# nyu-systems/CLM-GS

Measured on AMD Instinct MI355X. Metric: training images/s (Rubble-4K 28M Gaussians clm_offload), higher is better.
Workload: dtype f32

## Files before the change

clm_gs_amd/_lib.py:

```python
import ctypes
import os
import time

import torch

_HERE = os.path.dirname(os.path.abspath(__file__))
LIB_PATH = os.environ.get("CLMGS_LIB_PATH") or os.path.join(_HERE, "libclmgs_hip.so")

_vp, _i, _i64, _f, _sz = ctypes.c_void_p, ctypes.c_int, ctypes.c_int64, ctypes.c_float, ctypes.c_size_t
_d = ctypes.c_double

SIGNATURES = {
    "clmgs_version": (_i, []),
    "clmgs_last_error": (ctypes.c_char_p, []),
    "clmgs_projection_fwd": (_i, [_vp, _i, _i, _vp, _vp, _vp, _vp, _vp, _i, _i, _f, _f, _f, _f, _vp, _vp, _vp, _vp]),
    "clmgs_visibility_select_temp_bytes": (_sz, [_i, _i]),
    "clmgs_visibility_select_count": (_i, [_vp, _i, _i, _vp, _vp, _vp, _vp, _vp, _i, _i, _f, _f, _f, _f, _vp, _sz, _vp]),
    "clmgs_visibility_select_count_blocks": (_i, [_vp, _i, _i, _vp, _vp, _vp, _vp, _vp, _i, _i, _f, _f, _f, _f, _vp, _sz, _vp, _vp]),
    "clmgs_visibility_select_count_blocks_sel": (_i, [_vp, _i, _i, _vp, _vp, _vp, _vp, _vp, _i, _i, _f, _f, _f, _f, _vp, _sz, _vp, _vp,
                                                      _vp, ctypes.c_uint64, _i, _i]),
    "clmgs_visibility_select_emit": (_i, [_vp, _i, _i, _vp, _vp]),
    "clmgs_visibility_raw": (_i, [_vp, _i, _i, _vp, _vp, _vp, _vp, _vp, _i, _i, _f, _f, _f, _f, _vp]),
    "clmgs_projection_bwd": (_i, [_vp, _i, _i, _vp, _vp, _vp, _vp, _vp, _i, _i, _f, _vp, _vp, _vp, _vp, _vp, _vp, _vp]),
    "clmgs_sh_fwd": (_i, [_vp, _i, _i, _vp, _vp, _vp, _vp]),
    "clmgs_sh_bwd": (_i, [_vp, _i, _i, _vp, _vp, _vp, _vp, _vp, _i, _vp]),
    "clmgs_isect_count_temp_bytes": (_sz, [_i]),
    "clmgs_isect_count": (_i, [_vp, _i, _i, _vp, _vp, _i, _i, _i, _vp, _vp, _vp, _sz]),
    "clmgs_isect_sort_temp_bytes": (_sz, [_i64]),
    "clmgs_isect_emit_sort": (_i, [_vp, _i, _i, _i64, _vp, _vp, _vp, _vp, _i, _i, _i, _vp, _vp, _vp, _sz]),
    "clmgs_isect_offsets": (_i, [_vp, _i64, _vp, _i, _i, _i, _vp]),
    "clmgs_isect2_order_temp_bytes": (_sz, [_i]),
    "clmgs_isect2_order_count": (_i, [_vp, _i, _vp, _vp, _vp, _i, _i, _i, _vp, _vp, _vp, _vp, _vp, _vp, _sz, _vp]),
    "clmgs_isect2_sort_temp_bytes": (_sz, [_i64]),
    "clmgs_isect2_emit_sort": (_i, [_vp, _i, _i64, _vp, _vp, _vp, _vp, _i, _i, _vp, _vp, _vp, _vp, _vp, _sz, _vp]),
    "clmgs_isect2_emit_sort_dev": (_i, [_vp, _i, _i64, _vp, _vp, _vp, _vp, _vp, _i, _i, _vp, _vp, _vp, _vp, _vp, _sz, _vp]),
    "clmgs_isect3_front_temp_bytes": (_sz, [_i, _i]),
    "clmgs_isect3_front": (_i, [_vp, _i, _vp, _vp, _i, _i, _i, _vp, _vp, _vp, _vp, _sz]),
    "clmgs_isect3_bin_temp_bytes": (_sz, [_i64, _i]),
    "clmgs_isect3_bin": (_i, [_vp, _i, _i64, _vp, _i, _i, _vp, _vp, _vp, _vp, _vp, _vp, _vp, _sz]),
    "clmgs_isect3_bin_dev": (_i, [_vp, _i, _i64, _vp, _vp, _i, _i, _vp, _vp, _vp, _vp, _vp, _vp, _vp, _sz]),
    "clmgs_rasterize_fwd_dev": (_i, [_vp, _i, _i, _i64, _vp, _vp, _i, _i, _i, _i, _i, _vp, _vp, _vp, _vp, _vp, _vp]),
    "clmgs_rasterize_bwd_dev": (_i, [_vp, _i, _i, _i64, _vp, _vp, _vp, _i, _i, _i, _i, _i, _vp, _vp, _vp, _vp, _vp, _vp, _vp, _vp, _vp]),
    "clmgs_rasterize_pack_bytes": (_sz, [_i, _i]),
    "clmgs_rasterize_fwd": (_i, [_vp, _i, _i, _i64, _vp, _vp, _vp, _vp, _vp, _i, _i, _i, _i, _i, _vp, _vp, _vp, _vp, _vp, _vp]),
    "clmgs_rasterize_partials_bytes": (_sz, [_i64]),
    "clmgs_rasterize_bwd": (_i, [_vp, _i, _i, _i64, _vp, _vp, _i, _i, _i, _i, _i, _vp, _vp, _vp, _vp, _vp, _vp, _vp, _vp, _vp, _vp, _vp, _vp, _vp, _vp]),
    "clmgs_rasterize_contrib_pack_bytes": (_sz, [_i, _i]),
    "clmgs_rasterize_contrib": (_i, [_vp, _i, _i, _i64, _vp, _vp, _vp, _i, _i, _i, _i, _i, _vp, _vp, _vp, _i64, _vp, _vp, _vp, _vp]),
    "clmgs_rasterize_median_pack_bytes": (_sz, [_i, _i]),
    "clmgs_rasterize_median": (_i, [_vp, _i, _i, _i64, _vp, _vp, _vp, _vp, _i, _i, _i, _i, _i, _vp, _vp, _vp, _vp, _vp]),
    "clmgs_ray_depth": (_i, [_vp, _i, _i, _i, _i, _vp, _vp, _vp, _vp, _vp, _vp, _d, _i, _vp]),
    "clmgs_rasterize4_fwd": (_i, [_vp, _i, _i, _i64, _vp, _vp, _vp, _vp, _vp, _i, _i, _i, _i, _i, _vp, _vp, _vp, _vp, _vp, _vp]),
    "clmgs_rasterize4_bwd": (_i, [_vp, _i, _i, _i64, _vp, _vp, _i, _i, _i, _i, _i, _vp, _vp, _vp, _vp, _vp, _vp, _vp, _vp, _vp, _vp, _vp, _vp, _vp, _vp]),
    "clmgs_rasterize4_slot_bwd": (_i, [_vp, _i, _i, _i64, _vp, _vp, _i, _i, _i, _i, _i, _vp, _vp, _vp, _vp, _vp, _vp, _vp, _vp, _vp, _vp, _vp, _vp, _vp, _vp]),
    "clmgs_rasterize4_fwd_dev": (_i, [_vp, _i, _i, _i64, _vp, _vp, _i, _i, _i, _i, _i, _vp, _vp, _vp, _vp, _vp, _vp]),
    "clmgs_rasterize4_bwd_dev": (_i, [_vp, _i, _i, _i64, _vp, _vp, _vp, _i, _i, _i, _i, _i, _vp, _vp, _vp, _vp, _vp, _vp, _vp, _vp, _vp]),
    "clmgs_preprocess_grid_cap": (_i, []),
    "clmgs_preprocess_fwd": (_i, [_vp, _i, _vp, _vp, _vp, _vp, _vp, _vp, _i, _vp, _vp, _vp, _i, _i, _i, _f, _f, _f, _f, _vp, _vp, _vp, _vp, _vp, _vp, _vp, _vp]),
    "clmgs_preprocess_bwd": (_i, [_vp, _i, _vp, _vp, _vp, _vp, _vp, _vp, _i, _vp, _vp, _vp, _i, _i, _i, _f, _vp, _vp, _vp, _vp, _vp, _vp, _vp, _vp, _vp, _vp, _vp, _i, _vp, _vp, _vp, _vp, _i]),
    "clmgs_rasterize_abs_bwd": (_i, [_vp, _i, _i, _i64, _vp, _vp, _i, _i, _i, _i, _i, _vp, _vp, _vp, _vp, _vp, _vp, _vp, _vp, _vp, _vp, _vp, _vp, _vp, _vp, _vp]),
    "clmgs_rasterize_abs_bwd_dev": (_i, [_vp, _i, _i, _i64, _vp, _vp, _vp, _i, _i, _i, _i, _i, _vp, _vp, _vp, _vp, _vp, _vp, _vp, _vp, _vp]),
    "clmgs_preprocess_abs_bwd": (_i, [_vp, _i, _vp, _vp, _vp, _vp, _vp, _vp, _i, _vp, _vp, _vp, _i, _i, _i, _f, _vp, _vp, _vp, _vp, _vp, _vp, _vp, _vp, _vp, _vp, _vp, _i, _vp, _vp, _vp, _vp, _i, _vp]),
    "clmgs_projection_aa_fwd": (_i, [_vp, _i, _i, _vp, _vp, _vp, _vp, _vp, _i, _i, _f, _f, _f, _f, _vp, _vp, _vp, _vp, _vp]),
    "clmgs_projection_aa_bwd": (_i, [_vp, _i, _i, _vp, _vp, _vp, _vp, _vp, _i, _i, _f, _vp, _vp, _vp, _vp, _vp, _vp, _vp, _vp]),
    "clmgs_projection_ortho_fwd": (_i, [_vp, _i, _i, _vp, _vp, _vp, _vp, _vp, _i, _i, _f, _f, _f, _f, _vp, _vp, _vp, _vp, _vp]),
    "clmgs_projection_ortho_bwd": (_i, [_vp, _i, _i, _vp, _vp, _vp, _vp, _vp, _i, _i, _f, _vp, _vp, _vp, _vp, _vp, _vp, _vp, _vp]),
    "clmgs_preprocess_aa_fwd": (_i, [_vp, _i, _vp, _vp, _vp, _vp, _vp, _vp, _i, _vp, _vp, _vp, _i, _i, _i, _f, _f, _f, _f, _vp, _vp, _vp, _vp, _vp, _vp, _vp, _vp]),
    "clmgs_preprocess_aa_bwd": (_i, [_vp, _i, _vp, _vp, _vp, _vp, _vp, _vp, _i, _vp, _vp, _vp, _i, _i, _i, _f, _vp, _vp, _vp, _vp, _vp, _vp, _vp, _vp, _vp, _vp, _vp, _i, _vp, _vp, _vp, _vp, _i]),
    "clmgs_preprocess_aa_abs_bwd": (_i, [_vp, _i, _vp, _vp, _vp, _vp, _vp, _vp, _i, _vp, _vp, _vp, _i, _i, _i, _f, _vp, _vp, _vp, _vp, _vp, _vp, _vp, _vp, _vp, _vp, _vp, _i, _vp, _vp, _vp, _vp, _i, _vp]),
    "clmgs_ssim_fwd": (_i, [_vp, _i, _i, _i, _i, _vp, _vp, _vp, _vp, _vp, _vp]),
    "clmgs_ssim_bwd": (_i, [_vp, _i, _i, _i, _i, _vp, _vp, _vp, _f, _vp, _vp, _vp, _vp]),
    "clmgs_loss_slots": (_i, []),
    "clmgs_l1_ssim_loss_fwd": (_i, [_vp, _i, _i, _vp, _i64, _i64, _i64, _vp, _vp, _vp, _vp, _vp]),
    "clmgs_l1_ssim_loss_bwd": (_i, [_vp, _i, _i, _vp, _i64, _i64, _i64, _vp, _vp, _f, _vp, _vp, _vp, _vp]),
    "clmgs_l1_ssim_loss_masked_fwd": (_i, [_vp, _i, _i, _vp, _i64, _i64, _i64, _vp, _vp, _vp, _vp, _vp, _vp]),
    "clmgs_l1_ssim_loss_masked_bwd": (_i, [_vp, _i, _i, _vp, _i64, _i64, _i64, _vp, _vp, _f, _vp, _vp, _vp, _vp, _vp]),
    "clmgs_exposure_partials_rows": (_i, [_i, _i]),
    "clmgs_exposure_fwd": (_i, [_vp, _i, _i, _vp, _i64, _i64, _i64, _vp, _vp, _i64, _i64, _i64]),
    "clmgs_exposure_bwd": (_i, [_vp, _i, _i, _vp, _i64, _i64, _i64, _vp, _vp, _i64, _i64, _i64, _vp, _i64, _i64, _i64, _vp]),
    "clmgs_exposure_grad_finish": (_i, [_vp, _i, _vp, _vp]),
    "clmgs_bilagrid_partials_rows": (_i, [_i, _i, _i, _i]),
    "clmgs_bilagrid_fwd": (_i, [_vp, _i, _i, _vp, _i64, _i64, _i64, _vp, _i, _i, _i, _vp, _i64, _i64, _i64]),
    "clmgs_bilagrid_bwd": (_i, [_vp, _i, _i, _vp, _i64, _i64, _i64, _vp, _i, _i, _i, _vp, _i64, _i64, _i64, _vp, _i64, _i64, _i64, _vp]),
    "clmgs_bilagrid_grad_finish": (_i, [_vp, _i, _i, _i, _i, _i, _vp, _vp]),
    "clmgs_bilagrid_tv_grad": (_i, [_vp, _vp, _i64, _i, _i, _i, _f, _vp]),
    "clmgs_sky_fwd": (_i, [_vp, _i, _i, _vp, _i64, _i64, _i64, _vp, _vp, _vp, _vp, _i, _i, _vp, _i64, _i64, _i64]),
    "clmgs_sky_bwd": (_i, [_vp, _i, _i, _vp, _i64, _i64, _i64, _vp, _vp, _vp, _vp, _i, _i, _vp, _vp]),
    "clmgs_sky_acc_add": (_i, [_vp, _i64, _vp, _vp]),
    "clmgs_sky_grad_convert": (_i, [_vp, _i64, _vp, _vp]),
    "clmgs_pose_grad_partials_rows": (_i, [_i]),
    "clmgs_pose_grad": (_i, [_vp, _i, _vp, _vp, _vp, _vp, _vp, _vp, _i, _vp, _vp, _vp, _i, _i, _i, _f, _vp, _vp, _vp, _vp, _vp, _i, _vp]),
    "clmgs_pose_grad_finish": (_i, [_vp, _i, _vp, _vp]),
    "clmgs_projection_viewmat_partials_rows": (_i, [_i]),
    "clmgs_projection_viewmat_bwd": (_i, [_vp, _i, _i, _vp, _vp, _vp, _vp, _vp, _i, _i, _f, _vp, _vp, _vp, _vp, _vp, _vp, _vp]),
    "clmgs_invdepth_partials_rows": (_i, [_i, _i]),
    "clmgs_invdepth_pack": (_i, [_vp, _i, _vp, _vp, _vp]),
    "clmgs_invdepth_l1_fwd_bwd": (_i, [_vp, _i, _i, _vp, _i64, _i64, _vp, _f, _f, _vp, _f, _vp, _i64, _i64, _vp]),
    "clmgs_invdepth_finish": (_i, [_vp, _i, _vp, _vp]),
    "clmgs_invdepth_rows_bwd": (_i, [_vp, _i, _vp, _vp, _vp, _vp, _vp, _vp, _vp, _vp, _i]),
    "clmgs_area_resample_u8": (_i, [_vp, _i, _i, _i, _i, _vp, _vp]),
    "clmgs_area_resample_u16": (_i, [_vp, _i, _i, _i, _vp, _vp]),
    "clmgs_area_resample_mask": (_i, [_vp, _i, _i, _i, _vp, _vp, _vp]),
    "clmgs_undistort_u8": (_i, [_vp, _i, _i, _i, _i, _i, _vp, _i, _d, _d, _vp, _vp, _vp, _vp, _vp]),
    "clmgs_undistort_u16": (_i, [_vp, _i, _i, _i, _i, _vp, _i, _d, _d, _vp, _vp]),
    "clmgs_vq_assign_temp_bytes": (_sz, [_i]),
    "clmgs_vq_assign": (_i, [_vp, _i64, _i, _vp, _vp, _vp, _vp, _vp, _sz]),
    "clmgs_vq_accumulate": (_i, [_vp, _i64, _i, _vp, _vp, _d, _vp, _vp]),
    "clmgs_vq_finish": (_i, [_vp, _i, _vp, _vp, _d, _vp]),
    "clmgs_tsdf_integrate": (_i, [_vp, _i, _i, _i, _vp, _i, _i, _i, _vp, _vp, _vp, _vp, _f, _f, _f, _f, _f, _i]),
    "clmgs_tsdf_cells": (_i, [_vp, _i, _i, _i, _vp, _f, _vp]),
    "clmgs_tsdf_vertices": (_i, [_vp, _i, _i, _i, _vp, _vp, _i, _vp, _vp, _vp]),
    "clmgs_tsdf_quad_count": (_i, [_vp, _i, _i, _i, _vp, _f, _vp, _vp]),
    "clmgs_tsdf_quads": (_i, [_vp, _i, _i, _i, _vp, _f, _vp, _vp, _i, _i, _vp]),
    "clmgs_tsdf_mark": (_i, [_vp, _i, _i, _i, _vp, _i, _i, _i, _vp, _vp, _vp, _f, _f, _f, _f, _d]),
    "clmgs_tsdf_sparse_integrate": (_i, [_vp, _i, _i, _i, _i, _vp, _vp, _i, _i, _i, _vp, _vp, _vp, _vp, _f, _f, _f, _f, _f, _i]),
    "clmgs_tsdf_sparse_extract": (_i, [_vp, _i, _i, _i, _i, _i, _vp, _vp, _vp, _f, _vp, _vp, _vp, _i, _i, _vp, _vp, _vp, _vp,
                                       _vp, _vp]),
    "clmgs_mesh_hook": (_i, [_vp, _i, _i, _vp, _vp, _vp]),
    "clmgs_mesh_shortcut": (_i, [_vp, _i, _vp, _vp]),
    "clmgs_mesh_component_faces": (_i, [_vp, _i, _i, _vp, _vp, _vp]),
    "clmgs_mesh_decimate_mark": (_i, [_vp, _i, _i, _vp, _vp]),
    "clmgs_mesh_decimate_keys": (_i, [_vp, _i, _vp, _vp, _d, _vp, _vp]),
    "clmgs_mesh_decimate_faces": (_i, [_vp, _i, _i, _i, _vp, _vp, _vp, _vp, _vp]),
    "clmgs_mesh_decimate_place": (_i, [_vp, _i, _i, _i, _vp, _vp, _vp, _vp, _vp, _vp, _i64, _vp, _vp, _i64, _vp, _d, _vp, _vp,
                                       _vp]),
    "clmgs_mcmc_relocation": (_i, [_vp, _i64, _vp, _vp, _vp, _vp, _vp]),
    "clmgs_mcmc_reg_grad": (_i, [_vp, _i64, _vp, _i64, _vp, _i64, _vp, _i64, _vp, _i64, _f, _f]),
    "clmgs_mcmc_noise": (_i, [_vp, _i64, _vp, _vp, _vp, _vp, _vp, _f, _vp]),
    "clmgs_rows_gather": (_i, [_vp, _vp, _vp, _vp, _vp, _i, _i64, _i, _i]),
    "clmgs_rows_scatter_add": (_i, [_vp, _vp, _vp, _vp, _vp, _i, _i64, _i, _i]),
    "clmgs_scatter_to_bit": (_i, [_vp, _vp, _i, _vp, _i64, _i]),
    "clmgs_extract_ffs": (_i, [_vp, _vp, _i, _i64, _vp]),
    "clmgs_pair_overlap_count": (_i, [_vp, _vp, _i, _i64, _i, _vp]),
    "clmgs_set_signal": (_i, [_vp, _vp, _i, ctypes.c_int32]),
    "clmgs_adam_rows": (_i, [_vp, _vp, _vp, _vp, _vp, _vp, _i, _vp, _i64, _i, _vp, _d, _d, _d, _i, _i, _f, _i]),
    "clmgs_pack_small": (_i, [_vp, _i64, _vp, _vp, _vp, _vp, _vp]),
    "clmgs_adam_small_packed": (_i, [_vp, _i64, _vp, _vp, _vp, _vp, _vp, _vp, _d, _d, _d, _i, _i, _f, _vp, _i]),
    "clmgs_adam_catch_up": (_i, [_vp, _vp, _vp, _vp, _vp, _vp, _i, _i64, _i, _vp, _d, _d, _d, _i, _i, _i, _vp, _vp, _f, _i]),
    "clmgs_host_adam_rows": (_i, [_vp, _vp, _vp, _vp, _vp, _i64, _i, _vp, _d, _d, _d, _i, _i, _f, _i, _vp, _i]),
    "clmgs_host_pool_start": (_i, [_i]),
    "clmgs_host_usable_cpus": (_i, []),
    "clmgs_memcpy_async": (_i, [_vp, _vp, _vp, _sz, _i]),
    "clmgs_host_rows_prepare": (_i, [_vp, _vp, _vp, _vp, _vp, _vp, _vp, _i64, _i, _vp, _d, _d, _d, _i, _i, _i, _f, _i, _vp, _i]),
    "clmgs_densify_stats": (_i, [_vp, _i64, _vp, _vp, _vp, _i, _f, _f, _vp, _vp, _vp]),
    "clmgs_morton_order_temp_bytes": (_sz, [_i64]),
    "clmgs_morton_order": (_i, [_vp, _i64, _vp, _vp, _vp, _vp, _sz]),
    "clmgs_tsp_tour": (_i, [_i, _vp, _vp]),
    "clmgs_knn3_mean_dist2": (_i, [_vp, _i, _vp, _vp, _f, _f, _f, _f, _i, _i, _i, _i, _vp]),
    "clmgs_host_groups_temp_bytes": (_sz, [_i64]),
    "clmgs_host_groups": (_i, [_vp, _i64, _vp, _vp, _i, _i, _vp, _i, _vp, _vp, _vp, _vp, _vp, _sz]),
    "clmgs_publish_pack": (_i, [_vp, _vp, _vp, _vp, _vp, _i, _i64, _i64, _i64, _i]),
    "clmgs_visibility_candidates": (_i, [_vp, _i, _i, _i, _i, _vp, _vp, _vp, _vp, _i, _i, _f, _f, _f, _f, _f, _vp]),
    "clmgs_small_rows_scatter": (_i, [_vp, _i64, _vp, _vp, _vp, _vp, _vp, _vp, _vp]),
    "clmgs_adam_small_packed_range": (_i, [_vp, _i64, _i64, _i64, _vp, _vp, _vp, _vp, _vp, _vp, _d, _d, _d, _i, _i, _f, _vp, _i]),
    "clmgs_small_deferred_kmax": (_i, []),
    "clmgs_adam_small_deferred": (_i, [_vp, _i64, _vp, _vp, _vp, _vp, _vp, _vp, _vp, _i, _i, _vp, _vp, _vp, _vp, _d, _d, _d,
                                       _f, _i, _vp, _vp, _i, _i, _f, _f, _f, _i, _vp]),
    "clmgs_adam_small_deferred_sel": (_i, [_vp, _i64, _vp, _vp, _vp, _vp, _vp, _vp, _vp, _i, _i, _vp, _vp, _vp, _vp, _d, _d, _d,
                                           _f, _i, _vp, _vp, _i, _i, _f, _f, _f, _i, _vp, _vp, _vp, ctypes.c_uint64, _i]),
    "clmgs_device_errors": (_i, [_vp, _i]),
    "clmgs_pinned_alloc": (_vp, [_sz]),
    "clmgs_pinned_free": (_i, [_vp]),
}

_lib = None

TIMING = None
STATS = {"n_isects": [], "n_emitted": [], "host_wait_s": 0.0}


class ClmgsError(RuntimeError):
    pass


class _Entry:

    def __init__(self, name, fn, takes_stream):
        self.name, self.fn, self.takes_stream = name, fn, takes_stream

    def __call__(self, *args):
        if TIMING is None or not self.takes_stream:
            return self.fn(*args)
        s, e = torch.cuda.Event(enable_timing=True), torch.cuda.Event(enable_timing=True)
        h = getattr(args[0], "value", args[0])
        st = torch.cuda.ExternalStream(h) if h else torch.cuda.current_stream()
        s.record(st)
        rc = self.fn(*args)
        e.record(st)
        TIMING.setdefault(self.name, []).append((s, e))
        return rc


class _Namespace:
    pass


_NO_STREAM = {"clmgs_version", "clmgs_loss_slots", "clmgs_preprocess_grid_cap","clmgs_exposure_partials_rows", "clmgs_bilagrid_partials_rows", "clmgs_invdepth_partials_rows", "clmgs_pose_grad_partials_rows", "clmgs_projection_viewmat_partials_rows", "clmgs_small_deferred_kmax", "clmgs_isect3_front_temp_bytes",
              "clmgs_isect3_bin_temp_bytes", "clmgs_last_error", "clmgs_isect_count_temp_bytes",
              "clmgs_isect_sort_temp_bytes", "clmgs_host_groups_temp_bytes", "clmgs_isect2_order_temp_bytes", "clmgs_isect2_sort_temp_bytes", "clmgs_visibility_select_temp_bytes", "clmgs_rasterize_pack_bytes", "clmgs_rasterize_contrib_pack_bytes", "clmgs_rasterize_median_pack_bytes", "clmgs_rasterize_partials_bytes", "clmgs_host_adam_rows", "clmgs_host_pool_start", "clmgs_host_usable_cpus", "clmgs_host_rows_prepare", "clmgs_tsp_tour",
              "clmgs_pinned_alloc", "clmgs_pinned_free", "clmgs_device_errors", "clmgs_vq_assign_temp_bytes"}


def timing_summary():
    out = {}
    for name, evs in (TIMING or {}).items():
        out[name] = (len(evs), sum(s.elapsed_time(e) for s, e in evs))
    return out


def lib():
    global _lib
    if _lib is None:
        if not os.path.exists(LIB_PATH):
            raise ClmgsError(
                f"{LIB_PATH} not found: build it with `python -c 'import __graft_entry__ as g; g.build()'` "
                "(make -C clm_gs_amd/csrc).  clm_gs_amd has no CPU/eager fallback."
            )
        l = ctypes.CDLL(LIB_PATH)
        ns = _Namespace()
        for name, (res, args) in SIGNATURES.items():
            fn = getattr(l, name)
            fn.restype = res
# ... 88 lines not shown
```

clm_gs_amd/csrc/clm_ops.hip:

```cpp
#include <stdlib.h>

#include "common.h"
#include "vis_math.h"
#include "radix.h"

namespace clmgs {
__device__ uint32_t g_dev_err;
static uint32_t* device_error_word() {
  static thread_local uint32_t* p[16] = {nullptr};
  int dev = 0;
  if (hipGetDevice(&dev) != hipSuccess || dev < 0 || dev >= 16) dev = 0;
  if (!p[dev]) {
    void* a = nullptr;
    if (hipGetSymbolAddress(&a, HIP_SYMBOL(g_dev_err)) == hipSuccess) p[dev] = (uint32_t*)a;
  }
  return p[dev];
}


template <typename IdxT>
__device__ __forceinline__ int64_t row_of(const void* idx, int64_t i) {
  return idx ? (int64_t)reinterpret_cast<const IdxT*>(idx)[i] : i;
}

template <typename IdxT, bool ADD>
__global__ void __launch_bounds__(256)
rows_move_f4_kernel(float* __restrict__ dst, const float* __restrict__ src,
                    const void* __restrict__ dst_idx, const void* __restrict__ src_idx,
                    int64_t n_rows, int f4_per_row) {
  const int64_t total = n_rows * f4_per_row;
  for (int64_t i = blockIdx.x * (int64_t)blockDim.x + threadIdx.x; i < total;
       i += (int64_t)gridDim.x * blockDim.x) {
    const int64_t r = i / f4_per_row;
    const int k = (int)(i - r * f4_per_row);
    const int64_t sr = row_of<IdxT>(src_idx, r), dr = row_of<IdxT>(dst_idx, r);
    const float4 v = reinterpret_cast<const float4*>(src)[sr * f4_per_row + k];
    float4* d = reinterpret_cast<float4*>(dst) + dr * f4_per_row + k;
    if (ADD) {
      float4 o = *d;
      o.x += v.x; o.y += v.y; o.z += v.z; o.w += v.w;
      *d = o;
    } else {
      *d = v;
    }
  }
}

template <typename IdxT, bool ADD>
__global__ void __launch_bounds__(256)
rows_move_f1_kernel(float* __restrict__ dst, const float* __restrict__ src,
                    const void* __restrict__ dst_idx, const void* __restrict__ src_idx,
                    int64_t n_rows, int cols) {
  const int64_t total = n_rows * cols;
  for (int64_t i = blockIdx.x * (int64_t)blockDim.x + threadIdx.x; i < total;
       i += (int64_t)gridDim.x * blockDim.x) {
    const int64_t r = i / cols;
    const int k = (int)(i - r * cols);
    const int64_t sr = row_of<IdxT>(src_idx, r), dr = row_of<IdxT>(dst_idx, r);
    const float v = src[sr * cols + k];
    if (ADD) dst[dr * cols + k] += v; else dst[dr * cols + k] = v;
  }
}

template <bool ADD>
static int rows_move(void* stream, float* dst, const float* src, const void* dst_idx,
                     const void* src_idx, int idx_is_64, int64_t n_rows, int cols,
                     int grid_blocks) {
  CLMGS_CHECK_ARG(n_rows >= 0 && cols > 0);
  if (n_rows == 0) return 0;
  CLMGS_CHECK_ARG(dst && src);
  hipStream_t s = (hipStream_t)stream;
  const bool f4 = (cols % 4 == 0) && (((uintptr_t)dst | (uintptr_t)src) % 16 == 0);
  const int64_t total = f4 ? n_rows * (cols / 4) : n_rows * cols;
  int grid = grid_blocks > 0 ? grid_blocks : min(ceil_div(total, 256), 256 * 8);
  if (f4) {
    if (idx_is_64)
      hipLaunchKernelGGL((rows_move_f4_kernel<int64_t, ADD>), dim3(grid), dim3(256), 0, s, dst, src,
                         dst_idx, src_idx, n_rows, cols / 4);
    else
      hipLaunchKernelGGL((rows_move_f4_kernel<int32_t, ADD>), dim3(grid), dim3(256), 0, s, dst, src,
                         dst_idx, src_idx, n_rows, cols / 4);
  } else {
    if (idx_is_64)
      hipLaunchKernelGGL((rows_move_f1_kernel<int64_t, ADD>), dim3(grid), dim3(256), 0, s, dst, src,
                         dst_idx, src_idx, n_rows, cols);
    else
      hipLaunchKernelGGL((rows_move_f1_kernel<int32_t, ADD>), dim3(grid), dim3(256), 0, s, dst, src,
                         dst_idx, src_idx, n_rows, cols);
  }
  CLMGS_LAUNCH_CHECK();
  return 0;
}

__global__ void __launch_bounds__(256)
publish_pack_kernel(float* __restrict__ msg, const float* __restrict__ table, const int64_t* __restrict__ own,
                    const int32_t* __restrict__ stamp, int step, int64_t lo, int64_t n, int64_t chunk, int f4_per_row) {
  const int64_t total = n * f4_per_row;
  for (int64_t i = blockIdx.x * (int64_t)blockDim.x + threadIdx.x; i < total;
       i += (int64_t)gridDim.x * blockDim.x) {
    const int64_t r = i / f4_per_row;
    const int k = (int)(i - r * f4_per_row);
    const int64_t row = own[r];
    const bool live = !stamp || stamp[row] == step;
    float4 v = make_float4(0.f, 0.f, 0.f, 0.f);
    if (live) v = reinterpret_cast<const float4*>(table)[row * f4_per_row + k];
    reinterpret_cast<float4*>(msg)[i] = v;
    if (k == 0) reinterpret_cast<int32_t*>(msg)[chunk * f4_per_row * 4 + r] = (int32_t)(row - lo);
  }
}

template <typename T>
__global__ void __launch_bounds__(256)
host_group_keys_kernel(int64_t n, const int64_t* __restrict__ touched, const T* __restrict__ bitmap, int bsz,
                       const uint8_t* __restrict__ staged, uint32_t* __restrict__ kf, uint32_t* __restrict__ kl,
                       int32_t* __restrict__ rows32) {
  for (int64_t j = blockIdx.x * (int64_t)blockDim.x + threadIdx.x; j < n; j += (int64_t)gridDim.x * blockDim.x) {
    const int64_t row = touched[j];
    unsigned long long bm = (unsigned long long)(typename std::make_unsigned<T>::type)bitmap[row];
    if (bsz < 64) bm &= (1ull << bsz) - 1ull;
    int first = 254, last = 254;
    if (bm) {
      first = (bsz - 1) - (63 - __clzll((long long)bm));
      last = (bsz - 1) - (__ffsll((long long)bm) - 1);
    }
    kf[j] = (staged && staged[row]) ? 255u : (uint32_t)first;
    kl[j] = (uint32_t)last;
    rows32[j] = (int32_t)row;
  }
}

__global__ void __launch_bounds__(256)
host_group_finish_kernel(int64_t n, int bsz, const uint32_t* __restrict__ tot_first, const uint32_t* __restrict__ tot_last,
                         const int32_t* __restrict__ late_sorted, int slot0, int32_t* __restrict__ slot_of,
                         int64_t* __restrict__ counts) {
  const int64_t n_late = n - (int64_t)tot_first[255];
  if (blockIdx.x == 0 && threadIdx.x <= 2 * bsz) {
    const int t = threadIdx.x;
    counts[t] = t < bsz ? (int64_t)tot_first[t] : (t < 2 * bsz ? (int64_t)tot_last[t - bsz] : n_late);
  }
  for (int64_t k = blockIdx.x * (int64_t)blockDim.x + threadIdx.x; k < n_late; k += (int64_t)gridDim.x * blockDim.x)
    slot_of[late_sorted[k]] = slot0 + (int32_t)k;
}

template <typename T>
__global__ void scatter_to_bit_kernel(T* __restrict__ bitmap, const int64_t* __restrict__ filter,
                                      int64_t n, int bit) {
  using U = typename std::make_unsigned<T>::type;
  const U m = (U)((U)1 << bit);
  for (int64_t i = blockIdx.x * (int64_t)blockDim.x + threadIdx.x; i < n;
       i += (int64_t)gridDim.x * blockDim.x) {
    U* p = reinterpret_cast<U*>(bitmap) + filter[i];
    *p = (U)(*p | m);
  }
}

template <typename T>
__global__ void extract_ffs_kernel(const T* __restrict__ bitmap, int64_t N, uint8_t* __restrict__ ffs) {
  using U = typename std::make_unsigned<T>::type;
  for (int64_t i = blockIdx.x * (int64_t)blockDim.x + threadIdx.x; i < N;
       i += (int64_t)gridDim.x * blockDim.x) {
    const unsigned long long v = (unsigned long long)(U)bitmap[i];
    ffs[i] = (uint8_t)(v ? (__ffsll((long long)v)) : 0);
  }
}

template <typename T>
__global__ void __launch_bounds__(256)
pair_overlap_kernel(const T* __restrict__ bitmap, int64_t N, int bsz, int32_t* __restrict__ cnt) {
  using U = typename std::make_unsigned<T>::type;
  __shared__ int sh[64];
  for (int i = threadIdx.x; i < 64; i += blockDim.x) sh[i] = 0;
  __syncthreads();
  for (int64_t i = blockIdx.x * (int64_t)blockDim.x + threadIdx.x; i < N;
       i += (int64_t)gridDim.x * blockDim.x) {
    const unsigned long long v = (unsigned long long)(U)bitmap[i];
    unsigned long long both = v & (v << 1);
    while (both) {
      const int b = __ffsll((long long)both) - 1;
      both &= both - 1;
      atomicAdd(&sh[bsz - 1 - b], 1);
    }
  }
  __syncthreads();
  for (int i = threadIdx.x; i < bsz - 1; i += blockDim.x)
    if (sh[i]) atomicAdd(&cnt[i], sh[i]);
}

__global__ void set_signal_kernel(int32_t* signal, int idx, int32_t value) {
  __threadfence_system();
  __hip_atomic_store(signal + idx, value, __ATOMIC_RELEASE, __HIP_MEMORY_SCOPE_SYSTEM);
}

__device__ __forceinline__ float adam_update(float p, float m, float v, float lr_bc, float inv_sqrt_bc2, float eps) {
#pragma clang fp contract(off)
  const float ratio = m * __builtin_amdgcn_rcpf(__builtin_fmaf(__builtin_amdgcn_sqrtf(v), inv_sqrt_bc2, eps));
  return __builtin_fmaf(-lr_bc, ratio, p);
}

template <bool GRAD_FUSED = false>
__device__ __forceinline__ float adam_elem(float& m, float& v, float p, float g, float lr_bc, float beta1,
                                           float beta2, float ob1, float ob2, float eps,
                                           float inv_sqrt_bc2) {
#pragma clang fp contract(off)
  if constexpr (GRAD_FUSED) {
    m = __builtin_fmaf(ob1, g, beta1 * m);
    v = __builtin_fmaf(ob2 * g, g, beta2 * v);
  } else {
    m = __builtin_fmaf(beta1, m, ob1 * g);
    v = __builtin_fmaf(beta2, v, (ob2 * g) * g);
  }
  return adam_update(p, m, v, lr_bc, inv_sqrt_bc2, eps);
}

__device__ __forceinline__ float adam_elem_nograd(float& m, float& v, float p, float lr_bc, float beta1, float beta2,
                                                  float eps, float inv_sqrt_bc2) {
#pragma clang fp contract(off)
  m = beta1 * m;
  v = beta2 * v;
  return adam_update(p, m, v, lr_bc, inv_sqrt_bc2, eps);
}

template <int VEC> struct VecT;
template <> struct VecT<1> { using type = float; };
template <> struct VecT<4> { using type = float4; };
template <int VEC> __device__ __forceinline__ void vload(const float* a, float (&x)[VEC]) {
  if constexpr (VEC == 4) { const float4 t = *reinterpret_cast<const float4*>(a); x[0] = t.x; x[1] = t.y; x[2] = t.z; x[3] = t.w; }
  else x[0] = *a;
}
template <int VEC> __device__ __forceinline__ void vstore(float* a, const float (&x)[VEC]) {
  if constexpr (VEC == 4) *reinterpret_cast<float4*>(a) = make_float4(x[0], x[1], x[2], x[3]);
  else *a = x[0];
}

template <typename IdxT, int VEC>
__global__ void __launch_bounds__(256)
adam_rows_kernel(float* __restrict__ p, float* __restrict__ g, float* __restrict__ m,
                 float* __restrict__ v, const void* __restrict__ rows,
                 const uint8_t* __restrict__ mask, int64_t n_rows, int cols,
                 const float* __restrict__ col_lr, float beta1, float beta2, float ob1, float ob2,
                 float eps, float inv_bc1, float inv_sqrt_bc2, float grad_scale, int zero_grad) {
  const int cv = cols / VEC;
  const int64_t total = n_rows * cv;
  for (int64_t i = blockIdx.x * (int64_t)blockDim.x + threadIdx.x; i < total;
       i += (int64_t)gridDim.x * blockDim.x) {
    const int64_t r = i / cv;
    const int k = (int)(i - r * cv) * VEC;
    const int64_t row = row_of<IdxT>(rows, r);
    if (mask && !mask[row]) continue;
    const int64_t o = row * cols + k;
    float gg[VEC], mm[VEC], vv[VEC], pp[VEC], lr[VEC];
    vload<VEC>(m + o, mm); vload<VEC>(v + o, vv); vload<VEC>(p + o, pp); vload<VEC>(col_lr + k, lr);
    if (g) vload<VEC>(g + o, gg);
#pragma unroll
    for (int c = 0; c < VEC; ++c) {
      pp[c] = adam_elem(mm[c], vv[c], pp[c], g ? gg[c] * grad_scale : 0.f, lr[c] * inv_bc1, beta1, beta2, ob1, ob2,
                        eps, inv_sqrt_bc2);
      gg[c] = 0.f;
    }
    vstore<VEC>(m + o, mm); vstore<VEC>(v + o, vv); vstore<VEC>(p + o, pp);
    if (zero_grad && g) vstore<VEC>(g + o, gg);
  }
}

__device__ __forceinline__ float pow_beta(float beta, float x) {
  return __builtin_amdgcn_exp2f(x * __builtin_amdgcn_logf(beta));
}

struct CatchUpK {
  float beta1, beta2, ob1, ob2, eps, grad_scale;
  int bias_correction, max_replay;
};

__device__ __forceinline__ void adam_bias(const CatchUpK& K, float pw1, float pw2, float& inv_bc1, float& inv_sqrt_bc2) {
#pragma clang fp contract(off)
  inv_bc1 = inv_sqrt_bc2 = 1.f;
  if (K.bias_correction) {
    inv_bc1 = 1.f / (1.f - pw1);
    inv_sqrt_bc2 = 1.f / sqrtf(1.f - pw2);
  }
}

template <int VEC>
__device__ __forceinline__ void adam_replay(const CatchUpK& K, int from, int to, float (&pp)[VEC], float (&mm)[VEC],
                                            float (&vv)[VEC], const float (&lr)[VEC]) {
#pragma clang fp contract(off)
  const int missed = to - from;
  if (missed <= 0) return;
  const int n = min(missed, K.max_replay);
  float pw1 = pow_beta(K.beta1, (float)(from + 1)), pw2 = pow_beta(K.beta2, (float)(from + 1));
  for (int j = 0; j < n; ++j) {
    float inv_bc1, inv_sqrt_bc2;
    adam_bias(K, pw1, pw2, inv_bc1, inv_sqrt_bc2);
#pragma unroll
    for (int c = 0; c < VEC; ++c)
      pp[c] = adam_elem_nograd(mm[c], vv[c], pp[c], lr[c] * inv_bc1, K.beta1, K.beta2, K.eps, inv_sqrt_bc2);
    pw1 = pw1 * K.beta1; pw2 = pw2 * K.beta2;
  }
  if (missed > n) {
    const int d = missed - n;
    const float f1 = pow_beta(K.beta1, (float)d), f2 = pow_beta(K.beta2, (float)d);
#pragma unroll
    for (int c = 0; c < VEC; ++c) { mm[c] = mm[c] * f1; vv[c] = vv[c] * f2; }
  }
}

template <int VEC>
__device__ __forceinline__ void adam_waiting_step(const CatchUpK& K, int gs, float (&pp)[VEC], float (&mm)[VEC],
                                                  float (&vv)[VEC], float (&gg)[VEC], const float (&lr)[VEC]) {
#pragma clang fp contract(off)
  float inv_bc1, inv_sqrt_bc2;
  adam_bias(K, pow_beta(K.beta1, (float)gs), pow_beta(K.beta2, (float)gs), inv_bc1, inv_sqrt_bc2);
#pragma unroll
  for (int c = 0; c < VEC; ++c) {
    pp[c] = adam_elem<true>(mm[c], vv[c], pp[c], gg[c] * K.grad_scale, lr[c] * inv_bc1, K.beta1, K.beta2, K.ob1, K.ob2,
                            K.eps, inv_sqrt_bc2);
    gg[c] = 0.f;
  }
}

template <int VEC> __device__ __forceinline__ bool adam_any_state(const float (&mm)[VEC], const float (&vv)[VEC]) {
  bool any_state = false;
#pragma unroll
  for (int c = 0; c < VEC; ++c) any_state |= (mm[c] != 0.f) | (vv[c] != 0.f);
  return any_state;
}

template <typename IdxT, int VEC>
__global__ void __launch_bounds__(256)
adam_catch_up_kernel(float* __restrict__ p, float* __restrict__ m, float* __restrict__ v,
                     const int32_t* __restrict__ last_step, const void* __restrict__ rows,
                     int64_t n_rows, int cols, const float* __restrict__ col_lr, float beta1,
                     float beta2, float eps, int to_step, int bias_correction, int max_replay,
                     float* __restrict__ g, const int32_t* __restrict__ g_step, float grad_scale,
                     float ob1, float ob2,
                     int keep_grad) {
  const CatchUpK K = {beta1, beta2, ob1, ob2, eps, grad_scale, bias_correction, max_replay};
  const int cv = cols / VEC;
  const int64_t total = n_rows * cv;
  for (int64_t i = blockIdx.x * (int64_t)blockDim.x + threadIdx.x; i < total;
       i += (int64_t)gridDim.x * blockDim.x) {
    const int64_t r = i / cv;
    const int k = (int)(i - r * cv) * VEC;
    const int64_t row = row_of<IdxT>(rows, r);
    int a = last_step[row];
    const int gs = g_step ? g_step[row] : 0;
    const bool pending = gs > a && gs <= to_step;
    if (to_step - a <= 0) continue;
    const int64_t o = row * cols + k;
    float mm[VEC], vv[VEC], pp[VEC], lr[VEC], gg[VEC];
    vload<VEC>(m + o, mm); vload<VEC>(v + o, vv); vload<VEC>(p + o, pp); vload<VEC>(col_lr + k, lr);
    if (pending) vload<VEC>(g + o, gg);
    if (!pending && !adam_any_state<VEC>(mm, vv)) continue;
    if (pending) {
      adam_replay<VEC>(K, a, gs - 1, pp, mm, vv, lr);
      adam_waiting_step<VEC>(K, gs, pp, mm, vv, gg, lr);
      if (!keep_grad) vstore<VEC>(g + o, gg);
      a = gs;
    }
    adam_replay<VEC>(K, a, to_step, pp, mm, vv, lr);
    vstore<VEC>(m + o, mm); vstore<VEC>(v + o, vv); vstore<VEC>(p + o, pp);
  }
}

template <typename IdxT>
__global__ void __launch_bounds__(256)
adam_catch_up48_kernel(float* __restrict__ p, float* __restrict__ m, float* __restrict__ v,
                       const int32_t* __restrict__ last_step, const void* __restrict__ rows,
                       unsigned n_rows, const float* __restrict__ col_lr, float beta1,
                       float beta2, float eps, int to_step, int bias_correction, int max_replay,
                       float* __restrict__ g, const int32_t* __restrict__ g_step, float grad_scale,
                       float ob1, float ob2, int keep_grad) {
  constexpr int VEC = 4;
  const CatchUpK K = {beta1, beta2, ob1, ob2, eps, grad_scale, bias_correction, max_replay};
  const unsigned t0 = blockIdx.x * 256u + threadIdx.x;
  const unsigned r_stride = gridDim.x * 256u / 12u;
  unsigned r = t0 / 12u;
  const int k = (int)(t0 - r * 12u) * VEC;
  if (r >= n_rows) return;
  float lr[VEC];
  vload<VEC>(col_lr + k, lr);
  int64_t row_next = row_of<IdxT>(rows, (int64_t)r);
  int a_next = last_step[row_next];
  int gs_next = g_step ? g_step[row_next] : 0;
  int64_t row_next2 = (r + r_stride < n_rows) ? row_of<IdxT>(rows, (int64_t)(r + r_stride)) : row_next;
  for (; r < n_rows; r += r_stride) {
    const int64_t row = row_next;
    int a = a_next;
    const int gs = gs_next;
    row_next = row_next2;
    if (r + r_stride < n_rows) {
      a_next = last_step[row_next];
      gs_next = g_step ? g_step[row_next] : 0;
      if (r + 2 * r_stride < n_rows) row_next2 = row_of<IdxT>(rows, (int64_t)(r + 2 * r_stride));
    }
    const int64_t o = row * 48 + k;
    float mm[VEC], vv[VEC], pp[VEC], gg[VEC];
    const bool pending = gs > a && gs <= to_step;
    if (to_step - a <= 0) continue;
    vload<VEC>(m + o, mm); vload<VEC>(v + o, vv); vload<VEC>(p + o, pp);
    if (pending) vload<VEC>(g + o, gg);
    if (!pending && !adam_any_state<VEC>(mm, vv)) continue;
    if (pending) {
      adam_replay<VEC>(K, a, gs - 1, pp, mm, vv, lr);
      adam_waiting_step<VEC>(K, gs, pp, mm, vv, gg, lr);
      if (!keep_grad) vstore<VEC>(g + o, gg);
      a = gs;
    }
    adam_replay<VEC>(K, a, to_step, pp, mm, vv, lr);
    vstore<VEC>(m + o, mm); vstore<VEC>(v + o, vv); vstore<VEC>(p + o, pp);
  }
}

struct SmallAdam {
  float* p[4]; float* m[4]; float* v[4];
  float lr[4];
};

constexpr int SA_ROWS = 256;

__device__ __forceinline__ constexpr int small_w(int ti) { return ti == 0 ? 3 : (ti == 1 ? 1 : (ti == 2 ? 3 : 4)); }
__device__ __forceinline__ constexpr int small_co(int ti) { return ti == 0 ? 0 : (ti == 1 ? 3 : (ti == 2 ? 4 : 7)); }

template <typename Admit>
__device__ __forceinline__ void small_stage(float (&sg)[SA_ROWS * 12], const float4* __restrict__ packed_g,
                                            int64_t row0, int rows, Admit admit) {
#pragma clang loop unroll(disable) vectorize(disable) interleave(disable)
  for (int i = threadIdx.x; i < rows * 3; i += SA_ROWS)
    reinterpret_cast<float4*>(sg)[i] = admit(i / 3) ? packed_g[row0 * 3 + i] : make_float4(0.f, 0.f, 0.f, 0.f);
}

template <typename Step>
__device__ __forceinline__ void small_walk(const SmallAdam& t, int64_t row0, int rows, const float* sg, float* sp,
                                           float grad_scale, Step step) {
  const int tid = threadIdx.x;
  if (tid < rows) sp[tid * 12 + 11] = 0.f;
  __syncthreads();
#pragma unroll
  for (int ti = 0; ti < 4; ++ti) {
    const int w = small_w(ti), co = small_co(ti);
    const int n_el = rows * w;
    float* P = t.p[ti] + row0 * w;
    float* M = t.m[ti] + row0 * w;
    float* V = t.v[ti] + row0 * w;
    for (int i = tid * 4; i < n_el; i += SA_ROWS * 4) {
      if (i + 3 < n_el) {
        float4 p4 = *reinterpret_cast<float4*>(P + i), m4 = *reinterpret_cast<float4*>(M + i),
               v4 = *reinterpret_cast<float4*>(V + i);
        float pp[4] = {p4.x, p4.y, p4.z, p4.w}, mm[4] = {m4.x, m4.y, m4.z, m4.w},
              vv[4] = {v4.x, v4.y, v4.z, v4.w};
        float gg[4];
        int row[4];
#pragma unroll
        for (int k = 0; k < 4; ++k) {
          row[k] = (i + k) / w;
          gg[k] = sg[row[k] * 12 + co + (i + k - row[k] * w)] * grad_scale;
        }
        step(ti, row, pp, mm, vv, gg);
#pragma unroll
        for (int k = 0; k < 4; ++k) sp[row[k] * 12 + co + (i + k - row[k] * w)] = pp[k];
        *reinterpret_cast<float4*>(P + i) = make_float4(pp[0], pp[1], pp[2], pp[3]);
        *reinterpret_cast<float4*>(M + i) = make_float4(mm[0], mm[1], mm[2], mm[3]);
        *reinterpret_cast<float4*>(V + i) = make_float4(vv[0], vv[1], vv[2], vv[3]);
      } else {
        for (int idx = i; idx < n_el; ++idx) {
          const int row[1] = {idx / w};
          float pp[1] = {P[idx]}, mm[1] = {M[idx]}, vv[1] = {V[idx]};
          const float gg[1] = {sg[row[0] * 12 + co + (idx - row[0] * w)] * grad_scale};
          step(ti, row, pp, mm, vv, gg);
          P[idx] = pp[0]; M[idx] = mm[0]; V[idx] = vv[0];
          sp[row[0] * 12 + co + (idx - row[0] * w)] = pp[0];
        }
      }
    }
  }
  __syncthreads();
}

// ... 642 lines not shown
```

clm_gs_amd/csrc/preprocess.hip:

```cpp
#include <stdlib.h>

#include "common.h"
#include "gs_math.h"

namespace clmgs {

constexpr int PP_ROWS = 64;
constexpr int PP_PITCH = 52;
constexpr int PP_GRID_CAP = 256 * 12;

struct PreArgs {
  const int64_t* filter;
  const float* xyz;
  const float* opacity_raw;
  const float* scaling_raw;
  const float* rotation_raw;
  const float* sh_rows;
  int sh_by_filter;
  const int32_t* sh_index;
  int packed_small;
  float viewmat[16];
  float K[9];
  float campos[3];
  int width, height, degree;
  float eps2d, near_plane, far_plane, radius_clip;
};

#define CLMGS_FOR12(X) X(0) X(1) X(2) X(3) X(4) X(5) X(6) X(7) X(8) X(9) X(10) X(11)
#define CLMGS_DECL_ST(j) float4 st##j = make_float4(0.f, 0.f, 0.f, 0.f);
#define CLMGS_ELEM(j) const int e = tl + PP_ROWS * j, r = e / NF4, k = e - r * NF4;
#define CLMGS_LAUNDER_LANE int tl = t; asm volatile("" : "+v"(tl));

__device__ __forceinline__ float sigmoidf(float x) { return 1.f / (1.f + __expf(-x)); }

struct SmallRow { float m[3]; float4 q4; float s[3]; float oraw; };
template <bool PK>
__device__ __forceinline__ SmallRow load_small(const PreArgs& a, int64_t g) {
  SmallRow r;
  if (PK) {
    const float4* row = reinterpret_cast<const float4*>(a.xyz) + 3 * g;
    const float4 r0 = row[0], r1 = row[1], r2 = row[2];
    r.m[0] = r0.x; r.m[1] = r0.y; r.m[2] = r0.z; r.oraw = r0.w;
    r.s[0] = r1.x; r.s[1] = r1.y; r.s[2] = r1.z;
    r.q4 = make_float4(r1.w, r2.x, r2.y, r2.z);
  } else {
    r.m[0] = a.xyz[3 * g]; r.m[1] = a.xyz[3 * g + 1]; r.m[2] = a.xyz[3 * g + 2];
    r.q4 = *reinterpret_cast<const float4*>(a.rotation_raw + 4 * g);
    r.s[0] = a.scaling_raw[3 * g]; r.s[1] = a.scaling_raw[3 * g + 1]; r.s[2] = a.scaling_raw[3 * g + 2];
    r.oraw = a.opacity_raw[g];
  }
  return r;
}

__device__ __forceinline__ Cam launder_cam(const Cam& c) {
  Cam r = c;
#pragma unroll
  for (int i = 0; i < 9; ++i) asm volatile("" : "+s"(r.R[i]));
#pragma unroll
  for (int i = 0; i < 3; ++i) asm volatile("" : "+s"(r.t[i]));
  asm volatile("" : "+s"(r.fx)); asm volatile("" : "+s"(r.fy));
  asm volatile("" : "+s"(r.cx)); asm volatile("" : "+s"(r.cy));
  return r;
}

__device__ __forceinline__ void wave_lds_sync() {
  __builtin_amdgcn_fence(__ATOMIC_RELEASE, "wavefront");
  __builtin_amdgcn_wave_barrier();
  __builtin_amdgcn_fence(__ATOMIC_ACQUIRE, "wavefront");
}

template <int DEG, bool OVERLAP, bool PK, bool AA = false>
__global__ void __launch_bounds__(PP_ROWS, 3)
preprocess_fwd_kernel(int V, PreArgs a, int32_t* __restrict__ radii, float* __restrict__ means2d,
                      float* __restrict__ depths, float* __restrict__ conics,
                      float* __restrict__ colors, float* __restrict__ opacities,
                      float4* __restrict__ packed) {
  constexpr int NB = (DEG + 1) * (DEG + 1);
  constexpr int NF4 = (NB * 3 + 3) / 4;
  __shared__ __attribute__((aligned(16))) float lds[PP_ROWS * PP_PITCH];
  const Cam cam = load_cam(a.viewmat, a.K);
  const int n_chunks = (V + PP_ROWS - 1) / PP_ROWS;
  const int t = threadIdx.x;
  int chunk = blockIdx.x;
  int my_row = -1, my_sh = 0;
  if (chunk < n_chunks && chunk * PP_ROWS + t < V) {
    my_row = a.filter ? (int)a.filter[chunk * PP_ROWS + t] : chunk * PP_ROWS + t;
    my_sh = a.sh_index ? a.sh_index[chunk * PP_ROWS + t] : my_row;
  }
  for (; chunk < n_chunks; chunk += gridDim.x) {
    const int base = chunk * PP_ROWS;
    const bool mine = my_row >= 0;
    const int64_t g = mine ? my_row : 0;
    const int sh_id = mine ? my_sh : 0;
    const SmallRow sr = load_small<PK>(a, g);
    const float m[3] = {sr.m[0], sr.m[1], sr.m[2]};
    const float4 q4 = sr.q4;
    const float s[3] = {sr.s[0], sr.s[1], sr.s[2]};
    const float oraw = sr.oraw;
    CLMGS_FOR12(CLMGS_DECL_ST)
    if (OVERLAP) {
#define CLMGS_X(j)                                                                                  \
  if constexpr (j < NF4) {                                                                          \
    CLMGS_ELEM(j)                                                                                   \
    const int64_t src = a.sh_by_filter ? (int64_t)__shfl(sh_id, r) : (int64_t)min(base + r, V - 1); \
    st##j = *reinterpret_cast<const float4*>(a.sh_rows + src * 48 + 4 * k);                         \
  }
      { CLMGS_LAUNDER_LANE
      CLMGS_FOR12(CLMGS_X)
      }
#undef CLMGS_X
    }
    {
      const int ni = (chunk + (int)gridDim.x) * PP_ROWS + t;
      my_row = -1;
      if (ni < V) { my_row = a.filter ? (int)a.filter[ni] : ni; my_sh = a.sh_index ? a.sh_index[ni] : my_row; }
    }
    Proj p;
    p.radius = 0; p.mx = p.my = p.depth = p.ca = p.cb = p.cc = 0.f;
    float o = 0.f;
    if (mine) {
      const float q[4] = {q4.x, q4.y, q4.z, q4.w};
      const float se[3] = {__expf(s[0]), __expf(s[1]), __expf(s[2])};
      o = sigmoidf(oraw);
      if constexpr (AA) {
        float comp;
        p = project_fwd_aa(cam, m, q, se, (float)a.width, (float)a.height, a.eps2d, a.near_plane,
                           a.far_plane, a.radius_clip, comp);
        o *= comp;
      } else {
        p = project_fwd(cam, m, q, se, (float)a.width, (float)a.height, a.eps2d, a.near_plane,
                        a.far_plane, a.radius_clip);
      }
    }
    wave_lds_sync();
    if (OVERLAP) {
#define CLMGS_X(j)                                                                                  \
  if constexpr (j < NF4) {                                                                          \
    CLMGS_ELEM(j)                                                                                   \
    *reinterpret_cast<float4*>(lds + r * PP_PITCH + 4 * k) = st##j;                                 \
  }
      { CLMGS_LAUNDER_LANE
      CLMGS_FOR12(CLMGS_X)
      }
#undef CLMGS_X
    } else {
      const unsigned long long live = __ballot(p.radius > 0);
      const int first = live ? (int)__builtin_ctzll(live) : 0;
      if (live) {
#pragma unroll
        for (int j = 0; j < NF4; ++j) {
          const int e = t + PP_ROWS * j, r = e / NF4, k = e - r * NF4;
          const int rr = ((live >> r) & 1ull) ? r : first;
          const int64_t src = a.sh_by_filter ? (int64_t)__shfl(sh_id, rr) : (int64_t)(base + rr);
          *reinterpret_cast<float4*>(lds + r * PP_PITCH + 4 * k) =
              *reinterpret_cast<const float4*>(a.sh_rows + src * 48 + 4 * k);
        }
      }
    }
    wave_lds_sync();
    if (mine) {
      const int i = base + t;
      float cr = 0.f, cg = 0.f, cb = 0.f;
      if (p.radius > 0) {
        float x = m[0] - a.campos[0], y = m[1] - a.campos[1], z = m[2] - a.campos[2];
        const float inv = 1.0f / sqrtf(x * x + y * y + z * z);
        x *= inv; y *= inv; z *= inv;
        float B[16];
        sh_basis(DEG, x, y, z, B);
        const float* row = lds + t * PP_PITCH;
#pragma unroll
        for (int k = 0; k < NB; ++k) { cr += B[k] * row[3 * k]; cg += B[k] * row[3 * k + 1]; cb += B[k] * row[3 * k + 2]; }
        cr = fmaxf(cr + 0.5f, 0.f); cg = fmaxf(cg + 0.5f, 0.f); cb = fmaxf(cb + 0.5f, 0.f);
      }
      radii[i] = p.radius;
      *reinterpret_cast<float2*>(means2d + 2 * (size_t)i) = make_float2(p.mx, p.my);
      depths[i] = p.depth;
      if (conics) {
        conics[3 * (size_t)i] = p.ca; conics[3 * (size_t)i + 1] = p.cb; conics[3 * (size_t)i + 2] = p.cc;
        colors[3 * (size_t)i] = cr; colors[3 * (size_t)i + 1] = cg; colors[3 * (size_t)i + 2] = cb;
        opacities[i] = o;
      }
      float4* rec = packed + 4 * (size_t)i;
      rec[0] = make_float4(p.mx, p.my, o, p.ca);
      rec[1] = make_float4(p.cb, p.cc, cr, cg);
      rec[2] = make_float4(cb, 0.f, 0.f, 0.f);
    }
  }
}

struct PreGrads {
  float* g_xyz;
  float* g_opacity;
  float* g_scaling;
  float* g_rotation;
  float* g_sh_rows;
  float* max_radii2D;
  float* grad_accum;
  float* denom;
  int packed_grads;
  int packed_stats;
  float* v_means2d_out;
  int stats_only_visible;
  const float4* partials;
  const int64_t* row_cum;
  int32_t* sh_stamp;
  int cur_step;
};

template <bool ABS> struct PreGradsOf : PreGrads {};
template <> struct PreGradsOf<true> : PreGrads { float* v_means2d_abs_out; };

template <int DEG, bool PK, bool ABS = false, bool AA = false>
__global__ void __launch_bounds__(PP_ROWS, 2)
preprocess_bwd_kernel(int V, PreArgs a, const int32_t* __restrict__ radii,
                      const float4* __restrict__ packed_grad, PreGradsOf<ABS> o) {
  constexpr int NB = (DEG + 1) * (DEG + 1);
  constexpr int NF4 = (NB * 3 + 3) / 4;
  __shared__ __attribute__((aligned(16))) float lds[PP_ROWS * PP_PITCH];
  const Cam cam = load_cam(a.viewmat, a.K);
  const int n_chunks = (V + PP_ROWS - 1) / PP_ROWS;
  const int t = threadIdx.x;
  int chunk = blockIdx.x;
  int my_row = -1, my_radius = 0, my_sh = 0, my_stamp = 0;
  int64_t my_s0 = 0;
  int my_cnt = 0;
  if (chunk < n_chunks && chunk * PP_ROWS + t < V) {
    const int i = chunk * PP_ROWS + t;
    my_row = a.filter ? (int)a.filter[i] : i;
    my_sh = a.sh_index ? a.sh_index[i] : my_row;
    my_radius = radii[i];
    if (o.sh_stamp) my_stamp = o.sh_stamp[my_sh];
    if (o.partials) { my_s0 = i ? o.row_cum[i - 1] : 0; my_cnt = (int)(o.row_cum[i] - my_s0); }
  }
  for (; chunk < n_chunks; chunk += gridDim.x) {
    const int base = chunk * PP_ROWS;
    const int radius = my_radius;
    const int64_t s0 = my_s0;
    const int cnt = my_cnt;
    const bool mine = my_row >= 0;
    const bool vis = mine && radius > 0;
    const bool stat = mine && o.max_radii2D && (radius > 0 || !o.stats_only_visible);
    const unsigned long long live = __ballot(vis);
    const int first = live ? (int)__builtin_ctzll(live) : 0;
    const int64_t g = mine ? my_row : 0;
    const int sh_id = mine ? my_sh : 0;
    const bool fresh = o.sh_stamp && vis && (my_stamp != o.cur_step);
    const unsigned long long fresh_rows = __ballot(fresh);
    const int64_t gl = vis ? g : (int64_t)__shfl((int)g, first);
    const int i = mine ? base + t : base;
    float4 ga, gb;
    float go;
    float4 pa[4], pb[4];
    float po[4];
    float2 gq = make_float2(0.f, 0.f), pq[4];
    if (o.partials) {
      ga = make_float4(0.f, 0.f, 0.f, 0.f); gb = ga; go = 0.f;
      const float4* src = o.partials + PART_F4 * (size_t)s0;
#pragma unroll
      for (int u = 0; u < 4; ++u) {
        pa[u] = ga; pb[u] = ga; po[u] = 0.f;
        if constexpr (ABS) pq[u] = gq;
        if (mine && u < cnt) {
          pa[u] = src[PART_F4 * u]; pb[u] = src[PART_F4 * u + 1];
          if constexpr (ABS) { const float4 c = src[PART_F4 * u + 2]; po[u] = c.x; pq[u] = make_float2(c.z, c.w); }
          else po[u] = src[PART_F4 * u + 2].x;
        }
      }
    } else {
      ga = packed_grad[4 * (size_t)i];
      gb = packed_grad[4 * (size_t)i + 1];
      if constexpr (ABS) { const float4 c = packed_grad[4 * (size_t)i + 2]; go = c.x; gq = make_float2(c.z, c.w); }
      else go = packed_grad[4 * (size_t)i + 2].x;
    }
    const SmallRow sr = load_small<PK>(a, gl);
    const float m[3] = {sr.m[0], sr.m[1], sr.m[2]};
    const float4 q4 = sr.q4;
    const float s[3] = {sr.s[0], sr.s[1], sr.s[2]};
    const float oraw = sr.oraw;
    float c_xyz[3], c_sc[3], c_op;
    float4 c_rot;
    if (PK) {
      const float4* grow = reinterpret_cast<const float4*>(o.g_xyz) + 3 * gl;
      float4 g0 = make_float4(0.f, 0.f, 0.f, 0.f), g1 = g0, g2 = g0;
      if (!fresh) { g0 = grow[0]; g1 = grow[1]; g2 = grow[2]; }
// ... 70 lines not shown
    }
    if (stat) {
      const float gx = (ABS ? gq.x : v_m2[0]) * (0.5f * a.width), gy = (ABS ? gq.y : v_m2[1]) * (0.5f * a.height);
      if (o.packed_stats) {
        reinterpret_cast<float4*>(o.max_radii2D)[g] =
            make_float4(fmaxf(c_mr, (float)radius), c_ga + sqrtf(gx * gx + gy * gy), c_dn + 1.f, 0.f);
      } else {
        o.max_radii2D[g] = fmaxf(c_mr, (float)radius);
        o.grad_accum[g] = c_ga + sqrtf(gx * gx + gy * gy);
        o.denom[g] = c_dn + 1.f;
      }
    }
    float vm[3] = {0.f, 0.f, 0.f};
    float n_sc[3] = {0.f, 0.f, 0.f}, n_op = 0.f;
    float4 n_rot = make_float4(0.f, 0.f, 0.f, 0.f);
    if (vis) {
      const float q[4] = {q4.x, q4.y, q4.z, q4.w};
      const float se[3] = {__expf(s[0]), __expf(s[1]), __expf(s[2])};
      const float op = sigmoidf(oraw);
      const float v_con[3] = {ga.z, ga.w, gb.x};
      float vq[4], vs[3];
      const Cam camL = launder_cam(cam);
      float gk = go;
      if constexpr (AA)
        gk *= project_bwd_aa(camL, m, q, se, (float)a.width, (float)a.height, a.eps2d, v_m2, 0.f, v_con, go * op, vm, vq, vs);
      else
        project_bwd(camL, m, q, se, (float)a.width, (float)a.height, a.eps2d, v_m2, 0.f, v_con, vm, vq, vs);
      n_sc[0] = c_sc[0] + vs[0] * se[0]; n_sc[1] = c_sc[1] + vs[1] * se[1]; n_sc[2] = c_sc[2] + vs[2] * se[2];
      n_rot = make_float4(c_rot.x + vq[0], c_rot.y + vq[1], c_rot.z + vq[2], c_rot.w + vq[3]);
      n_op = c_op + gk * op * (1.f - op);
      if (!PK) {
        o.g_scaling[3 * g] = n_sc[0]; o.g_scaling[3 * g + 1] = n_sc[1]; o.g_scaling[3 * g + 2] = n_sc[2];
        *reinterpret_cast<float4*>(o.g_rotation + 4 * g) = n_rot;
        o.g_opacity[g] = n_op;
      }
    }
    if (!live) continue;
    { CLMGS_LAUNDER_LANE CLMGS_FOR12(CLMGS_LOAD_SH) }
#undef CLMGS_LOAD_SH
    wave_lds_sync();
#define CLMGS_X(j)                                                                                  \
  if constexpr (j < NF4) {                                                                          \
    CLMGS_ELEM(j)                                                                                   \
    *reinterpret_cast<float4*>(lds + r * PP_PITCH + 4 * k) = st##j;                                 \
  }
    { CLMGS_LAUNDER_LANE
    CLMGS_FOR12(CLMGS_X)
    }
#undef CLMGS_X
    wave_lds_sync();
    if (vis) {
      float* row = lds + t * PP_PITCH;
      float dx = m[0] - a.campos[0], dy = m[1] - a.campos[1], dz = m[2] - a.campos[2];
      const float inv = 1.0f / sqrtf(dx * dx + dy * dy + dz * dz);
      const float x = dx * inv, y = dy * inv, z = dz * inv;
      float B[16];
      sh_basis(DEG, x, y, z, B);
      float P[3] = {0.f, 0.f, 0.f};
      float U[3][3] = {{0.f, 0.f, 0.f}, {0.f, 0.f, 0.f}, {0.f, 0.f, 0.f}};
      {
        float Bx[16], By[16], Bz[16];
        if (DEG > 0) sh_basis_grad(DEG, x, y, z, Bx, By, Bz);
#pragma unroll
        for (int k = 0; k < NB; ++k) {
          if (k == 1 || k == 4 || k == 9) __builtin_amdgcn_sched_barrier(0);
          const float rk[3] = {row[3 * k], row[3 * k + 1], row[3 * k + 2]};
#pragma unroll
          for (int c = 0; c < 3; ++c) {
            P[c] += B[k] * rk[c];
            if (DEG > 0 && k > 0) { U[c][0] += rk[c] * Bx[k]; U[c][1] += rk[c] * By[k]; U[c][2] += rk[c] * Bz[k]; }
          }
        }
      }
      const float vc[3] = {(P[0] + 0.5f > 0.f) ? gb.y : 0.f, (P[1] + 0.5f > 0.f) ? gb.z : 0.f,
                           (P[2] + 0.5f > 0.f) ? gb.w : 0.f};
      float vdx = 0.f, vdy = 0.f, vdz = 0.f;
      if (DEG > 0) {
        const float ux = vc[0] * U[0][0] + vc[1] * U[1][0] + vc[2] * U[2][0];
        const float uy = vc[0] * U[0][1] + vc[1] * U[1][1] + vc[2] * U[2][1];
        const float uz = vc[0] * U[0][2] + vc[1] * U[1][2] + vc[2] * U[2][2];
        const float dot = ux * x + uy * y + uz * z;
        vdx = (ux - dot * x) * inv; vdy = (uy - dot * y) * inv; vdz = (uz - dot * z) * inv;
      }
#pragma unroll
      for (int k = 0; k < 4 * NF4 / 3 + 1 && k < 16; ++k) {
        const float bk = (k < NB) ? B[k] : 0.f;
        row[3 * k] = bk * vc[0]; row[3 * k + 1] = bk * vc[1]; row[3 * k + 2] = bk * vc[2];
      }
      if (PK) {
        float4* grow = reinterpret_cast<float4*>(o.g_xyz) + 3 * g;
        grow[0] = make_float4(c_xyz[0] + vm[0] + vdx, c_xyz[1] + vm[1] + vdy, c_xyz[2] + vm[2] + vdz, n_op);
        grow[1] = make_float4(n_sc[0], n_sc[1], n_sc[2], n_rot.x);
        grow[2] = make_float4(n_rot.y, n_rot.z, n_rot.w, 0.f);
      } else {
        o.g_xyz[3 * g] = c_xyz[0] + vm[0] + vdx;
        o.g_xyz[3 * g + 1] = c_xyz[1] + vm[1] + vdy;
        o.g_xyz[3 * g + 2] = c_xyz[2] + vm[2] + vdz;
      }
    }
    wave_lds_sync();
    int g_l = sh_id;
    asm volatile("" : "+v"(g_l));
#define CLMGS_X(j)                                                                                  \
  if constexpr (j < NF4) {                                                                          \
    CLMGS_ELEM(j)                                                                                   \
    const int64_t dst_row = a.sh_by_filter ? (int64_t)__shfl(g_l, r) : (int64_t)(base + r);         \
    if ((live >> r) & 1ull) {                                                                       \
      const float4 v = *reinterpret_cast<const float4*>(lds + r * PP_PITCH + 4 * k);                \
      float4 c = make_float4(0.f, 0.f, 0.f, 0.f);                                                   \
      if (!((fresh_rows >> r) & 1ull))                                                              \
        c = *reinterpret_cast<const float4*>(o.g_sh_rows + dst_row * 48 + 4 * k);                   \
      c.x += v.x; c.y += v.y; c.z += v.z; c.w += v.w;                                               \
      *reinterpret_cast<float4*>(o.g_sh_rows + dst_row * 48 + 4 * k) = c;                           \
    }                                                                                               \
  }
    { CLMGS_LAUNDER_LANE
    CLMGS_FOR12(CLMGS_X)
    }
#undef CLMGS_X
    if (fresh) o.sh_stamp[sh_id] = o.cur_step;
  }
}

}

using namespace clmgs;

static void fill_args(PreArgs& a, const int64_t* filter, const float* xyz, const float* opacity_raw,
                      const float* scaling_raw, const float* rotation_raw, const float* sh_rows,
                      int sh_by_filter, const float* viewmat, const float* K, const float* campos,
                      int width, int height, int degree, float eps2d, float near_plane,
                      float far_plane, float radius_clip) {
  a.filter = filter; a.xyz = xyz; a.opacity_raw = opacity_raw; a.scaling_raw = scaling_raw;
  a.rotation_raw = rotation_raw; a.sh_rows = sh_rows; a.sh_by_filter = sh_by_filter; a.sh_index = nullptr;
  a.packed_small = (!opacity_raw && !scaling_raw && !rotation_raw) ? 1 : 0;
  for (int i = 0; i < 16; ++i) a.viewmat[i] = viewmat[i];
  for (int i = 0; i < 9; ++i) a.K[i] = K[i];
  for (int i = 0; i < 3; ++i) a.campos[i] = campos[i];
  a.width = width; a.height = height; a.degree = degree;
  a.eps2d = eps2d; a.near_plane = near_plane; a.far_plane = far_plane; a.radius_clip = radius_clip;
}

extern "C" int clmgs_preprocess_grid_cap(void) { return PP_GRID_CAP; }

template <bool AA>
static int preprocess_fwd_impl(void* stream, int V, const int64_t* filter, const float* xyz,
                                    const float* opacity_raw, const float* scaling_raw,
                                    const float* rotation_raw, const float* sh_rows,
                                    int sh_by_filter, const float* viewmat_host,
                                    const float* K_host, const float* campos_host, int width,
                                    int height, int degree, float eps2d, float near_plane,
                                    float far_plane, float radius_clip, int32_t* radii,
                                    float* means2d, float* depths, float* conics, float* colors,
                                    float* opacities, void* packed, const int32_t* sh_index) {
  CLMGS_CHECK_ARG(V >= 0 && degree >= 0 && degree <= 3 && width > 0 && height > 0);
  if (V == 0) return 0;
  CLMGS_CHECK_ARG(xyz && sh_rows && viewmat_host && K_host && campos_host && radii && means2d &&
                  depths && packed);
  CLMGS_CHECK_ARG((opacity_raw && scaling_raw && rotation_raw) ||
                  (!opacity_raw && !scaling_raw && !rotation_raw && (((uintptr_t)xyz & 15) == 0)));
  CLMGS_CHECK_ARG(!conics || (colors && opacities));
  PreArgs a;
  fill_args(a, filter, xyz, opacity_raw, scaling_raw, rotation_raw, sh_rows, sh_by_filter,
            viewmat_host, K_host, campos_host, width, height, degree, eps2d, near_plane, far_plane,
            radius_clip);
  CLMGS_CHECK_ARG(!sh_index || sh_by_filter);
  a.sh_index = sh_index;
  const size_t lds = 0;
  const int grid = min(ceil_div(V, PP_ROWS), PP_GRID_CAP);
#define CLMGS_PRE_FWD(D, O)                                                                        \
  do {                                                                                             \
    if (a.packed_small)                                                                            \
      hipLaunchKernelGGL((preprocess_fwd_kernel<D, O, true, AA>), dim3(grid), dim3(PP_ROWS), lds,      \
                         (hipStream_t)stream, V, a, radii, means2d, depths, conics, colors,        \
                         opacities, (float4*)packed);                                              \
    else                                                                                           \
      hipLaunchKernelGGL((preprocess_fwd_kernel<D, O, false, AA>), dim3(grid), dim3(PP_ROWS), lds,     \
                         (hipStream_t)stream, V, a, radii, means2d, depths, conics, colors,        \
                         opacities, (float4*)packed);                                              \
  } while (0)
  const bool ov = filter != nullptr;
  switch (degree) {
    case 0: if (ov) CLMGS_PRE_FWD(0, true); else CLMGS_PRE_FWD(0, false); break;
    case 1: if (ov) CLMGS_PRE_FWD(1, true); else CLMGS_PRE_FWD(1, false); break;
    case 2: if (ov) CLMGS_PRE_FWD(2, true); else CLMGS_PRE_FWD(2, false); break;
    default: if (ov) CLMGS_PRE_FWD(3, true); else CLMGS_PRE_FWD(3, false); break;
  }
#undef CLMGS_PRE_FWD
  CLMGS_LAUNCH_CHECK();
  return 0;
}

#define CLMGS_PRE_FWD_PARAMS                                                                       \
  void* stream, int V, const int64_t* filter, const float* xyz, const float* opacity_raw,          \
  const float* scaling_raw, const float* rotation_raw, const float* sh_rows, int sh_by_filter,     \
  const float* viewmat_host, const float* K_host, const float* campos_host, int width, int height, \
  int degree, float eps2d, float near_plane, float far_plane, float radius_clip, int32_t* radii,   \
  float* means2d, float* depths, float* conics, float* colors, float* opacities, void* packed,     \
  const int32_t* sh_index
#define CLMGS_PRE_FWD_ARGS                                                                         \
  stream, V, filter, xyz, opacity_raw, scaling_raw, rotation_raw, sh_rows, sh_by_filter,           \
  viewmat_host, K_host, campos_host, width, height, degree, eps2d, near_plane, far_plane,          \
  radius_clip, radii, means2d, depths, conics, colors, opacities, packed, sh_index

extern "C" int clmgs_preprocess_fwd(CLMGS_PRE_FWD_PARAMS) { return preprocess_fwd_impl<false>(CLMGS_PRE_FWD_ARGS); }

extern "C" int clmgs_preprocess_aa_fwd(CLMGS_PRE_FWD_PARAMS) { return preprocess_fwd_impl<true>(CLMGS_PRE_FWD_ARGS); }

template <bool ABS>
static const PreGradsOf<ABS>& pre_grads_of(const PreGradsOf<false>& plain, const PreGradsOf<true>& abs) {
  if constexpr (ABS) return abs; else return plain;
}

template <bool AA>
static int preprocess_bwd_impl(bool abs, float* v_means2d_abs_out, void* stream, int V, const int64_t* filter, const float* xyz,
                                    const float* opacity_raw, const float* scaling_raw,
                                    const float* rotation_raw, const float* sh_rows,
                                    int sh_by_filter, const float* viewmat_host,
                                    const float* K_host, const float* campos_host, int width,
                                    int height, int degree, float eps2d, const int32_t* radii,
                                    const void* packed_grad, float* g_xyz, float* g_opacity,
                                    float* g_scaling, float* g_rotation, float* g_sh_rows,
                                    float* max_radii2D, float* grad_accum, float* denom,
                                    float* v_means2d_out, int stats_only_visible,
                                    const void* partials, const int64_t* row_cum,
                                    const int32_t* sh_index, int32_t* sh_stamp, int cur_step) {
  CLMGS_CHECK_ARG(V >= 0 && degree >= 0 && degree <= 3 && width > 0 && height > 0);
  CLMGS_CHECK_ARG(!sh_stamp || (sh_by_filter && cur_step >= 1));
  if (V == 0) return 0;
  CLMGS_CHECK_ARG(xyz && sh_rows && viewmat_host && K_host && campos_host && radii && g_xyz && g_sh_rows);
  CLMGS_CHECK_ARG((packed_grad != nullptr) != (partials != nullptr));
  CLMGS_CHECK_ARG(!partials || (row_cum && (((uintptr_t)partials & 15) == 0)));
  CLMGS_CHECK_ARG((opacity_raw && scaling_raw && rotation_raw) ||
                  (!opacity_raw && !scaling_raw && !rotation_raw && (((uintptr_t)xyz & 15) == 0)));
  const bool pg = !g_opacity && !g_scaling && !g_rotation;
  CLMGS_CHECK_ARG(pg || (g_opacity && g_scaling && g_rotation));
  CLMGS_CHECK_ARG(pg == (!opacity_raw && !scaling_raw && !rotation_raw) && (!pg || (((uintptr_t)g_xyz & 15) == 0)));
  const bool ps = max_radii2D && !grad_accum && !denom;
  CLMGS_CHECK_ARG(!max_radii2D || ps || (grad_accum && denom));
  CLMGS_CHECK_ARG(!ps || (((uintptr_t)max_radii2D & 15) == 0));
  PreArgs a;
  fill_args(a, filter, xyz, opacity_raw, scaling_raw, rotation_raw, sh_rows, sh_by_filter,
            viewmat_host, K_host, campos_host, width, height, degree, eps2d, 0.f, 0.f, 0.f);
  CLMGS_CHECK_ARG(!sh_index || sh_by_filter);
  a.sh_index = sh_index;
  PreGrads o{g_xyz, g_opacity, g_scaling, g_rotation, g_sh_rows, max_radii2D, grad_accum, denom,
             pg ? 1 : 0, ps ? 1 : 0, v_means2d_out, stats_only_visible, (const float4*)partials, row_cum,
             sh_stamp, cur_step};
  const size_t lds = 0;
  const int grid = min(ceil_div(V, PP_ROWS), PP_GRID_CAP);
  PreGradsOf<false> o0;
  PreGradsOf<true> o1;
  static_cast<PreGrads&>(o0) = o; static_cast<PreGrads&>(o1) = o; o1.v_means2d_abs_out = v_means2d_abs_out;
#define CLMGS_PRE_BWD_K(D, PKD, A)                                                                \
  hipLaunchKernelGGL((preprocess_bwd_kernel<D, PKD, A, AA>), dim3(grid), dim3(PP_ROWS), lds,           \
                     (hipStream_t)stream, V, a, radii, (const float4*)packed_grad, pre_grads_of<A>(o0, o1))
#define CLMGS_PRE_BWD(D)                                                                          \
  do {                                                                                             \
    if (abs) { if (pg) CLMGS_PRE_BWD_K(D, true, true); else CLMGS_PRE_BWD_K(D, false, true); }     \
    else if (pg) CLMGS_PRE_BWD_K(D, true, false);                                                  \
    else CLMGS_PRE_BWD_K(D, false, false);                                                         \
  } while (0)
  switch (degree) {
    case 0: CLMGS_PRE_BWD(0); break;
    case 1: CLMGS_PRE_BWD(1); break;
    case 2: CLMGS_PRE_BWD(2); break;
    default: CLMGS_PRE_BWD(3); break;
  }
#undef CLMGS_PRE_BWD
#undef CLMGS_PRE_BWD_K
  CLMGS_LAUNCH_CHECK();
  return 0;
}

extern "C" int clmgs_preprocess_bwd(void* stream, int V, const int64_t* filter, const float* xyz,
                                    const float* opacity_raw, const float* scaling_raw,
                                    const float* rotation_raw, const float* sh_rows,
                                    int sh_by_filter, const float* viewmat_host,
                                    const float* K_host, const float* campos_host, int width,
                                    int height, int degree, float eps2d, const int32_t* radii,
                                    const void* packed_grad, float* g_xyz, float* g_opacity,
                                    float* g_scaling, float* g_rotation, float* g_sh_rows,
                                    float* max_radii2D, float* grad_accum, float* denom,
                                    float* v_means2d_out, int stats_only_visible,
                                    const void* partials, const int64_t* row_cum,
                                    const int32_t* sh_index, int32_t* sh_stamp, int cur_step) {
  return preprocess_bwd_impl<false>(false, nullptr, stream, V, filter, xyz, opacity_raw, scaling_raw, rotation_raw, sh_rows,
                             sh_by_filter, viewmat_host, K_host, campos_host, width, height, degree, eps2d, radii,
                             packed_grad, g_xyz, g_opacity, g_scaling, g_rotation, g_sh_rows, max_radii2D, grad_accum,
                             denom, v_means2d_out, stats_only_visible, partials, row_cum, sh_index, sh_stamp, cur_step);
}

extern "C" int clmgs_preprocess_abs_bwd(void* stream, int V, const int64_t* filter, const float* xyz,
                                        const float* opacity_raw, const float* scaling_raw,
                                        const float* rotation_raw, const float* sh_rows,
                                        int sh_by_filter, const float* viewmat_host,
                                        const float* K_host, const float* campos_host, int width,
                                        int height, int degree, float eps2d, const int32_t* radii,
                                        const void* packed_grad, float* g_xyz, float* g_opacity,
                                        float* g_scaling, float* g_rotation, float* g_sh_rows,
                                        float* max_radii2D, float* grad_accum, float* denom,
                                        float* v_means2d_out, int stats_only_visible,
                                        const void* partials, const int64_t* row_cum,
                                        const int32_t* sh_index, int32_t* sh_stamp, int cur_step,
                                        float* v_means2d_abs_out) {
  return preprocess_bwd_impl<false>(true, v_means2d_abs_out, stream, V, filter, xyz, opacity_raw, scaling_raw, rotation_raw,
                             sh_rows, sh_by_filter, viewmat_host, K_host, campos_host, width, height, degree, eps2d, radii,
                             packed_grad, g_xyz, g_opacity, g_scaling, g_rotation, g_sh_rows, max_radii2D, grad_accum,
                             denom, v_means2d_out, stats_only_visible, partials, row_cum, sh_index, sh_stamp, cur_step);
}

extern "C" int clmgs_preprocess_aa_bwd(void* stream, int V, const int64_t* filter, const float* xyz,
                                       const float* opacity_raw, const float* scaling_raw,
                                       const float* rotation_raw, const float* sh_rows,
                                       int sh_by_filter, const float* viewmat_host,
                                       const float* K_host, const float* campos_host, int width,
                                       int height, int degree, float eps2d, const int32_t* radii,
                                       const void* packed_grad, float* g_xyz, float* g_opacity,
                                       float* g_scaling, float* g_rotation, float* g_sh_rows,
                                       float* max_radii2D, float* grad_accum, float* denom,
                                       float* v_means2d_out, int stats_only_visible,
                                       const void* partials, const int64_t* row_cum,
                                       const int32_t* sh_index, int32_t* sh_stamp, int cur_step) {
  return preprocess_bwd_impl<true>(false, nullptr, stream, V, filter, xyz, opacity_raw, scaling_raw, rotation_raw, sh_rows,
                                   sh_by_filter, viewmat_host, K_host, campos_host, width, height, degree, eps2d, radii,
                                   packed_grad, g_xyz, g_opacity, g_scaling, g_rotation, g_sh_rows, max_radii2D, grad_accum,
                                   denom, v_means2d_out, stats_only_visible, partials, row_cum, sh_index, sh_stamp, cur_step);
}

extern "C" int clmgs_preprocess_aa_abs_bwd(void* stream, int V, const int64_t* filter, const float* xyz,
                                           const float* opacity_raw, const float* scaling_raw,
                                           const float* rotation_raw, const float* sh_rows,
                                           int sh_by_filter, const float* viewmat_host,
                                           const float* K_host, const float* campos_host, int width,
                                           int height, int degree, float eps2d, const int32_t* radii,
                                           const void* packed_grad, float* g_xyz, float* g_opacity,
                                           float* g_scaling, float* g_rotation, float* g_sh_rows,
                                           float* max_radii2D, float* grad_accum, float* denom,
                                           float* v_means2d_out, int stats_only_visible,
                                           const void* partials, const int64_t* row_cum,
                                           const int32_t* sh_index, int32_t* sh_stamp, int cur_step,
                                           float* v_means2d_abs_out) {
  return preprocess_bwd_impl<true>(true, v_means2d_abs_out, stream, V, filter, xyz, opacity_raw, scaling_raw, rotation_raw,
                                   sh_rows, sh_by_filter, viewmat_host, K_host, campos_host, width, height, degree, eps2d,
                                   radii, packed_grad, g_xyz, g_opacity, g_scaling, g_rotation, g_sh_rows, max_radii2D,
                                   grad_accum, denom, v_means2d_out, stats_only_visible, partials, row_cum, sh_index,
                                   sh_stamp, cur_step);
}
```

clm_gs_amd/fused.py:

```python
import ctypes
import math

import numpy as np
import torch

from . import _lib, utils
from ._lib import check, dptr
from .cameras import (camera_colour, camera_invdepth, camera_loss_mask, camera_pose_grad, camera_sky, check_sky_background,
                      refuse_ortho)
from .clm_kernels import COLOUR, check_depth_prior_args, check_sky, masked_loss_value, sky_acc_add, sky_backward, sky_forward
from .gsplat import _record_counts, bucket_size, empty_bucketed, isect_begin, isect_counts, isect_finish

F32, I32, U8, U16 = torch.float32, torch.int32, torch.uint8, torch.uint16
TILE = 16


def _partial_line_floats():
    global _PART_FLOATS
    if _PART_FLOATS is None:
        _PART_FLOATS = int(_lib.lib().clmgs_rasterize_partials_bytes(1)) // 4
    return _PART_FLOATS


_PART_FLOATS = None


def _cam_host(camera):
    refuse_ortho(camera, "the fused front end (fused.camera_front)")
    h = getattr(camera, "_clmgs_host", None)
    if h is None:
        vm = camera.world_view_transform.detach().t().contiguous().cpu().numpy().astype(np.float32)
        K = camera.K.detach().cpu().numpy().astype(np.float32) if getattr(camera, "K", None) is not None \
            else camera.create_k_on_gpu().cpu().numpy().astype(np.float32)
        c2w = getattr(camera, "camtoworlds", None)
        if c2w is not None:
            campos = c2w.detach().reshape(-1, 4, 4)[0, :3, 3].cpu().numpy().astype(np.float32)
        else:
            campos = np.linalg.inv(vm.astype(np.float64))[:3, 3].astype(np.float32)
        h = (np.ascontiguousarray(vm.reshape(16)), np.ascontiguousarray(K.reshape(9)),
             np.ascontiguousarray(campos.reshape(3)))
        camera._clmgs_host = h
    return h


def _np(a):
    return a.ctypes.data_as(ctypes.c_void_p)


class _CameraPass:
    __slots__ = ("V", "cam", "filt", "sh_rows", "sh_by_filter", "small_in", "small_packed", "radii",
                 "packed", "fids", "offsets", "emit_slot", "row_cum", "out", "alphas", "last_ids",
                 "bg", "v_out", "maps", "loss", "ev_loss", "streams", "deg", "aux", "loss_partials",
                 "lambda_dssim", "gt_u8", "background", "isect", "sh_index", "means2d", "n_dev", "antialiased",
                 "loss_mask", "mask_count", "colour", "colour_partials",
                 "invdepth", "depth_weight", "depths", "id_partials", "id_term", "pose_grad",
                 "sky", "v_alphas", "sky_scratch")


def _sptr(torch_stream):
    return ctypes.c_void_p(torch_stream.cuda_stream)


_CAPACITY = {}
_CAP_HELD = {}
_CAP_IDS = __import__("itertools").count(1)


def _cap_key(gaussians, W, H):
    k = getattr(gaussians, "_clmgs_cap_id", None)
    if k is None:
        k = gaussians._clmgs_cap_id = next(_CAP_IDS)
    return (int(W), int(H), k)


def _observe_count(key, n):
    _CAPACITY[key] = max(int(n), int(0.98 * _CAPACITY.get(key, 0)))


def _capacity_for(key, args):
    seen = _CAPACITY.get(key)
    if not seen or not getattr(args, "device_side_counts", True):
        return None
    margin = float(getattr(args, "isect_capacity_margin", 1.25))
    floor = int(getattr(args, "isect_capacity_floor", 4096))
    held = _CAP_HELD.get(key)
    if held is not None and margin > 1.0 and int(seen * 1.10) + floor <= held <= int(seen * margin * 1.5) + floor:
        return held
    cap = int(seen * margin) + floor
    cap = bucket_size(cap) if cap > 4096 else max(cap, 1)
    _CAP_HELD[key] = cap
    return cap


def camera_forward(gaussians, camera, this_filter, sh_rows, sh_by_filter, background, gt_u8,
                   lambda_dssim=0.2, small_packed=None, streams=None, sh_index=None, exact=True):
    return camera_forward_finish(gaussians, camera_front(
        gaussians, camera, this_filter, sh_rows, sh_by_filter, background, gt_u8, lambda_dssim,
        small_packed, streams, sh_index), exact=exact)


def camera_front(gaussians, camera, this_filter, sh_rows, sh_by_filter, background, gt_u8,
                 lambda_dssim=0.2, small_packed=None, streams=None, sh_index=None):
    L = _lib.lib()
    args = utils.get_args()
    W, H = int(utils.get_img_width()), int(utils.get_img_height())
    dev = gaussians._xyz.device
    cur = torch.cuda.current_stream()
    s_front, s_mem, s_raster = streams if streams is not None else (cur, cur, cur)
    p = _CameraPass()
    p.streams = (s_front, s_mem, s_raster)
    V = p.V = int(this_filter.shape[0]) if this_filter is not None else int(gaussians._xyz.shape[0])
    p.cam = _cam_host(camera)
    vm, K, campos = p.cam
    deg = p.deg = int(gaussians.active_sh_degree)
    p.sh_rows, p.sh_by_filter, p.small_packed = sh_rows, sh_by_filter, small_packed
    p.sh_index = sh_index
    p.gt_u8, p.lambda_dssim, p.background = gt_u8, float(lambda_dssim), background
    p.loss_mask, p.mask_count = camera_loss_mask(camera)
    p.colour, p.colour_partials = camera_colour(camera), None
    p.invdepth = camera_invdepth(camera) if check_depth_prior_args(camera) else None
    p.depth_weight, p.id_partials, p.id_term, p.depths = 0.0, None, None, None
    if p.invdepth is not None:
        raw = p.invdepth[0]
        if tuple(raw.shape) != (H, W) or raw.dtype != U16:
            raise _lib.ClmgsError(f"camera.invdepth must be uint16 [{H}, {W}], got {raw.dtype} {tuple(raw.shape)}")
        p.depth_weight = utils.depth_l1_weight()
    p.pose_grad = camera_pose_grad(camera)
    if p.pose_grad is not None:
        if p.invdepth is not None:
            raise ValueError("a camera carries both a pose-gradient buffer and an inverse-depth prior: pose refinement is not "
                             "supported with the depth regularisation")
        if tuple(p.pose_grad.shape) != (15,) or p.pose_grad.dtype != F32 or not p.pose_grad.is_contiguous():
            raise _lib.ClmgsError(f"camera.pose_grad must be contiguous float32 [15], got {p.pose_grad.dtype} "
                                  f"{tuple(p.pose_grad.shape)}")
        if sh_index is not None or not sh_rows.is_cuda:
            raise ValueError("pose refinement needs the SH rows in HBM (sh_residency=\"hbm\")")
    p.sky, p.v_alphas, p.sky_scratch = camera_sky(camera), None, None
    if p.sky is not None:
        check_sky(p.sky[0], "camera.sky")
        check_sky_background(background)
    p.antialiased = utils.antialiased()
    filt = p.filt = this_filter.contiguous() if this_filter is not None else None
    if small_packed is not None:
        small_in = (dptr(small_packed, F32), None, None, None)
        p.aux = (small_packed,)
    else:
        xyz, opa = gaussians._xyz.detach(), gaussians._opacity.detach()
        sca, rot = gaussians._scaling.detach(), gaussians._rotation.detach()
        small_in = (dptr(xyz, F32), dptr(opa, F32), dptr(sca, F32), dptr(rot, F32))
        p.aux = (xyz, opa, sca, rot)
    p.small_in = small_in
    tw, th = math.ceil(W / float(TILE)), math.ceil(H / float(TILE))
    with torch.cuda.stream(s_front):
        radii = p.radii = empty_bucketed(V, (), I32, dev).reshape(1, V)
        means2d = empty_bucketed(V, (2,), F32, dev).reshape(1, V, 2)
        depths = empty_bucketed(V, (), F32, dev).reshape(1, V)
        packed = p.packed = empty_bucketed(V, (16,), F32, dev)
        check((L.clmgs_preprocess_aa_fwd if p.antialiased else L.clmgs_preprocess_fwd)(
            _sptr(s_front), V, dptr(filt, torch.int64, True), *small_in,
            dptr(sh_rows, F32, allow_host=True), int(sh_by_filter), _np(vm), _np(K), _np(campos), W, H, deg,
            0.3, 0.01, 1e10, float(getattr(args, "radius_clip", 0.0)), dptr(radii), dptr(means2d),
            dptr(depths), None, None, None, dptr(packed),
            dptr(sh_index, I32, True)))
        if p.invdepth is not None:
            check(L.clmgs_invdepth_pack(_sptr(s_front), V, dptr(radii), dptr(depths), dptr(packed)))
            p.depths = depths
        p.isect = isect_begin("tile" if getattr(args, "binning", "tile") == "tile" else "sort", means2d, radii, depths, TILE,
                              tw, th, want_slots=True, packed=packed if getattr(args, "exact_tile_cull", True) else None)
        p.aux = p.aux + (means2d, depths)
        p.means2d = means2d
    return p


def camera_forward_finish(gaussians, p, exact=False):
    L = _lib.lib()
    args = utils.get_args()
    W, H = int(utils.get_img_width()), int(utils.get_img_height())
    dev = gaussians._xyz.device
    s_front, s_mem, s_raster = p.streams
    V, packed, background, gt_u8, lambda_dssim = p.V, p.packed, p.background, p.gt_u8, p.lambda_dssim
    tw, th = math.ceil(W / float(TILE)), math.ceil(H / float(TILE))
    cap = None if (exact or V == 0) else _capacity_for(_cap_key(gaussians, W, H), args)
    with torch.cuda.stream(s_front):
        with _lib.host_region("fwd_isect"):
            p.fids, p.offsets, _, (p.emit_slot, p.row_cum) = isect_finish(p.isect, capacity=cap)
        if cap is None:
            p.isect, p.n_dev = None, None
            if V:
                _observe_count(_cap_key(gaussians, W, H), p.fids.numel())
        else:
            p.n_dev = p.isect.totals
        nch = 4 if p.invdepth is not None else 3
        p.out = torch.empty((H, W, nch), dtype=F32, device=dev)
        p.alphas = torch.empty((H, W), dtype=F32, device=dev)
        p.last_ids = torch.empty((H, W), dtype=I32, device=dev)
        p.bg = background.reshape(1, 3).to(F32).contiguous() if background is not None and p.sky is None else None
        if nch == 4 and p.bg is not None:
            p.bg = torch.cat([p.bg, p.bg.new_zeros((1, 1))], dim=1).contiguous()
    if s_raster is not s_front:
        s_raster.wait_stream(s_front)
    n_isects = p.fids.numel()
    raster_fwd, raster_fwd_dev = (L.clmgs_rasterize4_fwd, L.clmgs_rasterize4_fwd_dev) if nch == 4 else \
        (L.clmgs_rasterize_fwd, L.clmgs_rasterize_fwd_dev)
    if p.n_dev is None:
        check(raster_fwd(_sptr(s_raster), 1, V, n_isects, None, None, None, None, dptr(p.bg, F32, True),
                         W, H, TILE, tw, th, dptr(p.offsets), dptr(p.fids), dptr(packed), dptr(p.out),
                         dptr(p.alphas), dptr(p.last_ids)))
    else:
        check(raster_fwd_dev(_sptr(s_raster), 1, V, n_isects, dptr(p.n_dev), dptr(p.bg, F32, True),
                             W, H, TILE, tw, th, dptr(p.offsets), dptr(p.fids), dptr(packed), dptr(p.out),
                             dptr(p.alphas), dptr(p.last_ids)))
    if s_mem is not s_raster:
        ev = torch.cuda.Event()
        ev.record(s_raster)
        s_mem.wait_event(ev)
    with torch.cuda.stream(s_mem):
        slots = L.clmgs_loss_slots()
        partials = torch.zeros((slots, 2), dtype=F32, device=dev)
        maps = p.maps = torch.empty((3, 3, H, W), dtype=F32, device=dev)
        sc, sy, sx = 1, nch * W, nch
        gt = gt_u8.contiguous()
        sm = _sptr(s_mem)
        mask = p.loss_mask
        if p.sky is not None:
            sky_forward(sm, H, W, dptr(p.out), (sc, sy, sx), p.alphas, p.cam[0], p.cam[1], p.sky[0],
                        dptr(p.out), (sc, sy, sx))
        img = p.out
        if p.colour is not None:
            kind, param, _ = p.colour
            COLOUR[kind].check(param, f"camera.{kind}")
            img = torch.empty_like(p.out)
            COLOUR[kind].forward(sm, H, W, dptr(p.out), (sc, sy, sx), param, dptr(img), (sc, sy, sx))
        if mask is None:
            check(L.clmgs_l1_ssim_loss_fwd(sm, H, W, dptr(img), sc, sy, sx, dptr(gt, U8), dptr(partials),
                                           dptr(maps[0]), dptr(maps[1]), dptr(maps[2])))
        else:
            if tuple(mask.shape) != (H, W):
                raise _lib.ClmgsError(f"loss_mask is {tuple(mask.shape)}, the image is {(H, W)}")
            check(L.clmgs_l1_ssim_loss_masked_fwd(sm, H, W, dptr(img), sc, sy, sx, dptr(gt, U8), dptr(partials),
                                                  dptr(maps[0]), dptr(maps[1]), dptr(maps[2]), dptr(mask, U8)))
        p.loss_partials, p.loss = partials, None
        one = getattr(gaussians, "_clmgs_one", None)
        if one is None or one.device != dev:
            one = gaussians._clmgs_one = torch.ones((1,), dtype=F32, device=dev)
        p.v_out = torch.empty_like(p.out)
        if mask is None:
            check(L.clmgs_l1_ssim_loss_bwd(sm, H, W, dptr(img), sc, sy, sx, dptr(gt, U8), dptr(one),
                                           float(lambda_dssim), dptr(maps[0]), dptr(maps[1]), dptr(maps[2]),
                                           dptr(p.v_out)))
        else:
            check(L.clmgs_l1_ssim_loss_masked_bwd(sm, H, W, dptr(img), sc, sy, sx, dptr(gt, U8), dptr(one),
                                                  float(lambda_dssim), dptr(maps[0]), dptr(maps[1]), dptr(maps[2]),
                                                  dptr(p.v_out), dptr(mask, U8)))
        if p.colour is not None:
            kind, param, _ = p.colour
            p.colour_partials = COLOUR[kind].backward(sm, H, W, dptr(p.out), (sc, sy, sx), param, dptr(p.v_out), (sc, sy, sx),
                                                      dptr(p.v_out), (sc, sy, sx), dev)
        p.v_alphas, p.sky_scratch = None, None
        if p.sky is not None and p.sky[1] is not None:
            p.v_alphas = torch.empty((H, W), dtype=F32, device=dev)
            p.sky_scratch = torch.zeros(p.sky[0].shape, dtype=torch.int64, device=dev)
            sky_backward(sm, H, W, dptr(p.v_out), (sc, sy, sx), p.alphas, p.cam[0], p.cam[1], p.sky[0], p.v_alphas,
                         p.sky_scratch)
        if p.invdepth is not None:
            raw, scale, offset = p.invdepth
            p.id_partials = torch.empty((int(L.clmgs_invdepth_partials_rows(H, W)),), dtype=F32, device=dev)
            p.id_term = None
            ch3 = 3 * p.out.element_size()
            check(L.clmgs_invdepth_l1_fwd_bwd(sm, H, W, ctypes.c_void_p(p.out.data_ptr() + ch3), 4 * W, 4, dptr(raw, U16),
                                              scale, offset, dptr(mask, U8, True), p.depth_weight,
                                              ctypes.c_void_p(p.v_out.data_ptr() + ch3), 4 * W, 4, dptr(p.id_partials)))
        p.ev_loss = None
        if s_raster is not s_mem:
            p.ev_loss = torch.cuda.Event()
            p.ev_loss.record(s_mem)
        p.aux = p.aux + (gt, one, partials) + ((mask,) if mask is not None else ())
        p.maps = None
        del maps, img
    return p


def camera_loss(p):
    if p.loss is None:
        W, H = int(utils.get_img_width()), int(utils.get_img_height())
        if p.loss_mask is None:
            tot = p.loss_partials.sum(dim=0) / float(3 * H * W)
            p.loss = ((1.0 - p.lambda_dssim) * tot[0] + p.lambda_dssim * (1.0 - tot[1])).detach()
        else:
            tot = p.loss_partials.sum(dim=0)
            p.loss = masked_loss_value(tot[0], tot[1], p.lambda_dssim, p.mask_count, H, W).detach()
        if p.id_partials is not None:
            L = _lib.lib()
            total = torch.empty((1,), dtype=F32, device=p.id_partials.device)
            check(L.clmgs_invdepth_finish(_lib.stream(), int(p.id_partials.numel()), dptr(p.id_partials), dptr(total)))
            p.id_term = (total[0] * (p.depth_weight / float(H * W))).detach()
            p.loss = p.loss + p.id_term
    return p.loss


def camera_verify(gaussians, p):
    c = p.isect
    if c is None or p.n_dev is None:
        return
    W, H = int(utils.get_img_width()), int(utils.get_img_height())
    n, n_ref = isect_counts(c)
    _observe_count(_cap_key(gaussians, W, H), n)
    if n <= p.fids.numel():
        _record_counts(n, n_ref)
        p.isect = None
        return
    _lib.STATS["isect_capacity_redo"] = _lib.STATS.get("isect_capacity_redo", 0) + 1
    for st in set(p.streams):
        st.synchronize()
    p.n_dev = None
    camera_forward_finish(gaussians, p, exact=True)


def camera_backward(gaussians, p, g_sh_rows, small_grad=None, update_stats=True, stats_delta=None,
                    stats_only_visible=False, visibility_out=None, accumulate_after=None, sh_stamp=None,
                    cur_step=0, release=False):
    L = _lib.lib()
    args = utils.get_args()
    W, H = int(utils.get_img_width()), int(utils.get_img_height())
    dev = gaussians._xyz.device
    camera_verify(gaussians, p)
    s_front, s_mem, s_raster = p.streams
    if p.colour_partials is not None:
        kind, param, grad = p.colour
        if grad is not None:
            COLOUR[kind].finish(_sptr(s_mem), H, W, param, p.colour_partials, grad)
        p.colour_partials = None
    if p.sky_scratch is not None:
        with torch.cuda.stream(s_mem):
            sky_acc_add(_sptr(s_mem), p.sky_scratch, p.sky[1])
        p.sky_scratch = None
    V = p.V
    vm, K, campos = p.cam
    tw, th = math.ceil(W / float(TILE)), math.ceil(H / float(TILE))
    n_isects = p.fids.numel()
    if p.small_packed is not None:
        assert small_grad is not None
        small_out = (dptr(small_grad, F32), None, None, None)
    else:
        small_out = (dptr(gaussians._xyz.grad, F32), dptr(gaussians._opacity.grad, F32),
                     dptr(gaussians._scaling.grad, F32), dptr(gaussians._rotation.grad, F32))
    with torch.cuda.stream(s_raster):
        partials = empty_bucketed(max(n_isects, 1), (_partial_line_floats(),), F32, dev)
    if p.ev_loss is not None:
        s_raster.wait_event(p.ev_loss)
    absgrad = bool(getattr(args, "absgrad", False))
    raster_bwd, raster_bwd_dev = (L.clmgs_rasterize_abs_bwd, L.clmgs_rasterize_abs_bwd_dev) if absgrad else \
        (L.clmgs_rasterize_bwd, L.clmgs_rasterize_bwd_dev)
    if p.invdepth is not None:
        assert not absgrad
        raster_bwd, raster_bwd_dev = L.clmgs_rasterize4_slot_bwd, L.clmgs_rasterize4_bwd_dev
    if p.n_dev is None:
        check(raster_bwd(_sptr(s_raster), 1, V, n_isects, dptr(p.packed), dptr(p.bg, F32, True), W, H,
                         TILE, tw, th, dptr(p.offsets), dptr(p.fids), dptr(p.alphas), dptr(p.last_ids),
                         dptr(p.v_out), dptr(p.v_alphas, F32, True), None, None, None, None, None,
                         dptr(p.emit_slot), dptr(p.row_cum), dptr(partials), *((None,) if absgrad else ())))
    else:
        check(raster_bwd_dev(_sptr(s_raster), 1, V, n_isects, dptr(p.n_dev), dptr(p.packed),
                             dptr(p.bg, F32, True), W, H, TILE, tw, th, dptr(p.offsets), dptr(p.fids),
                             dptr(p.alphas), dptr(p.last_ids), dptr(p.v_out), dptr(p.v_alphas, F32, True),
                             dptr(p.emit_slot), dptr(p.row_cum), dptr(partials)))
    if s_mem is not s_raster:
        ev = torch.cuda.Event()
        ev.record(s_raster)
        s_mem.wait_event(ev)
    stats = update_stats and (not args.disable_auto_densification) and \
        utils.get_cur_iter() <= args.densify_until_iter
    if stats and stats_delta is not None:
        stat_ptrs = (dptr(stats_delta, F32), None, None)
    else:
        stat_ptrs = (dptr(gaussians.max_radii2D if stats else None, F32, True),
                     dptr(gaussians.xyz_gradient_accum if stats else None, F32, True),
                     dptr(gaussians.denom if stats else None, F32, True))
    with torch.cuda.stream(s_mem):
        if accumulate_after is not None:
            s_mem.wait_event(accumulate_after)
        if visibility_out is not None:
            visibility_out |= (p.radii.reshape(-1) > 0)
        if p.antialiased:
            pre_bwd = L.clmgs_preprocess_aa_abs_bwd if absgrad else L.clmgs_preprocess_aa_bwd
        else:
            pre_bwd = L.clmgs_preprocess_abs_bwd if absgrad else L.clmgs_preprocess_bwd
        check(pre_bwd(
            _sptr(s_mem), V, dptr(p.filt, torch.int64, True), *p.small_in, dptr(p.sh_rows, F32, allow_host=True),
            int(p.sh_by_filter), _np(vm), _np(K), _np(campos), W, H, p.deg, 0.3, dptr(p.radii),
            None, *small_out, dptr(g_sh_rows, F32, allow_host=True),
            *stat_ptrs, None, int(bool(stats_only_visible)), dptr(partials), dptr(p.row_cum),
            dptr(p.sh_index, I32, True), dptr(sh_stamp, I32, True), int(cur_step), *((None,) if absgrad else ())))
        if p.pose_grad is not None:
            pose_rows = torch.empty((int(L.clmgs_pose_grad_partials_rows(V)), 16), dtype=F32, device=dev)
            check(L.clmgs_pose_grad(
                _sptr(s_mem), V, dptr(p.filt, torch.int64, True), *p.small_in, dptr(p.sh_rows, F32),
                int(p.sh_by_filter), _np(vm), _np(K), _np(campos), W, H, p.deg, 0.3, dptr(p.radii), None,
                dptr(partials), dptr(p.row_cum), None, int(bool(p.antialiased)), dptr(pose_rows)))
            check(L.clmgs_pose_grad_finish(_sptr(s_mem), int(pose_rows.shape[0]), dptr(pose_rows), dptr(p.pose_grad, F32)))
            del pose_rows
        if p.invdepth is not None:
            check(L.clmgs_invdepth_rows_bwd(_sptr(s_mem), V, dptr(p.filt, torch.int64, True), dptr(p.radii),
                                            dptr(p.depths), _np(vm), dptr(partials), dptr(p.row_cum), None,
                                            small_out[0], 1 if p.small_packed is not None else 0))
    if s_mem is not s_raster:
        partials.record_stream(s_mem)
        p.v_out.record_stream(s_raster)
        if p.v_alphas is not None:
            p.v_alphas.record_stream(s_raster)
    del partials
    p.v_out, p.v_alphas = None, None
    if release:
        for name in ("radii", "packed", "fids", "offsets", "emit_slot", "row_cum", "out", "alphas", "last_ids", "n_dev",
                     "depths"):
            t = getattr(p, name)
            if t is not None:
                for st in {s_mem, s_raster} - {s_front}:
                    t.record_stream(st)
                setattr(p, name, None)
        for t in p.aux:
            if isinstance(t, torch.Tensor) and t.is_cuda and t is not p.loss_partials:
                for st in {s_mem, s_raster} - {s_front}:
                    t.record_stream(st)
        p.aux = (p.loss_partials,)
        p.means2d = None
    return p


def train_one_camera(gaussians, camera, this_filter, sh_rows, sh_by_filter, g_sh_rows, background,
                     gt_u8, lambda_dssim=0.2, update_stats=True, keep=None, accumulate_after=None,
                     return_event=False, stats_only_visible=False, visibility_out=None,
                     raster_stream=None, small_packed=None, small_grad=None, stats_delta=None, sh_index=None,
                     sh_stamp=None, cur_step=0):
    cur = torch.cuda.current_stream()
    p = camera_forward(gaussians, camera, this_filter, sh_rows, sh_by_filter, background, gt_u8,
                       lambda_dssim, small_packed, (cur, cur, raster_stream if raster_stream is not None else cur),
                       sh_index, exact=False)
    camera_backward(gaussians, p, g_sh_rows, small_grad, update_stats, stats_delta,
                    stats_only_visible, visibility_out, accumulate_after, sh_stamp, cur_step)
    loss = camera_loss(p)
    if keep is not None:
        keep.append(p)
    if return_event:
        ev = torch.cuda.Event()
        ev.record(cur)
        return loss, ev
    return loss
```

clm_gs_amd/strategies/clm_offload/engine.py:

```python
import os

import torch

from ... import _lib, clm_kernels, dp, fast_tsp, mcmc, utils
from ...clm_kernels import (apply_camera_colour, check_depth_prior_args,
                            send_shs2cpu_grad_buffer_stream, send_shs2gpu_stream, spherical_harmonics_bwd_inplace)
from ...densification import check_mcmc_args, update_densification_stats_offload_accum_grads
from ...host import pinned_empty
from ..base_engine import (select_filters, select_filter_words, calculate_filters, camera_forward_ops,
                           camera_loss_backward, pipeline_forward_one_step)

_BITMAP_DTYPE = {4: torch.int8, 8: torch.int8, 16: torch.int16, 32: torch.int32, 64: torch.int64}


def pipeline_forward_one_step_shs_inplace(filtered_opacity_gpu, filtered_scaling_gpu,
                                          filtered_rotation_gpu, filtered_xyz_gpu, filtered_shs,
                                          camera, scene, gaussians, background, pipe_args, render_mode="RGB"):
    image, means2D, radiis, depth_alpha, sh_leaf = camera_forward_ops(
        filtered_xyz_gpu, filtered_rotation_gpu, filtered_scaling_gpu, filtered_opacity_gpu,
        filtered_shs.reshape(1, filtered_xyz_gpu.shape[0], 16, 3), gaussians.active_sh_degree,
        camera.world_view_transform.transpose(0, 1), camera.K, camera.camtoworlds[:, None, :3, 3],
        background.reshape(1, 3) if background is not None else None, render_mode, train=True, sh_autograd=False,
        sky_camera=camera)
    return (image, means2D, radiis) + sh_leaf + depth_alpha[:1]
# ... 164 lines not shown
    total = sum(int(nb) for _, nb in plan.values())
    shrink = 1.0 if not free_now or total <= free_now / 3 else (free_now / 3) / total
    for name, (st, nbytes) in plan.items():
        nbytes = int(nbytes * shrink)
        if nbytes < (1 << 20):
            out[name] = 0
            continue
        try:
            with torch.cuda.stream(st):
                blk = torch.empty((nbytes,), dtype=torch.uint8, device=gaussians._xyz.device)
                small = [torch.empty((1 << 19,), dtype=torch.uint8, device=gaussians._xyz.device) for _ in range(16)]
                del blk, small
            out[name] = nbytes
        except torch.cuda.OutOfMemoryError:
            torch.cuda.empty_cache()
            out[name] = 0
    return out


class _Batch:
    """State of one HBM-resident batch, handed from stage to stage (see _train_one_batch_hbm)."""


def _host_camera_mats(cams, device):
    import numpy as np
    C = len(cams)
    h = torch.from_numpy(np.concatenate([c._clmgs_host[0] for c in cams] + [c._clmgs_host[1] for c in cams])
                         .astype(np.float32, copy=False)).pin_memory()
    d = h.to(device, non_blocking=True)
    return d[:16 * C].view(C, 4, 4), d[16 * C:].view(C, 3, 3)


def _head_record(b):
    sd = b.gaussians._small_def
    if b.head_overlap and b.head_words is not None and b.head_event is not None and sd["hist"] \
            and sd["hist"][-1][0] == b.step and sd["blk_last"] is b.head_blk_last:
        mask = 0
        for c in b.ordered_cams[-b.head_depth:]:
            mask |= 1 << int(c)
        sd["head"] = {"event": b.head_event, "words": b.head_words, "last": int(b.ordered_cams[-1]), "mask": mask,
                      "mutations": b.gaussians._mutations, "step": b.step, "n": b.N}


def _stage_visibility(b):
    gaussians, args, cams = b.gaussians, b.args, b.cameras
    N = b.N
    b.touched = b.touched_rows = None
    b.small_owner = bool(getattr(gaussians, "small_owner", False) and gaussians.lazy_rows and dp.active()
                         and not args.stop_update_param)
    if b.small_owner:
        with torch.no_grad(), _lib.host_region("dp_small_fetch"), dp.phase("S"):
            gaussians.small_prepare(cams)
    b.small_deferred = bool(getattr(gaussians, "small_deferred", False) and b.fused and gaussians.lazy_rows
                            and not args.stop_update_param and getattr(args, "packed_small", True))
    blk_flags = None
    sd = getattr(gaussians, "_small_def", None)
    rec = sd.pop("head", None) if sd else None
    b.head_words = b.head_event = None
    b.head_overlap = bool(b.small_deferred and getattr(args, "head_overlap", True) and b.bsz >= 2 and not dp.active()
                          and getattr(args, "overlap_cameras", True) in (True, "pipeline")
                          and not getattr(args, "pose_opt", False) and sd["hist"]
                          and all(getattr(c, "_clmgs_host", None) is not None for c in cams))
    b.head_depth = max(1, min(int(getattr(args, "head_overlap_cameras", 2)), b.bsz - 1))
    sel = temp = None
    if b.small_deferred:
        with torch.no_grad():
            if b.head_overlap:
                b.head_words = gaussians.small_head_words()
                if (rec is not None and rec["mutations"] == getattr(gaussians, "_mutations", 0)
                        and rec["step"] == sd["hist"][-1][0] and rec["n"] == N and rec["words"].shape == b.head_words.shape):
                    sel = (rec["words"], rec["mask"])
                    s_front = _pipeline_streams(gaussians)["mem"][0]
                    s_front.wait_event(rec["event"])
                    with torch.cuda.stream(s_front):
                        mats = _host_camera_mats(cams, gaussians._xyz.device)
                        flags0 = gaussians.small_catch_up(cams, cam_words=b.head_words, sel=sel + (0,), cam_mats=mats)
                        temp = select_filter_words(cams, gaussians._xyz.detach(), gaussians._scaling.detach(),
                                                   gaussians._rotation.detach(), mats, flags0, sel + (0,))
                    torch.cuda.current_stream().wait_stream(s_front)
                    _lib.STATS["head_overlap_split"] = _lib.STATS.get("head_overlap_split", 0) + 1
            blk_flags = gaussians.small_catch_up(cams, cam_words=b.head_words, sel=sel + (1,) if sel else None)
            b.head_blk_last = sd["blk_last"]
    with torch.no_grad():
        if b.fused:
            with _lib.host_region("select_filters"):
                b.filters, b.touched_rows = select_filters(cams, gaussians._xyz.detach(), gaussians._scaling.detach(),
                                                           gaussians._rotation.detach(), block_flags=blk_flags,
                                                           block_sel=sel + (1,) if sel else None, temp=temp)
        else:
            b.filters, _, _ = calculate_filters(cams, gaussians.get_xyz, gaussians.get_opacity,
                                                gaussians.get_scaling, gaussians.get_rotation)
    if b.small_owner and os.environ.get("CLMGS_DP_DEBUG") and b.touched_rows is not None:
        lo_, hi_ = dp.owner_range(N)
        foreign = b.touched_rows[(b.touched_rows < lo_) | (b.touched_rows >= hi_)]
        cand_ = getattr(gaussians, "_dbg_cand", None)
        miss = -1
        if cand_ is not None and gaussians._small_since > 0:
            isc = torch.zeros((N,), dtype=torch.bool, device=foreign.device)
            isc[cand_] = True
            miss = int((~isc[foreign]).sum())
        print("DPDEBUG batch rank %d since %d foreign touched rows %d not candidates %d" % (
            dp.rank(), gaussians._small_since, foreign.numel(), miss), flush=True)
        assert miss <= 0
    b.sparsity = [len(f) / float(N) for f in b.filters]
    b.ordered_cams = list(range(b.bsz))
    if getattr(args, "reference_camera_order", False):
        _, b.cameras, b.filters, b.sparsity, b.ordered_cams = order_calculation(
            list(b.filters), list(cams), N, b.bsz, None, args)[:5]


def _stage_plan(b):
    gaussians, args, N, bsz = b.gaussians, b.args, b.N, b.bsz
    b.lazy = gaussians.lazy_rows and not args.stop_update_param
    mode = getattr(args, "overlap_cameras", True)
    b.pipelined = b.fused and mode in (True, "pipeline")
    b.use_packed = (b.fused and getattr(args, "packed_small", True) and not args.sparse_adam
                    and not args.stop_update_param)
    b.locality = bool(b.lazy and dp.active() and getattr(args, "dp_locality", False))
    b.locality_sparse = bool(dp.active() and getattr(args, "dp_locality", False) and args.sparse_adam and b.fused
                             and not args.stop_update_param and not b.lazy)
    if getattr(args, "dp_locality", False) and dp.active():
        assert b.touched_rows is not None and (b.locality_sparse or (b.locality and b.use_packed and gaussians.first_touch_grads)), (
            "dp_locality needs the fused front end and either the dense deferred row optimizer with the packed "
            "small-attribute tables and first-touch gradient stores (defaults) or sparse_adam")
    need_mask = b.touched_rows is None or args.sparse_adam or (dp.active() and not b.locality) or not b.lazy
    if need_mask:
        b.touched = torch.zeros((N,), dtype=torch.bool, device=gaussians._xyz.device)
        if b.touched_rows is not None:
            utils.fill_rows(b.touched, b.touched_rows, True)
        else:
            for f in b.filters:
                utils.fill_rows(b.touched, f, True)
        if dp.active() and not b.locality_sparse:
            b.local_touched = b.touched
            b.touched = dp.allreduce_touched(b.touched)
            b.touched_rows = None
    b.row_adam = gaussians.optimizer.cpu_adam
    b.params = gaussians._parameters
    b.grad_buf = b.parameters_grad_buffer[:N]
    b.params.grad = b.grad_buf
    b.row_adam.global_step += 1
    b.step = b.row_adam.global_step
    _mark_batch(gaussians)
    b.group = b.row_adam.param_groups[0]
    b.st = b.row_adam.state[b.params]
    b.default_stream = torch.cuda.current_stream()
    b.side_event = None
    b.col_lr = b.row_adam._col_lr(b.params.device)
    if b.touched_rows is None:
        b.touched_rows = torch.nonzero(b.touched).flatten()
    b.touched_rows = b.touched_rows.to(torch.int32)
    _lib.STATS.setdefault("touched_rows", []).append(int(b.touched_rows.shape[0]))
    b.ft_stamp = gaussians._row_g_step if (b.lazy and b.fused and gaussians.first_touch_grads) else None


def _mark_batch(gaussians):
    gaussians._lazy_dirty = True
    gaussians._mutations = getattr(gaussians, "_mutations", 0) + 1
    gaussians._sorted_tag = None


def _row_update(b, rows, zero_grad_rows=False):
    clm_kernels.adam_rows(b.params.data, None if zero_grad_rows else b.grad_buf, b.st["exp_avg"],
                          b.st["exp_avg_sq"], rows, b.col_lr,
                          b.group["betas"][0], b.group["betas"][1], b.group["eps"], b.step,
                          b.group["bias_correction"], 1.0 / (b.bsz * dp.world_size()), True)


def _stage_exchange_head(b):
    gaussians, args, N, bsz, step = b.gaussians, b.args, b.N, b.bsz, b.step
    params, touched_rows = b.params, b.touched_rows
    b.owner = b.border = None
    b.split_catch = False
    b.dp_ev_b0 = b.dp_ev_b1 = b.dp_comm = None
    b.dp_split = False
    if b.locality:
        b.dp_split = bool(b.pipelined and bsz >= 2 and getattr(args, "dp_overlap", True))
        with _lib.host_region("dp_border_plan"), dp.phase("plan"):
            b.border = dp.border_plan(touched_rows.long(), N, first_rows=b.filters[0] if b.dp_split else None,
                                      last_rows=b.filters[bsz - 1] if b.dp_split else None,
                                      publish_counts=not b.small_owner)
        gaussians._owner_dirty = True
        own_rows = b.border.own_rows
        if own_rows.numel():
            with dp.phase("catch_up_own"):
                gaussians.catch_up_rows(own_rows.to(torch.int32), to_step=step - 1)
        if b.dp_split:
            b.dp_comm = getattr(gaussians, "_dp_comm_stream", None)
            if b.dp_comm is None:
                b.dp_comm = gaussians._dp_comm_stream = torch.cuda.Stream()
            b.dp_comm.wait_stream(b.default_stream)
            with torch.cuda.stream(b.dp_comm):
                with dp.phase("B0"):
                    dp.border_params_out(params.data, b.border, "params0")
                b.dp_ev_b0 = torch.cuda.Event()
                b.dp_ev_b0.record(b.dp_comm)
                with dp.phase("B1"):
                    dp.border_params_out(params.data, b.border, "params1")
                b.dp_ev_b1 = torch.cuda.Event()
                b.dp_ev_b1.record(b.dp_comm)
        else:
            with dp.phase("B"):
                dp.border_params_out(params.data, b.border)
    elif b.locality_sparse:
        with _lib.host_region("dp_border_plan"), dp.phase("plan"):
            b.border = dp.border_plan(touched_rows.long(), N)
        gaussians._owner_dirty = True
        with dp.phase("B"):
            dp.border_params_out(params.data, b.border)
    elif b.lazy and dp.active() and getattr(args, "dp_owner_computes", False):
        b.owner = dp.owner_plan(touched_rows.long(), N)
        gaussians._owner_dirty = True
        own_rows = touched_rows[b.owner.lo:b.owner.hi]
        if b.owner.hi > b.owner.lo:
            gaussians.catch_up_rows(own_rows, to_step=step - 1)
        dp.owner_gather_rows(params.data, b.owner)
    elif b.lazy:
        if (b.pipelined and bsz >= 2 and getattr(args, "split_catch_up", True) and b.filters is not None):
            b.foreign_rows = None
            if dp.active():
                lt = getattr(b, "local_touched", None)
                assert lt is not None
                b.foreign_rows = touched_rows[~lt[touched_rows.long()]]
            b.split_catch = True
            s_front = _pipeline_streams(gaussians)["mem"][0]
            s_front.wait_stream(b.default_stream)
            b.first_catch_done = bool(getattr(args, "early_first_catch_up", True))
            if b.first_catch_done and b.filters[0].numel():
                with torch.cuda.stream(s_front):
                    gaussians.catch_up_rows(b.filters[0], to_step=step - 1)
        else:
            gaussians.catch_up_rows(touched_rows, to_step=step - 1)
    elif not args.stop_update_param and not args.sparse_adam:
        untouched_rows = torch.nonzero(~b.touched).flatten().to(torch.int32)
        b.comm_stream.wait_stream(b.default_stream)
        with torch.cuda.stream(b.comm_stream):
            _row_update(b, untouched_rows, zero_grad_rows=True)
            b.side_event = torch.cuda.Event()
            b.side_event.record(b.comm_stream)
        untouched_rows.record_stream(b.comm_stream)


def _cameras_pipelined(b):
    from ...fused import camera_backward, camera_forward_finish, camera_front, camera_loss
    gaussians, bsz, step = b.gaussians, b.bsz, b.step
    sts = _pipeline_streams(gaussians)
    s_front, s_mem, s_raster = sts["mem"][0], sts["mem"][1], sts["raster"][0]
    if getattr(gaussians, "_clmgs_one", None) is None:
        gaussians._clmgs_one = torch.ones((1,), dtype=torch.float32, device=b.params.device)
    for st_ in (s_front, s_mem, s_raster):
        st_.wait_stream(b.default_stream)
    gaussians._clmgs_passes = None
    passes = []
    dp_recv0 = [None]

    def backward(k):
        with _lib.host_region("camera_backward"):
            camera_backward(gaussians, passes[k], b.grad_buf, b.small_gk, stats_delta=b.stats_d,
                            sh_stamp=b.ft_stamp, cur_step=step, release=True)
        if b.head_overlap and k == bsz - 1 - b.head_depth:
            b.head_event = torch.cuda.Event()
            b.head_event.record(s_mem)
        if b.dp_split and k == bsz - 2:
            ev = torch.cuda.Event()
            ev.record(s_mem)
            b.dp_comm.wait_event(ev)
            with torch.cuda.stream(b.dp_comm), dp.phase("D0"):
                dp_recv0[0] = dp.border_grads_send([b.grad_buf, b.small_gk], b.ft_stamp, step, b.border, "grads0")

    def catch(k):
        if b.filters[k].numel():
            with torch.cuda.stream(s_front):
                gaussians.catch_up_rows(b.filters[k], to_step=step - 1)
    for k in range(bsz):
        if b.dp_split:
            s_front.wait_event(b.dp_ev_b0 if k == 0 else b.dp_ev_b1)
        if b.split_catch and (k or not b.first_catch_done):
            catch(k)
        if b.split_catch and k == bsz - 1 and getattr(b, "foreign_rows", None) is not None and b.foreign_rows.numel():
            with torch.cuda.stream(s_front):
                gaussians.catch_up_rows(b.foreign_rows, to_step=step - 1)
        with _lib.host_region("camera_front"):
            cur_pass = camera_front(gaussians, b.cameras[k], b.filters[k], b.params.data, 1, b.background,
                                    b.cameras[k].original_image, small_packed=b.small_pk,
                                    streams=(s_front, s_mem, s_raster))
        with _lib.host_region("camera_forward"):
            passes.append(camera_forward_finish(gaussians, cur_pass))
        if k >= 1:
            backward(k - 1)
    backward(bsz - 1)
    if b.dp_split:
        b.default_stream.wait_stream(b.dp_comm)
        gaussians._dp_recv0 = dp_recv0[0]
    for st_ in (s_front, s_mem, s_raster):
        b.default_stream.wait_stream(st_)
    losses = [camera_loss(p_) for p_ in passes]
    gaussians._clmgs_passes = passes
    return losses


def _stage_cameras(b):
    gaussians, args, bsz = b.gaussians, b.args, b.bsz
    b.small_pk = b.small_gk = b.stats_d = None
    if b.use_packed:
        b.small_pk, b.small_gk = gaussians.small_packed(), gaussians.small_grad()
        if (getattr(args, "packed_stats", True) and (not args.disable_auto_densification)
                and utils.get_cur_iter() <= args.densify_until_iter):
            b.stats_d = gaussians.stats_delta()
    else:
        _zero_small_grads(gaussians)
    if b.pipelined:
        return _cameras_pipelined(b)
    losses = []
    if b.fused:
        from ...fused import train_one_camera
        for k in range(bsz):
            losses.append(train_one_camera(
                gaussians, b.cameras[k], b.filters[k], b.params.data, 1, b.grad_buf, b.background,
                b.cameras[k].original_image, small_packed=b.small_pk, small_grad=b.small_gk,
                stats_delta=b.stats_d, sh_stamp=b.ft_stamp, cur_step=b.step))
        return losses
    for k in range(bsz):
        this_filter = b.filters[k]
        with torch.no_grad():
            shs = torch.empty((this_filter.shape[0], 48), device=b.params.device)
            send_shs2gpu_stream(shs, b.params.data, this_filter)
            shs_grad = torch.zeros_like(shs)
        loss = _render_and_backward(gaussians, b.scene, b.cameras[k], b.background, b.pipe_args, this_filter, shs,
                                    shs_grad)
        with torch.no_grad():
            send_shs2cpu_grad_buffer_stream(shs_grad, b.grad_buf, this_filter, True)
        losses.append(loss)
    return losses


def _stage_exchange_tail(b):
    if not dp.active():
        return
    gaussians, N, step = b.gaussians, b.N, b.step
    grad_buf, small_gk, ft_stamp, border = b.grad_buf, b.small_gk, b.ft_stamp, b.border
    if border is not None and b.locality_sparse:
        small_grads = [gaussians._xyz.grad, gaussians._opacity.grad, gaussians._scaling.grad, gaussians._rotation.grad]
        dp.border_grads_home([grad_buf] + small_grads, None, 0, border)
        own_rows = border.own_rows
        _, got = dp.publish_rows(small_grads, own_rows, N, counts=border.own_counts)
        b.touched = torch.zeros((N,), dtype=torch.bool, device=b.params.device)
        for ids in [own_rows] + got:
            if ids.numel():
                utils.fill_rows(b.touched, ids, True)
        b.touched_rows = own_rows.to(torch.int32)
    elif border is not None:
        if b.dp_split:
            r0 = gaussians._dp_recv0
            gaussians._dp_recv0 = None
            for t_ in (r0[0], r0[1], r0[3]):
                if isinstance(t_, torch.Tensor) and t_.is_cuda:
                    t_.record_stream(b.default_stream)
            with dp.phase("D1"):
                r1 = dp.border_grads_send([grad_buf, small_gk], ft_stamp, step, border, "grads1")
            with dp.phase("D_apply"):
                dp.border_grads_apply([grad_buf, small_gk], ft_stamp, step, border, r0)
                dp.border_grads_apply([grad_buf, small_gk], ft_stamp, step, border, r1)
        else:
            with dp.phase("D"):
                dp.border_grads_home([grad_buf, small_gk], ft_stamp, step, border)
        if not b.small_owner:
            dp.publish_small(small_gk, ft_stamp, step, N, border)
    elif b.owner is not None:
        if b.use_packed:
            dp.allreduce_tables_rows([small_gk], b.touched_rows, N, average=False)
        else:
            dp.allreduce_small_grads([gaussians._xyz.grad, gaussians._opacity.grad,
                                      gaussians._scaling.grad, gaussians._rotation.grad], average=False)
        dp.owner_reduce_rows(grad_buf, b.owner)
    elif b.use_packed:
        with dp.phase("allreduce"):
            dp.allreduce_tables_rows([small_gk, grad_buf], b.touched_rows, N, average=False)
    else:
        dp.allreduce_small_grads([gaussians._xyz.grad, gaussians._opacity.grad,
                                  gaussians._scaling.grad, gaussians._rotation.grad], average=False)
        dp.allreduce_rows(grad_buf, b.touched, average=False, rows=b.touched_rows)


def _stage_optimizer(b):
    gaussians, args, N, bsz, step = b.gaussians, b.args, b.N, b.bsz, b.step
    if b.use_packed and b.small_deferred and b.ft_stamp is not None and not dp.active():
        gaussians.small_defer_record(step)
        _head_record(b)
    elif b.use_packed:
        if getattr(gaussians, "small_deferred", False):
            gaussians.flush_small()
        if mcmc.enabled(args):
            mcmc.add_reg_grads(gaussians, grad_div=bsz * dp.world_size(), packed=b.small_pk, packed_grad=b.small_gk)
        gaussians.optimizer.gpu_step_packed(b.small_pk, b.small_gk, 1.0 / (bsz * dp.world_size()),
                                            g_stamp=b.ft_stamp, cur_step=step,
                                            row_range=dp.owner_range(N) if (b.small_owner and b.locality) else None)
        if b.small_owner and b.locality:
            gaussians.small_after_step()
        if mcmc.enabled(args):
            mcmc.inject_noise(gaussians, packed=b.small_pk)
    else:
        if mcmc.enabled(args):
            mcmc.add_reg_grads(gaussians, grad_div=bsz * dp.world_size())
        _gpu_adam_step(gaussians, args, b.touched if args.sparse_adam else None,
                       grad_div=bsz * dp.world_size())
        if mcmc.enabled(args):
            mcmc.inject_noise(gaussians)
        gaussians.invalidate_small_packed()
    if b.lazy:
        stamp = b.touched_rows[b.owner.lo:b.owner.hi] if b.owner is not None else b.touched_rows
        if stamp.numel() and b.ft_stamp is None:
            utils.fill_rows(gaussians._row_g_step, stamp.long(), step)
    elif not args.stop_update_param:
        _row_update(b, b.touched_rows)
    b.st["step"] = step


def _train_one_batch_hbm(gaussians, scene, batched_cameras, parameters_grad_buffer, background,
                         pipe_args, comm_stream, args):
    b = _Batch()
    b.gaussians, b.scene, b.cameras, b.args = gaussians, scene, batched_cameras, args
    b.parameters_grad_buffer, b.background, b.pipe_args, b.comm_stream = parameters_grad_buffer, background, pipe_args, comm_stream
    b.bsz, b.N = len(batched_cameras), gaussians._xyz.shape[0]
    b.fused = bool(getattr(args, "fused_front_end", True))
    _stage_visibility(b)
    _stage_plan(b)
    _stage_exchange_head(b)
    losses = _stage_cameras(b)
    with dp.phase("tail_exchange"):
        _stage_exchange_tail(b)
    if getattr(args, "debug_skip_optimizer", False):
        b.row_adam.global_step -= 1
        if b.side_event is not None:
            b.default_stream.wait_event(b.side_event)
        return losses, b.ordered_cams, b.sparsity
    _stage_optimizer(b)
    if b.side_event is not None:
        b.default_stream.wait_event(b.side_event)
    if getattr(args, "sync_each_batch", False):
        torch.cuda.synchronize()
    return losses, b.ordered_cams, b.sparsity


def hint_next_batch(gaussians, cameras):
    gaussians._next_batch_hint = list(cameras) if cameras else None


def _train_one_batch_host(gaussians, scene, batched_cameras, parameters_grad_buffer, background,
                          pipe_args, comm_stream, perm_generator, args):
    if getattr(args, "host_staging", "window") == "window":
        from .host_window import train_one_batch_host_windowed as run
    else:
        from .host_batch import train_one_batch_host_batched as run
    return run(gaussians, scene, batched_cameras, parameters_grad_buffer, background, pipe_args, comm_stream,
               perm_generator, args)


def clm_offload_train_one_batch(gaussians, scene, batched_cameras, parameters_grad_buffer,
                                background, pipe_args, comm_stream, perm_generator):
    args = utils.get_args()
    bsz = len(batched_cameras)
    assert bsz > 1 and bsz in _BITMAP_DTYPE, "clm_offload supports bsz in (4, 8, 16, 32, 64)"
    assert bsz == args.bsz, f"batch of {bsz} cameras but args.bsz = {args.bsz} (optimizer hyper-parameters are scaled by args.bsz)"
    for camera in batched_cameras:
        check_depth_prior_args(camera)
    check_mcmc_args(args)
    if gaussians._parameters.is_cuda:
        with _lib.host_region("batch_total"):
            return _train_one_batch_hbm(gaussians, scene, batched_cameras, parameters_grad_buffer,
                                        background, pipe_args, comm_stream, args)
    return _train_one_batch_host(gaussians, scene, batched_cameras, parameters_grad_buffer,
                                 background, pipe_args, comm_stream, perm_generator, args)

# ... 30 lines not shown
```

clm_gs_amd/utils.py:

```python
import io
import time
from types import SimpleNamespace

import numpy as np
import torch

ARGS = None
LOG_FILE = None
CUR_ITER = 0
IMG_W = 0
IMG_H = 0
TIMERS = None
DENSIFY_ITER = 0


def default_args(**over):
    a = SimpleNamespace(
        no_offload=False, naive_offload=False, clm_offload=False, prealloc_capacity=-1,
        comm_stream_priority=-1, grid_size_H=32, grid_size_D=128,
        reorder_by_min_sparsity_at_end=True, sparse_adam=False, gpu=0, packed=False,
        sh_degree=3, radius_clip=0.0, white_background=False,
        iterations=30_000, position_lr_init=0.00016, position_lr_final=0.0000016,
        position_lr_delay_mult=0.01, position_lr_max_steps=30_000, feature_lr=0.0025,
        opacity_lr=0.05, scaling_lr=0.005, lr_scale_loss=1.0, lr_scale_pos_and_scale=1.0,
        rotation_lr=0.001, percent_dense=0.01, lambda_dssim=0.2, densification_interval=100,
        opacity_reset_interval=3000, densify_from_iter=500, densify_until_iter=15_000,
        densify_grad_threshold=0.0002, disable_auto_densification=False, min_opacity=0.005,
        absgrad=False,
        rasterize_mode="classic",
        exposure=False, exposure_lr_init=0.01, exposure_lr_final=0.001,
        bilagrid=False, bilagrid_shape=(16, 16, 8), bilagrid_lr_init=2e-3, bilagrid_lr_final=2e-5, bilagrid_tv_weight=10.0,
        sky=False, sky_shape=(256, 512), sky_init=(0.5, 0.5, 0.5), sky_lr_init=0.01, sky_lr_final=0.001,
        depths="", depth_l1_weight_init=1.0, depth_l1_weight_final=0.01,
        mcmc=False, mcmc_cap_max=1_000_000, mcmc_noise_lr=5e5, mcmc_refine_start_iter=500, mcmc_refine_stop_iter=25_000,
        mcmc_refine_every=100, mcmc_min_opacity=0.005, mcmc_opacity_reg=0.01, mcmc_scale_reg=0.01,
        pose_opt=False, pose_opt_lr=1e-5, pose_opt_reg=1e-6, pose_noise=0.0, defer_pose_step=True,
        contrib_prune_iterations=(), contrib_prune_mode="sum", contrib_prune_ratio=0.3, contrib_prune_threshold=0.01,
        num_downscales=0, resolution_schedule=3000,
        undistort=False, undistort_zoom=1.0,
        compress=False, compress_codebook=65536, compress_iters=10, compress_sample=1 << 22, compress_pos_bits=16,
        compress_scale_bits=8, compress_opacity_bits=8, compress_rot_bits=8, compress_dc_bits=8,
        mesh_voxel=0.0, mesh_trunc_voxels=4.0, mesh_min_weight=2.0, mesh_every=1, mesh_grid_gb=16.0, mesh_depth_mode=None,
        mesh_min_component_faces=0, mesh_keep_components=0, mesh_sparse=False, mesh_decimate_cell=0.0,
        lr_scale_mode="sqrt", bsz=1, exact_filter=True, log_cpu_adam_trailing_overhead=False,
        stop_update_param=False, drop_initial_3dgs_p=0.0,
        debug_skip_optimizer=False,
        sh_residency="hbm",
        fused_front_end=True,
        overlap_cameras=True,
        packed_small=True, packed_stats=True, exact_tile_cull=True,
        sync_each_batch=False,
        dp_overlap=True,
        dp_shard_moments=True,
        dp_small_owner=True,
        dp_small_refresh=8,
        dp_small_max_log_gain=0.7,
        binning="tile",
        deferred_small_adam=True,
        allocator_reservoir=True,
        split_catch_up=True,
        early_first_catch_up=True,
        head_overlap=True,
        head_overlap_cameras=2,
        warm_structural_ops=True,
        defer_loss_log=True,
        spatial_row_order=True,
        first_touch_grads=True,
        host_staging="window",
        placement_candidates=1,
        sh_hbm_budget_gb=0.0,
        host_speculative_prefetch=True,
        device_side_counts=True,
        isect_capacity_margin=1.25,
        isect_capacity_floor=4096,
        reference_camera_order=False,
        dp_locality=False,
        dp_owner_computes=False,
        lazy_dense_adam=True,
    )
    for k, v in over.items():
        setattr(a, k, v)
    return a


RASTERIZE_MODES = ("classic", "antialiased")


def antialiased():
    mode = getattr(ARGS, "rasterize_mode", "classic")
    if mode not in RASTERIZE_MODES:
        raise ValueError(f"rasterize_mode must be one of {RASTERIZE_MODES}, got {mode!r}")
    return mode == "antialiased"


def depth_l1_weight(iteration=None):
    a = get_args()
    it = get_cur_iter() if iteration is None else iteration
    return float(get_expon_lr_func(float(getattr(a, "depth_l1_weight_init", 1.0)),
                                   float(getattr(a, "depth_l1_weight_final", 0.01)),
                                   max_steps=int(getattr(a, "iterations", 30_000)))(int(it)))


class _NullLog(io.StringIO):
    def write(self, s):
        return len(s)


class Timers:
    def __init__(self):
        self.t = {}
        self.acc = {}

    def start(self, k):
        self.t[k] = time.perf_counter()

    def stop(self, k):
        if k in self.t:
            self.acc[k] = self.acc.get(k, 0.0) + time.perf_counter() - self.t.pop(k)


def set_args(a):
    global ARGS
    ARGS = a


def get_args():
    global ARGS
    if ARGS is None:
        ARGS = default_args()
    return ARGS


def set_log_file(f):
    global LOG_FILE
    LOG_FILE = f


def get_log_file():
    global LOG_FILE
    if LOG_FILE is None:
        LOG_FILE = _NullLog()
    return LOG_FILE


def set_cur_iter(i):
    global CUR_ITER
    CUR_ITER = i


def get_cur_iter():
    return CUR_ITER


def set_img_size(h, w):
    global IMG_H, IMG_W
    IMG_H, IMG_W = int(h), int(w)


def get_img_width():
    return IMG_W


def get_img_height():
    return IMG_H


def get_timers():
    global TIMERS
    if TIMERS is None:
        TIMERS = Timers()
    return TIMERS


def inc_densify_iter():
    global DENSIFY_ITER
    DENSIFY_ITER += 1


def check_update_at_this_iter(iteration, bsz, update_interval, update_residual):
    lo = iteration % update_interval
    hi = lo + bsz
    return (lo <= update_residual < hi) or (lo <= update_residual + update_interval < hi)


def inverse_sigmoid(x):
    return torch.log(x / (1 - x))


def get_expon_lr_func(lr_init, lr_final, lr_delay_steps=0, lr_delay_mult=1.0, max_steps=1000000):

    def helper(step):
        if step < 0 or (lr_init == 0.0 and lr_final == 0.0):
            return 0.0
        if lr_delay_steps > 0:
            delay = lr_delay_mult + (1 - lr_delay_mult) * np.sin(0.5 * np.pi * np.clip(step / lr_delay_steps, 0, 1))
        else:
            delay = 1.0
        t = np.clip(step / max_steps, 0, 1)
        return delay * np.exp(np.log(lr_init) * (1 - t) + np.log(lr_final) * t)

    return helper


def build_rotation(r):
    q = r / r.norm(dim=1, keepdim=True)
    w, x, y, z = q.unbind(1)
    R = torch.stack([
        1 - 2 * (y * y + z * z), 2 * (x * y - w * z), 2 * (x * z + w * y),
        2 * (x * y + w * z), 1 - 2 * (x * x + z * z), 2 * (y * z - w * x),
        2 * (x * z - w * y), 2 * (y * z + w * x), 1 - 2 * (x * x + y * y)], dim=1)
    return R.reshape(-1, 3, 3)


SH_C0 = 0.28209479177387814


def RGB2SH(rgb):
    return (rgb - 0.5) / SH_C0


# ... 77 lines not shown
```

include/clmgs.h:

```cpp
#ifndef CLMGS_H
#define CLMGS_H
#include <stddef.h>
#include <stdint.h>

#ifdef __cplusplus
extern "C" {
#endif

#define CLMGS_EINVAL 10001
#define CLMGS_ENOMEM 10002

int clmgs_version(void);
const char* clmgs_last_error(void);

int clmgs_projection_fwd(void* stream, int C, int N, const float* means, const float* quats,
                         const float* scales, const float* viewmats, const float* Ks, int width,
                         int height, float eps2d, float near_plane, float far_plane,
                         float radius_clip, int32_t* radii, float* means2d, float* depths,
                         float* conics);
int clmgs_visibility_raw(void* stream, int C, int N, const float* means, const float* quats_raw,
                         const float* log_scales, const float* viewmats, const float* Ks, int width,
                         int height, float eps2d, float near_plane, float far_plane,
                         float radius_clip, int32_t* radii);

// ... 102 lines not shown
                           const float* conics, const float* opacities, const float* depths, int width, int height,
                           int tile_size, int tile_width, int tile_height, const int32_t* offsets,
                           const int32_t* flatten_ids, void* packed, float* median_depth, int32_t* median_id);

int clmgs_ray_depth(void* stream, int C, int N, int height, int width, const float* means, const float* quats,
                    const float* scales, const double* cams, const int32_t* median_id, const float* median_depth,
                    double near_plane, int camera_model, float* ray_depth);

int clmgs_rasterize4_fwd(void* stream, int C, int N, int64_t n_isects, const float* means2d,
                         const float* conics, const float* colors, const float* opacities,
                         const float* backgrounds, int width, int height, int tile_size,
                         int tile_width, int tile_height, const int32_t* offsets,
                         const int32_t* flatten_ids, void* packed, float* render_colors,
                         float* render_alphas, int32_t* last_ids);
int clmgs_rasterize4_bwd(void* stream, int C, int N, int64_t n_isects, const void* packed,
                         const float* backgrounds, int width, int height, int tile_size,
                         int tile_width, int tile_height, const int32_t* offsets,
                         const int32_t* flatten_ids, const float* render_alphas,
                         const int32_t* last_ids, const float* v_render_colors,
                         const float* v_render_alphas, void* packed_grad, float* v_means2d,
                         float* v_conics, float* v_colors, float* v_opacities,
                         const int32_t* emit_slot, const int64_t* row_cum, void* partials);
int clmgs_rasterize4_slot_bwd(void* stream, int C, int N, int64_t n_isects, const void* packed,
                              const float* backgrounds, int width, int height, int tile_size,
                              int tile_width, int tile_height, const int32_t* offsets,
                              const int32_t* flatten_ids, const float* render_alphas,
                              const int32_t* last_ids, const float* v_render_colors,
                              const float* v_render_alphas, void* packed_grad, float* v_means2d,
                              float* v_conics, float* v_colors, float* v_opacities,
                              const int32_t* emit_slot, const int64_t* row_cum, void* partials);

int clmgs_rasterize_abs_bwd(void* stream, int C, int N, int64_t n_isects, const void* packed,
                            const float* backgrounds, int width, int height, int tile_size,
                            int tile_width, int tile_height, const int32_t* offsets,
                            const int32_t* flatten_ids, const float* render_alphas,
                            const int32_t* last_ids, const float* v_render_colors,
                            const float* v_render_alphas, void* packed_grad, float* v_means2d,
                            float* v_conics, float* v_colors, float* v_opacities,
                            const int32_t* emit_slot, const int64_t* row_cum, void* partials,
                            float* v_means2d_abs);

int clmgs_isect2_emit_sort_dev(void* stream, int V, int64_t capacity, const int64_t* n_isects_dev,
                               const float* depths, const int32_t* order, const int64_t* cum,
                               const uint64_t* boxes, int tile_width, int tile_height,
                               int32_t* flatten_ids, int32_t* offsets, int64_t* isect_ids,
                               int32_t* emit_slot, void* temp, size_t temp_bytes, const int64_t* row_cum);

size_t clmgs_isect3_front_temp_bytes(int V, int n_tiles);
int clmgs_isect3_front(void* stream, int V, const float* means2d, const int32_t* radii, int tile_size, int tile_width,
                       int tile_height, const void* packed, int64_t* totals, int64_t* row_cum, void* temp,
                       size_t temp_bytes);
size_t clmgs_isect3_bin_temp_bytes(int64_t n_isects, int n_tiles);
int clmgs_isect3_bin(void* stream, int V, int64_t n_isects, const float* depths, int tile_width, int tile_height,
                     const int64_t* row_cum, const void* front_temp, int32_t* flatten_ids, int32_t* offsets,
                     int64_t* isect_ids, int32_t* emit_slot, void* temp, size_t temp_bytes);
int clmgs_isect3_bin_dev(void* stream, int V, int64_t capacity, const int64_t* n_isects_dev, const float* depths,
                         int tile_width, int tile_height, const int64_t* row_cum, const void* front_temp,
                         int32_t* flatten_ids, int32_t* offsets, int64_t* isect_ids, int32_t* emit_slot, void* temp,
                         size_t temp_bytes);
int clmgs_rasterize_fwd_dev(void* stream, int C, int N, int64_t capacity, const int64_t* n_isects_dev,
                            const float* backgrounds, int width, int height, int tile_size,
                            int tile_width, int tile_height, const int32_t* offsets,
                            const int32_t* flatten_ids, void* packed, float* render_colors,
                            float* render_alphas, int32_t* last_ids);
int clmgs_rasterize_bwd_dev(void* stream, int C, int N, int64_t capacity, const int64_t* n_isects_dev,
                            const void* packed, const float* backgrounds, int width, int height,
                            int tile_size, int tile_width, int tile_height, const int32_t* offsets,
                            const int32_t* flatten_ids, const float* render_alphas,
                            const int32_t* last_ids, const float* v_render_colors,
                            const float* v_render_alphas, const int32_t* emit_slot,
                            const int64_t* row_cum, void* partials);

int clmgs_rasterize4_fwd_dev(void* stream, int C, int N, int64_t capacity, const int64_t* n_isects_dev,
                             const float* backgrounds, int width, int height, int tile_size,
                             int tile_width, int tile_height, const int32_t* offsets,
                             const int32_t* flatten_ids, void* packed, float* render_colors,
                             float* render_alphas, int32_t* last_ids);
int clmgs_rasterize4_bwd_dev(void* stream, int C, int N, int64_t capacity, const int64_t* n_isects_dev,
                             const void* packed, const float* backgrounds, int width, int height,
                             int tile_size, int tile_width, int tile_height, const int32_t* offsets,
                             const int32_t* flatten_ids, const float* render_alphas,
                             const int32_t* last_ids, const float* v_render_colors,
                             const float* v_render_alphas, const int32_t* emit_slot,
                             const int64_t* row_cum, void* partials);

int clmgs_rasterize_abs_bwd_dev(void* stream, int C, int N, int64_t capacity, const int64_t* n_isects_dev,
                                const void* packed, const float* backgrounds, int width, int height,
                                int tile_size, int tile_width, int tile_height, const int32_t* offsets,
                                const int32_t* flatten_ids, const float* render_alphas,
                                const int32_t* last_ids, const float* v_render_colors,
                                const float* v_render_alphas, const int32_t* emit_slot,
                                const int64_t* row_cum, void* partials);

int clmgs_preprocess_grid_cap(void);
int clmgs_preprocess_fwd(void* stream, int V, const int64_t* filter, const float* xyz,
                         const float* opacity_raw, const float* scaling_raw,
                         const float* rotation_raw, const float* sh_rows, int sh_by_filter,
                         const float* viewmat_host, const float* K_host, const float* campos_host,
                         int width, int height, int degree, float eps2d, float near_plane,
                         float far_plane, float radius_clip, int32_t* radii, float* means2d,
                         float* depths, float* conics, float* colors, float* opacities, void* packed,
                         const int32_t* sh_index);
int clmgs_preprocess_bwd(void* stream, int V, const int64_t* filter, const float* xyz,
                         const float* opacity_raw, const float* scaling_raw,
                         const float* rotation_raw, const float* sh_rows, int sh_by_filter,
                         const float* viewmat_host, const float* K_host, const float* campos_host,
                         int width, int height, int degree, float eps2d, const int32_t* radii,
                         const void* packed_grad, float* g_xyz, float* g_opacity, float* g_scaling,
                         float* g_rotation, float* g_sh_rows, float* max_radii2D, float* grad_accum,
                         float* denom, float* v_means2d_out, int stats_only_visible,
                         const void* partials, const int64_t* row_cum, const int32_t* sh_index,
                         int32_t* sh_stamp, int cur_step);

int clmgs_preprocess_abs_bwd(void* stream, int V, const int64_t* filter, const float* xyz,
                             const float* opacity_raw, const float* scaling_raw,
                             const float* rotation_raw, const float* sh_rows, int sh_by_filter,
                             const float* viewmat_host, const float* K_host, const float* campos_host,
                             int width, int height, int degree, float eps2d, const int32_t* radii,
                             const void* packed_grad, float* g_xyz, float* g_opacity, float* g_scaling,
                             float* g_rotation, float* g_sh_rows, float* max_radii2D, float* grad_accum,
                             float* denom, float* v_means2d_out, int stats_only_visible,
                             const void* partials, const int64_t* row_cum, const int32_t* sh_index,
                             int32_t* sh_stamp, int cur_step, float* v_means2d_abs_out);

int clmgs_preprocess_aa_fwd(void* stream, int V, const int64_t* filter, const float* xyz,
                            const float* opacity_raw, const float* scaling_raw,
                            const float* rotation_raw, const float* sh_rows, int sh_by_filter,
                            const float* viewmat_host, const float* K_host, const float* campos_host,
                            int width, int height, int degree, float eps2d, float near_plane,
                            float far_plane, float radius_clip, int32_t* radii, float* means2d,
                            float* depths, float* conics, float* colors, float* opacities, void* packed,
                            const int32_t* sh_index);
int clmgs_preprocess_aa_bwd(void* stream, int V, const int64_t* filter, const float* xyz,
                            const float* opacity_raw, const float* scaling_raw,
                            const float* rotation_raw, const float* sh_rows, int sh_by_filter,
                            const float* viewmat_host, const float* K_host, const float* campos_host,
                            int width, int height, int degree, float eps2d, const int32_t* radii,
                            const void* packed_grad, float* g_xyz, float* g_opacity, float* g_scaling,
                            float* g_rotation, float* g_sh_rows, float* max_radii2D, float* grad_accum,
                            float* denom, float* v_means2d_out, int stats_only_visible,
                            const void* partials, const int64_t* row_cum, const int32_t* sh_index,
                            int32_t* sh_stamp, int cur_step);
int clmgs_preprocess_aa_abs_bwd(void* stream, int V, const int64_t* filter, const float* xyz,
                                const float* opacity_raw, const float* scaling_raw,
                                const float* rotation_raw, const float* sh_rows, int sh_by_filter,
                                const float* viewmat_host, const float* K_host, const float* campos_host,
                                int width, int height, int degree, float eps2d, const int32_t* radii,
                                const void* packed_grad, float* g_xyz, float* g_opacity, float* g_scaling,
                                float* g_rotation, float* g_sh_rows, float* max_radii2D, float* grad_accum,
                                float* denom, float* v_means2d_out, int stats_only_visible,
                                const void* partials, const int64_t* row_cum, const int32_t* sh_index,
                                int32_t* sh_stamp, int cur_step, float* v_means2d_abs_out);

int clmgs_ssim_fwd(void* stream, int B, int CH, int H, int W, const float* img1,
                   const float* img2, float* ssim_sum, float* dm_dmu1, float* dm_dsigma1_sq,
                   float* dm_dsigma12);
int clmgs_ssim_bwd(void* stream, int B, int CH, int H, int W, const float* img1,
                   const float* img2, const float* v_mean, float inv_numel, const float* dm_dmu1,
                   const float* dm_dsigma1_sq, const float* dm_dsigma12, float* v_img1);

int clmgs_loss_slots(void);
int clmgs_l1_ssim_loss_fwd(void* stream, int H, int W, const float* img, int64_t stride_c,
                           int64_t stride_y, int64_t stride_x, const uint8_t* gt_u8,
                           float* partials, float* m1, float* m2, float* m3);
int clmgs_l1_ssim_loss_bwd(void* stream, int H, int W, const float* img, int64_t stride_c,
                           int64_t stride_y, int64_t stride_x, const uint8_t* gt_u8,
                           const float* v_loss, float lambda_dssim, const float* m1,
                           const float* m2, const float* m3, float* v_img);
int clmgs_l1_ssim_loss_masked_fwd(void* stream, int H, int W, const float* img, int64_t stride_c,
                                  int64_t stride_y, int64_t stride_x, const uint8_t* gt_u8,
                                  float* partials, float* m1, float* m2, float* m3,
                                  const uint8_t* mask);
int clmgs_l1_ssim_loss_masked_bwd(void* stream, int H, int W, const float* img, int64_t stride_c,
                                  int64_t stride_y, int64_t stride_x, const uint8_t* gt_u8,
                                  const float* v_loss, float lambda_dssim, const float* m1,
                                  const float* m2, const float* m3, float* v_img,
                                  const uint8_t* mask);

int clmgs_exposure_partials_rows(int H, int W);
int clmgs_exposure_fwd(void* stream, int H, int W, const float* x, int64_t stride_c, int64_t stride_y,
                       int64_t stride_x, const float* E_dev, float* y, int64_t ystride_c, int64_t ystride_y,
                       int64_t ystride_x);
int clmgs_exposure_bwd(void* stream, int H, int W, const float* x, int64_t stride_c, int64_t stride_y,
                       int64_t stride_x, const float* E_dev, const float* g, int64_t gstride_c,
                       int64_t gstride_y, int64_t gstride_x, float* v_x, int64_t vstride_c, int64_t vstride_y,
                       int64_t vstride_x, float* partials);
int clmgs_exposure_grad_finish(void* stream, int rows, const float* partials, float* grad12);

int clmgs_sky_fwd(void* stream, int H, int W, const float* x, int64_t stride_c, int64_t stride_y, int64_t stride_x,
                  const float* alphas, const float* viewmat_host, const float* K_host, const float* sky, int Hs,
                  int Ws, float* y, int64_t ystride_c, int64_t ystride_y, int64_t ystride_x);
int clmgs_sky_bwd(void* stream, int H, int W, const float* g, int64_t gstride_c, int64_t gstride_y, int64_t gstride_x,
                  const float* alphas, const float* viewmat_host, const float* K_host, const float* sky, int Hs,
                  int Ws, float* v_alphas, int64_t* acc);
int clmgs_sky_acc_add(void* stream, int64_t n, const int64_t* src, int64_t* dst);
int clmgs_sky_grad_convert(void* stream, int64_t n, int64_t* acc, float* grad);

int clmgs_invdepth_partials_rows(int H, int W);
int clmgs_invdepth_pack(void* stream, int V, const int32_t* radii, const float* depths, void* packed);
int clmgs_invdepth_l1_fwd_bwd(void* stream, int H, int W, const float* I, int64_t stride_y, int64_t stride_x,
                              const uint16_t* prior_u16, float scale, float offset, const uint8_t* mask,
                              float weight, float* v_I, int64_t vstride_y, int64_t vstride_x, float* partials);
int clmgs_invdepth_finish(void* stream, int rows, const float* partials, float* sum_out);
int clmgs_invdepth_rows_bwd(void* stream, int V, const int64_t* filter, const int32_t* radii, const float* depths,
                            const float* viewmat, const void* partials, const int64_t* row_cum,
                            const void* packed_grad, float* g_xyz, int packed_grads);

int clmgs_mcmc_relocation(void* stream, int64_t n, const float* opacities, const float* scales, const int32_t* ratios,
                          float* new_opacities, float* new_scales);
int clmgs_mcmc_reg_grad(void* stream, int64_t n, const float* opacity_raw, int64_t opacity_stride,
                        const float* scaling_raw, int64_t scaling_stride, float* g_opacity, int64_t g_opacity_stride,
                        float* g_scaling, int64_t g_scaling_stride, float c_o, float c_s);
int clmgs_mcmc_noise(void* stream, int64_t n, float* xyz, const float* opacity_raw, const float* scaling_raw,
                     const float* rotation_raw, const float* noise, float scaler, float* packed_mirror);

int clmgs_bilagrid_partials_rows(int H, int W, int Hg, int Wg);
int clmgs_bilagrid_fwd(void* stream, int H, int W, const float* x, int64_t stride_c, int64_t stride_y,
                       int64_t stride_x, const float* grid_dev, int L, int Hg, int Wg, float* y, int64_t ystride_c,
                       int64_t ystride_y, int64_t ystride_x);
int clmgs_bilagrid_bwd(void* stream, int H, int W, const float* x, int64_t stride_c, int64_t stride_y,
                       int64_t stride_x, const float* grid_dev, int L, int Hg, int Wg, const float* g,
                       int64_t gstride_c, int64_t gstride_y, int64_t gstride_x, float* v_x, int64_t vstride_c,
                       int64_t vstride_y, int64_t vstride_x, float* partials);
int clmgs_bilagrid_grad_finish(void* stream, int H, int W, int L, int Hg, int Wg, const float* partials, float* grad);
int clmgs_bilagrid_tv_grad(void* stream, const float* table, int64_t n, int L, int Hg, int Wg, float weight,
                           float* grad);

int clmgs_pose_grad_partials_rows(int V);
int clmgs_pose_grad(void* stream, int V, const int64_t* filter, const float* xyz, const float* opacity_raw,
                    const float* scaling_raw, const float* rotation_raw, const float* sh_rows, int sh_by_filter,
                    const float* viewmat_host, const float* K_host, const float* campos_host, int width, int height,
                    int degree, float eps2d, const int32_t* radii, const void* packed_grad, const void* partials,
                    const int64_t* row_cum, const int32_t* sh_index, int antialiased, float* partials_out);
int clmgs_pose_grad_finish(void* stream, int rows, const float* partials, float* grad15);
int clmgs_projection_viewmat_partials_rows(int N);
int clmgs_projection_viewmat_bwd(void* stream, int C, int N, const float* means, const float* quats,
                                 const float* scales, const float* viewmats, const float* Ks, int width, int height,
                                 float eps2d, const int32_t* radii, const float* v_means2d, const float* v_depths,
                                 const float* v_conics, const float* v_compensations, float* partials,
                                 float* v_viewmats);

int clmgs_rows_gather(void* stream, float* dst, const float* src, const void* dst_idx,
                      const void* src_idx, int idx_is_64, int64_t n_rows, int cols,
                      int grid_blocks);
int clmgs_rows_scatter_add(void* stream, float* dst, const float* src, const void* dst_idx,
                           const void* src_idx, int idx_is_64, int64_t n_rows, int cols,
                           int grid_blocks);

int clmgs_scatter_to_bit(void* stream, void* bitmap, int elem_bytes, const int64_t* filter,
                         int64_t n, int bit);
int clmgs_extract_ffs(void* stream, const void* bitmap, int elem_bytes, int64_t N, uint8_t* ffs);
int clmgs_pair_overlap_count(void* stream, const void* bitmap, int elem_bytes, int64_t N,
                             int bsz, int32_t* cnt);
int clmgs_set_signal(void* stream, int32_t* signal_pinned, int idx, int32_t value);

int clmgs_adam_rows(void* stream, float* p, float* g, float* m, float* v, const void* rows,
                    int idx_is_64, const uint8_t* mask, int64_t n_rows, int cols,
                    const float* col_lr, double beta1, double beta2, double eps, int step,
                    int bias_correction, float grad_scale, int zero_grad);
int clmgs_pack_small(void* stream, int64_t n, const float* xyz, const float* opacity,
                     const float* scaling, const float* rotation, void* packed_p);
int clmgs_adam_small_packed(void* stream, int64_t n, float* const* params, float* const* exp_avg,
                            float* const* exp_avg_sq, const double* lr4, void* packed_p,
                            void* packed_g, double beta1, double beta2, double eps, int step,
                            int bias_correction, float grad_scale, const int32_t* g_stamp, int cur_step);
int clmgs_adam_catch_up(void* stream, float* p, float* m, float* v, const int32_t* last_step,
                        const void* rows, int idx_is_64, int64_t n_rows, int cols,
                        const float* col_lr, double beta1, double beta2, double eps, int to_step,
                        int bias_correction, int max_replay, float* g, const int32_t* g_step,
                        float grad_scale, int keep_grad);
int clmgs_host_adam_rows(float* p, float* g, float* m, float* v, const int32_t* rows,
                         int64_t n_rows, int cols, const float* col_lr, double beta1,
                         double beta2, double eps, int step, int bias_correction, float grad_scale,
                         int zero_grad, const volatile int32_t* signal, int n_threads);

int clmgs_host_pool_start(int n_threads);
int clmgs_host_usable_cpus(void);
int clmgs_memcpy_async(void* stream, void* dst, const void* src, size_t bytes, int kind);
int clmgs_host_rows_prepare(float* p, const float* g, float* m, float* v, int32_t* last_step,
                            int32_t* g_step, const int32_t* rows, int64_t n_rows, int cols,
                            const float* col_lr, double beta1, double beta2, double eps, int to_step,
                            int next_g_step, int bias_correction, float grad_scale, int max_replay,
                            float* stage, int sparse);

int clmgs_densify_stats(void* stream, int64_t n, const int64_t* filter, const float* v_means2d,
                        const int32_t* radii, int only_visible, float half_w, float half_h,
                        float* max_radii2D,
                        float* xyz_gradient_accum, float* denom);

size_t clmgs_morton_order_temp_bytes(int64_t n);
int clmgs_morton_order(void* stream, int64_t n, const float* xyz, const double* lo_hi, int64_t* order, void* temp,
                       size_t temp_bytes);

int clmgs_tsp_tour(int n, const int64_t* dist, int32_t* tour);

int clmgs_knn3_mean_dist2(void* stream, int n, const float* pts_sorted, const int32_t* cell_start,
                          float ox, float oy, float oz, float h, int gx, int gy, int gz,
                          int max_ring, float* mean_d2_sorted);

size_t clmgs_host_groups_temp_bytes(int64_t n);
int clmgs_host_groups(void* stream, int64_t n, const int64_t* touched, const void* bitmap, int elem_bytes, int bsz,
                      const uint8_t* staged, int slot0, int32_t* late_sorted, int32_t* rows_by_last, int32_t* slot_of,
                      int64_t* counts, void* temp, size_t temp_bytes);

int clmgs_publish_pack(void* stream, float* msg, const float* table, const int64_t* own_rows, const int32_t* stamp,
                       int step, int64_t lo, int64_t n_rows, int64_t chunk, int cols);
// ... 93 lines not shown
```

Measured before the change: 194.8.

## Fuse lazy Adam catch-up of SH rows into preprocess forward kernel

Adds a STEP variant of the preprocess forward kernel that, for rows whose optimizer state lags the current step, replays pending Adam updates (including a waiting gradient) on the SH rows before projecting and shading them. The separate catch-up pass over the batch's touched rows is skipped when this path is active. The aim is to avoid an extra kernel pass and re-reading of SH parameter rows. In exchange the fused kernel loads moments and grads, uses lower occupancy (launch bounds 2 instead of 3), and writes parameters in place during the forward.

```diff
diff --git a/clm_gs_amd/_lib.py b/clm_gs_amd/_lib.py
--- a/clm_gs_amd/_lib.py
+++ b/clm_gs_amd/_lib.py
@@ -68,6 +68,8 @@
     "clmgs_preprocess_aa_fwd": (_i, [_vp, _i, _vp, _vp, _vp, _vp, _vp, _vp, _i, _vp, _vp, _vp, _i, _i, _i, _f, _f, _f, _f, _vp, _vp, _vp, _vp, _vp, _vp, _vp, _vp]),
     "clmgs_preprocess_aa_bwd": (_i, [_vp, _i, _vp, _vp, _vp, _vp, _vp, _vp, _i, _vp, _vp, _vp, _i, _i, _i, _f, _vp, _vp, _vp, _vp, _vp, _vp, _vp, _vp, _vp, _vp, _vp, _i, _vp, _vp, _vp, _vp, _i]),
     "clmgs_preprocess_aa_abs_bwd": (_i, [_vp, _i, _vp, _vp, _vp, _vp, _vp, _vp, _i, _vp, _vp, _vp, _i, _i, _i, _f, _vp, _vp, _vp, _vp, _vp, _vp, _vp, _vp, _vp, _vp, _vp, _i, _vp, _vp, _vp, _vp, _i, _vp]),
+    "clmgs_preprocess_fwd_step": (_i, [_vp, _i, _vp, _vp, _vp, _vp, _vp, _vp, _i, _vp, _vp, _vp, _i, _i, _i, _f, _f, _f, _f, _vp, _vp, _vp, _vp, _vp, _vp, _vp, _vp,
+                                       _i, _vp, _vp, _vp, _vp, _vp, _vp, _d, _d, _d, _i, _i, _i, _f]),
     "clmgs_ssim_fwd": (_i, [_vp, _i, _i, _i, _i, _vp, _vp, _vp, _vp, _vp, _vp]),
     "clmgs_ssim_bwd": (_i, [_vp, _i, _i, _i, _i, _vp, _vp, _vp, _f, _vp, _vp, _vp, _vp]),
     "clmgs_loss_slots": (_i, []),
diff --git a/clm_gs_amd/csrc/adam_step.h b/clm_gs_amd/csrc/adam_step.h
--- /dev/null
+++ b/clm_gs_amd/csrc/adam_step.h
@@ -0,0 +1,98 @@
+#pragma once
+#include "common.h"
+
+namespace clmgs {
+
+__device__ __forceinline__ float adam_update(float p, float m, float v, float lr_bc, float inv_sqrt_bc2, float eps) {
+#pragma clang fp contract(off)
+  const float ratio = m * __builtin_amdgcn_rcpf(__builtin_fmaf(__builtin_amdgcn_sqrtf(v), inv_sqrt_bc2, eps));
+  return __builtin_fmaf(-lr_bc, ratio, p);
+}
+
+template <bool GRAD_FUSED = false>
+__device__ __forceinline__ float adam_elem(float& m, float& v, float p, float g, float lr_bc, float beta1,
+                                           float beta2, float ob1, float ob2, float eps,
+                                           float inv_sqrt_bc2) {
+#pragma clang fp contract(off)
+  if constexpr (GRAD_FUSED) {
+    m = __builtin_fmaf(ob1, g, beta1 * m);
+    v = __builtin_fmaf(ob2 * g, g, beta2 * v);
+  } else {
+    m = __builtin_fmaf(beta1, m, ob1 * g);
+    v = __builtin_fmaf(beta2, v, (ob2 * g) * g);
+  }
+  return adam_update(p, m, v, lr_bc, inv_sqrt_bc2, eps);
+}
+
+__device__ __forceinline__ float adam_elem_nograd(float& m, float& v, float p, float lr_bc, float beta1, float beta2,
+                                                  float eps, float inv_sqrt_bc2) {
+#pragma clang fp contract(off)
+  m = beta1 * m;
+  v = beta2 * v;
+  return adam_update(p, m, v, lr_bc, inv_sqrt_bc2, eps);
+}
+
+__device__ __forceinline__ float pow_beta(float beta, float x) {
+  return __builtin_amdgcn_exp2f(x * __builtin_amdgcn_logf(beta));
+}
+
+struct CatchUpK {
+  float beta1, beta2, ob1, ob2, eps, grad_scale;
+  int bias_correction, max_replay;
+};
+
+__device__ __forceinline__ void adam_bias(const CatchUpK& K, float pw1, float pw2, float& inv_bc1, float& inv_sqrt_bc2) {
+#pragma clang fp contract(off)
+  inv_bc1 = inv_sqrt_bc2 = 1.f;
+  if (K.bias_correction) {
+    inv_bc1 = 1.f / (1.f - pw1);
+    inv_sqrt_bc2 = 1.f / sqrtf(1.f - pw2);
+  }
+}
+
+template <int VEC>
+__device__ __forceinline__ void adam_replay(const CatchUpK& K, int from, int to, float (&pp)[VEC], float (&mm)[VEC],
+                                            float (&vv)[VEC], const float (&lr)[VEC]) {
+#pragma clang fp contract(off)
+  const int missed = to - from;
+  if (missed <= 0) return;
+  const int n = min(missed, K.max_replay);
+  float pw1 = pow_beta(K.beta1, (float)(from + 1)), pw2 = pow_beta(K.beta2, (float)(from + 1));
+  for (int j = 0; j < n; ++j) {
+    float inv_bc1, inv_sqrt_bc2;
+    adam_bias(K, pw1, pw2, inv_bc1, inv_sqrt_bc2);
+#pragma unroll
+    for (int c = 0; c < VEC; ++c)
+      pp[c] = adam_elem_nograd(mm[c], vv[c], pp[c], lr[c] * inv_bc1, K.beta1, K.beta2, K.eps, inv_sqrt_bc2);
+    pw1 = pw1 * K.beta1; pw2 = pw2 * K.beta2;
+  }
+  if (missed > n) {
+    const int d = missed - n;
+    const float f1 = pow_beta(K.beta1, (float)d), f2 = pow_beta(K.beta2, (float)d);
+#pragma unroll
+    for (int c = 0; c < VEC; ++c) { mm[c] = mm[c] * f1; vv[c] = vv[c] * f2; }
+  }
+}
+
+template <int VEC>
+__device__ __forceinline__ void adam_waiting_step(const CatchUpK& K, int gs, float (&pp)[VEC], float (&mm)[VEC],
+                                                  float (&vv)[VEC], float (&gg)[VEC], const float (&lr)[VEC]) {
+#pragma clang fp contract(off)
+  float inv_bc1, inv_sqrt_bc2;
+  adam_bias(K, pow_beta(K.beta1, (float)gs), pow_beta(K.beta2, (float)gs), inv_bc1, inv_sqrt_bc2);
+#pragma unroll
+  for (int c = 0; c < VEC; ++c) {
+    pp[c] = adam_elem<true>(mm[c], vv[c], pp[c], gg[c] * K.grad_scale, lr[c] * inv_bc1, K.beta1, K.beta2, K.ob1, K.ob2,
+                            K.eps, inv_sqrt_bc2);
+    gg[c] = 0.f;
+  }
+}
+
+template <int VEC> __device__ __forceinline__ bool adam_any_state(const float (&mm)[VEC], const float (&vv)[VEC]) {
+  bool any_state = false;
+#pragma unroll
+  for (int c = 0; c < VEC; ++c) any_state |= (mm[c] != 0.f) | (vv[c] != 0.f);
+  return any_state;
+}
+
+}
diff --git a/clm_gs_amd/csrc/clm_ops.hip b/clm_gs_amd/csrc/clm_ops.hip
--- a/clm_gs_amd/csrc/clm_ops.hip
+++ b/clm_gs_amd/csrc/clm_ops.hip
@@ -1,6 +1,7 @@
 #include <stdlib.h>
 
 #include "common.h"
+#include "adam_step.h"
 #include "vis_math.h"
 #include "radix.h"
 
@@ -191,34 +192,6 @@
   __hip_atomic_store(signal + idx, value, __ATOMIC_RELEASE, __HIP_MEMORY_SCOPE_SYSTEM);
 }
 
-__device__ __forceinline__ float adam_update(float p, float m, float v, float lr_bc, float inv_sqrt_bc2, float eps) {
-#pragma clang fp contract(off)
-  const float ratio = m * __builtin_amdgcn_rcpf(__builtin_fmaf(__builtin_amdgcn_sqrtf(v), inv_sqrt_bc2, eps));
-  return __builtin_fmaf(-lr_bc, ratio, p);
-}
-
-template <bool GRAD_FUSED = false>
-__device__ __forceinline__ float adam_elem(float& m, float& v, float p, float g, float lr_bc, float beta1,
-                                           float beta2, float ob1, float ob2, float eps,
-                                           float inv_sqrt_bc2) {
-#pragma clang fp contract(off)
-  if constexpr (GRAD_FUSED) {
-    m = __builtin_fmaf(ob1, g, beta1 * m);
-    v = __builtin_fmaf(ob2 * g, g, beta2 * v);
-  } else {
-    m = __builtin_fmaf(beta1, m, ob1 * g);
-    v = __builtin_fmaf(beta2, v, (ob2 * g) * g);
-  }
-  return adam_update(p, m, v, lr_bc, inv_sqrt_bc2, eps);
-}
-
-__device__ __forceinline__ float adam_elem_nograd(float& m, float& v, float p, float lr_bc, float beta1, float beta2,
-                                                  float eps, float inv_sqrt_bc2) {
-#pragma clang fp contract(off)
-  m = beta1 * m;
-  v = beta2 * v;
-  return adam_update(p, m, v, lr_bc, inv_sqrt_bc2, eps);
-}
 
 template <int VEC> struct VecT;
 template <> struct VecT<1> { using type = float; };
@@ -260,69 +233,6 @@
     vstore<VEC>(m + o, mm); vstore<VEC>(v + o, vv); vstore<VEC>(p + o, pp);
     if (zero_grad && g) vstore<VEC>(g + o, gg);
   }
-}
-
-__device__ __forceinline__ float pow_beta(float beta, float x) {
-  return __builtin_amdgcn_exp2f(x * __builtin_amdgcn_logf(beta));
-}
-
-struct CatchUpK {
-  float beta1, beta2, ob1, ob2, eps, grad_scale;
-  int bias_correction, max_replay;
-};
-
-__device__ __forceinline__ void adam_bias(const CatchUpK& K, float pw1, float pw2, float& inv_bc1, float& inv_sqrt_bc2) {
-#pragma clang fp contract(off)
-  inv_bc1 = inv_sqrt_bc2 = 1.f;
-  if (K.bias_correction) {
-    inv_bc1 = 1.f / (1.f - pw1);
-    inv_sqrt_bc2 = 1.f / sqrtf(1.f - pw2);
-  }
-}
-
-template <int VEC>
-__device__ __forceinline__ void adam_replay(const CatchUpK& K, int from, int to, float (&pp)[VEC], float (&mm)[VEC],
-                                            float (&vv)[VEC], const float (&lr)[VEC]) {
-#pragma clang fp contract(off)
-  const int missed = to - from;
-  if (missed <= 0) return;
-  const int n = min(missed, K.max_replay);
-  float pw1 = pow_beta(K.beta1, (float)(from + 1)), pw2 = pow_beta(K.beta2, (float)(from + 1));
-  for (int j = 0; j < n; ++j) {
-    float inv_bc1, inv_sqrt_bc2;
-    adam_bias(K, pw1, pw2, inv_bc1, inv_sqrt_bc2);
-#pragma unroll
-    for (int c = 0; c < VEC; ++c)
-      pp[c] = adam_elem_nograd(mm[c], vv[c], pp[c], lr[c] * inv_bc1, K.beta1, K.beta2, K.eps, inv_sqrt_bc2);
-    pw1 = pw1 * K.beta1; pw2 = pw2 * K.beta2;
-  }
-  if (missed > n) {
-    const int d = missed - n;
-    const float f1 = pow_beta(K.beta1, (float)d), f2 = pow_beta(K.beta2, (float)d);
-#pragma unroll
-    for (int c = 0; c < VEC; ++c) { mm[c] = mm[c] * f1; vv[c] = vv[c] * f2; }
-  }
-}
-
-template <int VEC>
-__device__ __forceinline__ void adam_waiting_step(const CatchUpK& K, int gs, float (&pp)[VEC], float (&mm)[VEC],
-                                                  float (&vv)[VEC], float (&gg)[VEC], const float (&lr)[VEC]) {
-#pragma clang fp contract(off)
-  float inv_bc1, inv_sqrt_bc2;
-  adam_bias(K, pow_beta(K.beta1, (float)gs), pow_beta(K.beta2, (float)gs), inv_bc1, inv_sqrt_bc2);
-#pragma unroll
-  for (int c = 0; c < VEC; ++c) {
-    pp[c] = adam_elem<true>(mm[c], vv[c], pp[c], gg[c] * K.grad_scale, lr[c] * inv_bc1, K.beta1, K.beta2, K.ob1, K.ob2,
-                            K.eps, inv_sqrt_bc2);
-    gg[c] = 0.f;
-  }
-}
-
-template <int VEC> __device__ __forceinline__ bool adam_any_state(const float (&mm)[VEC], const float (&vv)[VEC]) {
-  bool any_state = false;
-#pragma unroll
-  for (int c = 0; c < VEC; ++c) any_state |= (mm[c] != 0.f) | (vv[c] != 0.f);
-  return any_state;
 }
 
 template <typename IdxT, int VEC>
diff --git a/clm_gs_amd/csrc/preprocess.hip b/clm_gs_amd/csrc/preprocess.hip
--- a/clm_gs_amd/csrc/preprocess.hip
+++ b/clm_gs_amd/csrc/preprocess.hip
@@ -1,6 +1,7 @@
 #include <stdlib.h>
 
 #include "common.h"
+#include "adam_step.h"
 #include "gs_math.h"
 
 namespace clmgs {
@@ -69,29 +70,89 @@
   __builtin_amdgcn_fence(__ATOMIC_ACQUIRE, "wavefront");
 }
 
-template <int DEG, bool OVERLAP, bool PK, bool AA = false>
-__global__ void __launch_bounds__(PP_ROWS, 3)
+struct FrontStep {
+  float* m; float* v;
+  const float* g;
+  int32_t* last_step;
+  const int32_t* g_step;
+  const float* col_lr;
+  CatchUpK K;
+  int to_step;
+};
+
+struct StepPiece { float mm[4], vv[4], gg[4]; };
+
+__device__ __forceinline__ void step_request_mv(StepPiece& s, const FrontStep& fs, int row, int k, int a) {
+  const int64_t o = (int64_t)row * 48 + 4 * k;
+#pragma unroll
+  for (int c = 0; c < 4; ++c) s.mm[c] = s.vv[c] = 0.f;
+  if (fs.to_step - a > 0) {
+    const float4 m4 = *reinterpret_cast<const float4*>(fs.m + o), v4 = *reinterpret_cast<const float4*>(fs.v + o);
+    s.mm[0] = m4.x; s.mm[1] = m4.y; s.mm[2] = m4.z; s.mm[3] = m4.w;
+    s.vv[0] = v4.x; s.vv[1] = v4.y; s.vv[2] = v4.z; s.vv[3] = v4.w;
+  }
+}
+
+__device__ __forceinline__ void step_request_g(StepPiece& s, const FrontStep& fs, int row, int k, int a, int gs) {
+#pragma unroll
+  for (int c = 0; c < 4; ++c) s.gg[c] = 0.f;
+  if (fs.to_step - a > 0 && gs > a && gs <= fs.to_step) {
+    const float4 g4 = *reinterpret_cast<const float4*>(fs.g + (int64_t)row * 48 + 4 * k);
+    s.gg[0] = g4.x; s.gg[1] = g4.y; s.gg[2] = g4.z; s.gg[3] = g4.w;
+  }
+}
+
+__device__ __forceinline__ void step_apply(StepPiece& s, const FrontStep& fs, float* __restrict__ p, int row, int k,
+                                           int a, int gs, float4& p4) {
+  if (fs.to_step - a <= 0) return;
+  const bool pend = gs > a && gs <= fs.to_step;
+  if (!pend && !adam_any_state<4>(s.mm, s.vv)) return;
+  const int64_t o = (int64_t)row * 48 + 4 * k;
+  const float4 l4 = *reinterpret_cast<const float4*>(fs.col_lr + 4 * k);
+  const float lr[4] = {l4.x, l4.y, l4.z, l4.w};
+  float pp[4] = {p4.x, p4.y, p4.z, p4.w};
+  if (pend) {
+    adam_replay<4>(fs.K, a, gs - 1, pp, s.mm, s.vv, lr);
+    adam_waiting_step<4>(fs.K, gs, pp, s.mm, s.vv, s.gg, lr);
+    a = gs;
+  }
+  adam_replay<4>(fs.K, a, fs.to_step, pp, s.mm, s.vv, lr);
+  p4 = make_float4(pp[0], pp[1], pp[2], pp[3]);
+  *reinterpret_cast<float4*>(fs.m + o) = make_float4(s.mm[0], s.mm[1], s.mm[2], s.mm[3]);
+  *reinterpret_cast<float4*>(fs.v + o) = make_float4(s.vv[0], s.vv[1], s.vv[2], s.vv[3]);
+  *reinterpret_cast<float4*>(p + o) = p4;
+}
+
+template <int DEG, bool OVERLAP, bool PK, bool AA = false, bool STEP = false>
+__global__ void __launch_bounds__(PP_ROWS, STEP ? 2 : 3)
 preprocess_fwd_kernel(int V, PreArgs a, int32_t* __restrict__ radii, float* __restrict__ means2d,
                       float* __restrict__ depths, float* __restrict__ conics,
                       float* __restrict__ colors, float* __restrict__ opacities,
-                      float4* __restrict__ packed) {
+                      float4* __restrict__ packed, FrontStep fs) {
   constexpr int NB = (DEG + 1) * (DEG + 1);
-  constexpr int NF4 = (NB * 3 + 3) / 4;
+  constexpr int NC4 = (NB * 3 + 3) / 4;
+  constexpr int NF4 = STEP ? 12 : NC4;
+  static_assert(!STEP || OVERLAP, "the STEP forward stages before it projects");
   __shared__ __attribute__((aligned(16))) float lds[PP_ROWS * PP_PITCH];
   const Cam cam = load_cam(a.viewmat, a.K);
   const int n_chunks = (V + PP_ROWS - 1) / PP_ROWS;
   const int t = threadIdx.x;
   int chunk = blockIdx.x;
   int my_row = -1, my_sh = 0;
+  int my_a = 0x7fffffff, my_gs = 0;
   if (chunk < n_chunks && chunk * PP_ROWS + t < V) {
     my_row = a.filter ? (int)a.filter[chunk * PP_ROWS + t] : chunk * PP_ROWS + t;
     my_sh = a.sh_index ? a.sh_index[chunk * PP_ROWS + t] : my_row;
+    if constexpr (STEP) { my_a = fs.last_step[my_row]; my_gs = fs.g_step[my_row]; }
   }
   for (; chunk < n_chunks; chunk += gridDim.x) {
     const int base = chunk * PP_ROWS;
     const bool mine = my_row >= 0;
     const int64_t g = mine ? my_row : 0;
     const int sh_id = mine ? my_sh : 0;
+    const int a_row = my_a, gs_row = my_gs;
+    const bool behind = STEP && fs.to_step - a_row > 0;
+    const unsigned long long behind_rows = STEP ? __ballot(behind) : 0ull;
     const SmallRow sr = load_small<PK>(a, g);
     const float m[3] = {sr.m[0], sr.m[1], sr.m[2]};
     const float4 q4 = sr.q4;
@@ -103,17 +164,34 @@
   if constexpr (j < NF4) {                                                                          \
     CLMGS_ELEM(j)                                                                                   \
     const int64_t src = a.sh_by_filter ? (int64_t)__shfl(sh_id, r) : (int64_t)min(base + r, V - 1); \
-    st##j = *reinterpret_cast<const float4*>(a.sh_rows + src * 48 + 4 * k);                         \
+    if (!STEP || NC4 == 12 || k < NC4 || ((behind_rows >> r) & 1ull))   \
+      st##j = *reinterpret_cast<const float4*>(a.sh_rows + src * 48 + 4 * k);                       \
   }
       { CLMGS_LAUNDER_LANE
       CLMGS_FOR12(CLMGS_X)
       }
 #undef CLMGS_X
+    }
+#define CLMGS_DECL_SP(j) StepPiece sp##j;
+    CLMGS_FOR12(CLMGS_DECL_SP)
+#undef CLMGS_DECL_SP
+    if constexpr (STEP) {
+      if (behind_rows) {
+#define CLMGS_X(j) { CLMGS_ELEM(j) step_request_mv(sp##j, fs, __shfl(sh_id, r), k, __shfl(a_row, r)); }
+        { CLMGS_LAUNDER_LANE
+        CLMGS_FOR12(CLMGS_X)
+        }
+#undef CLMGS_X
+      }
     }
     {
       const int ni = (chunk + (int)gridDim.x) * PP_ROWS + t;
       my_row = -1;
-      if (ni < V) { my_row = a.filter ? (int)a.filter[ni] : ni; my_sh = a.sh_index ? a.sh_index[ni] : my_row; }
+      if constexpr (STEP) my_a = 0x7fffffff;
+      if (ni < V) {
+        my_row = a.filter ? (int)a.filter[ni] : ni; my_sh = a.sh_index ? a.sh_index[ni] : my_row;
+        if constexpr (STEP) { my_a = fs.last_step[my_row]; my_gs = fs.g_step[my_row]; }
+      }
     }
     Proj p;
     p.radius = 0; p.mx = p.my = p.depth = p.ca = p.cb = p.cc = 0.f;
@@ -130,6 +208,22 @@
       } else {
         p = project_fwd(cam, m, q, se, (float)a.width, (float)a.height, a.eps2d, a.near_plane,
                         a.far_plane, a.radius_clip);
+      }
+    }
+    if constexpr (STEP) {
+      if (behind_rows) {
+        float* const p_rows = const_cast<float*>(a.sh_rows);
+#define CLMGS_X(j) { CLMGS_ELEM(j) step_request_g(sp##j, fs, __shfl(sh_id, r), k, __shfl(a_row, r), __shfl(gs_row, r)); }
+        { CLMGS_LAUNDER_LANE
+        CLMGS_FOR12(CLMGS_X)
+        }
+#undef CLMGS_X
+#define CLMGS_X(j) { CLMGS_ELEM(j) step_apply(sp##j, fs, p_rows, __shfl(sh_id, r), k, __shfl(a_row, r), __shfl(gs_row, r), st##j); }
+        { CLMGS_LAUNDER_LANE
+        CLMGS_FOR12(CLMGS_X)
+        }
+#undef CLMGS_X
+        if (behind) fs.last_step[g] = fs.to_step;
       }
     }
     wave_lds_sync();
@@ -506,7 +600,8 @@
                                     int height, int degree, float eps2d, float near_plane,
                                     float far_plane, float radius_clip, int32_t* radii,
                                     float* means2d, float* depths, float* conics, float* colors,
-                                    float* opacities, void* packed, const int32_t* sh_index) {
+                                    float* opacities, void* packed, const int32_t* sh_index,
+                                    const FrontStep* step = nullptr) {
   CLMGS_CHECK_ARG(V >= 0 && degree >= 0 && degree <= 3 && width > 0 && height > 0);
   if (V == 0) return 0;
   CLMGS_CHECK_ARG(xyz && sh_rows && viewmat_host && K_host && campos_host && radii && means2d &&
@@ -522,16 +617,34 @@
   a.sh_index = sh_index;
   const size_t lds = 0;
   const int grid = min(ceil_div(V, PP_ROWS), PP_GRID_CAP);
+  FrontStep fs = {};
+  if (step) {
+    CLMGS_CHECK_ARG(filter && sh_by_filter && !sh_index && a.packed_small);
+    fs = *step;
+#define CLMGS_PRE_FWD_STEP(D)                                                                      \
+  hipLaunchKernelGGL((preprocess_fwd_kernel<D, true, true, AA, true>), dim3(grid), dim3(PP_ROWS), lds, \
+                     (hipStream_t)stream, V, a, radii, means2d, depths, conics, colors, opacities, \
+                     (float4*)packed, fs)
+    switch (degree) {
+      case 0: CLMGS_PRE_FWD_STEP(0); break;
+      case 1: CLMGS_PRE_FWD_STEP(1); break;
+      case 2: CLMGS_PRE_FWD_STEP(2); break;
+      default: CLMGS_PRE_FWD_STEP(3); break;
+    }
+#undef CLMGS_PRE_FWD_STEP
+    CLMGS_LAUNCH_CHECK();
+    return 0;
+  }
 #define CLMGS_PRE_FWD(D, O)                                                                        \
   do {                                                                                             \
     if (a.packed_small)                                                                            \
       hipLaunchKernelGGL((preprocess_fwd_kernel<D, O, true, AA>), dim3(grid), dim3(PP_ROWS), lds,      \
                          (hipStream_t)stream, V, a, radii, means2d, depths, conics, colors,        \
-                         opacities, (float4*)packed);                                              \
+                         opacities, (float4*)packed, fs);                                            \
     else                                                                                           \
       hipLaunchKernelGGL((preprocess_fwd_kernel<D, O, false, AA>), dim3(grid), dim3(PP_ROWS), lds,     \
                          (hipStream_t)stream, V, a, radii, means2d, depths, conics, colors,        \
-                         opacities, (float4*)packed);                                              \
+                         opacities, (float4*)packed, fs);                                            \
   } while (0)
   const bool ov = filter != nullptr;
   switch (degree) {
@@ -560,6 +673,20 @@
 extern "C" int clmgs_preprocess_fwd(CLMGS_PRE_FWD_PARAMS) { return preprocess_fwd_impl<false>(CLMGS_PRE_FWD_ARGS); }
 
 extern "C" int clmgs_preprocess_aa_fwd(CLMGS_PRE_FWD_PARAMS) { return preprocess_fwd_impl<true>(CLMGS_PRE_FWD_ARGS); }
+
+extern "C" int clmgs_preprocess_fwd_step(CLMGS_PRE_FWD_PARAMS, int antialiased, float* m, float* v, const float* g,
+                                         int32_t* last_step, const int32_t* g_step, const float* col_lr, double beta1,
+                                         double beta2, double eps, int to_step, int bias_correction, int max_replay,
+                                         float grad_scale) {
+  CLMGS_CHECK_ARG(m && v && g && last_step && g_step && col_lr && to_step >= 0 && max_replay >= 1);
+  CLMGS_CHECK_ARG((((uintptr_t)sh_rows | (uintptr_t)m | (uintptr_t)v | (uintptr_t)g | (uintptr_t)col_lr) & 15) == 0);
+  FrontStep fs = {};
+  fs.m = m; fs.v = v; fs.g = g; fs.last_step = last_step; fs.g_step = g_step; fs.col_lr = col_lr;
+  fs.K = {(float)beta1, (float)beta2, (float)(1.0 - beta1), (float)(1.0 - beta2), (float)eps, grad_scale,
+          bias_correction, max_replay};
+  fs.to_step = to_step;
+  return antialiased ? preprocess_fwd_impl<true>(CLMGS_PRE_FWD_ARGS, &fs) : preprocess_fwd_impl<false>(CLMGS_PRE_FWD_ARGS, &fs);
+}
 
 template <bool ABS>
 static const PreGradsOf<ABS>& pre_grads_of(const PreGradsOf<false>& plain, const PreGradsOf<true>& abs) {
diff --git a/clm_gs_amd/fused.py b/clm_gs_amd/fused.py
--- a/clm_gs_amd/fused.py
+++ b/clm_gs_amd/fused.py
@@ -93,14 +93,14 @@
 
 
 def camera_forward(gaussians, camera, this_filter, sh_rows, sh_by_filter, background, gt_u8,
-                   lambda_dssim=0.2, small_packed=None, streams=None, sh_index=None, exact=True):
+                   lambda_dssim=0.2, small_packed=None, streams=None, sh_index=None, exact=True, row_step=None):
     return camera_forward_finish(gaussians, camera_front(
         gaussians, camera, this_filter, sh_rows, sh_by_filter, background, gt_u8, lambda_dssim,
-        small_packed, streams, sh_index), exact=exact)
+        small_packed, streams, sh_index, row_step), exact=exact)
 
 
 def camera_front(gaussians, camera, this_filter, sh_rows, sh_by_filter, background, gt_u8,
-                 lambda_dssim=0.2, small_packed=None, streams=None, sh_index=None):
+                 lambda_dssim=0.2, small_packed=None, streams=None, sh_index=None, row_step=None):
     L = _lib.lib()
     args = utils.get_args()
     W, H = int(utils.get_img_width()), int(utils.get_img_height())
@@ -156,12 +156,21 @@
         means2d = empty_bucketed(V, (2,), F32, dev).reshape(1, V, 2)
         depths = empty_bucketed(V, (), F32, dev).reshape(1, V)
         packed = p.packed = empty_bucketed(V, (16,), F32, dev)
-        check((L.clmgs_preprocess_aa_fwd if p.antialiased else L.clmgs_preprocess_fwd)(
-            _sptr(s_front), V, dptr(filt, torch.int64, True), *small_in,
-            dptr(sh_rows, F32, allow_host=True), int(sh_by_filter), _np(vm), _np(K), _np(campos), W, H, deg,
-            0.3, 0.01, 1e10, float(getattr(args, "radius_clip", 0.0)), dptr(radii), dptr(means2d),
-            dptr(depths), None, None, None, dptr(packed),
-            dptr(sh_index, I32, True)))
+        pre_args = (_sptr(s_front), V, dptr(filt, torch.int64, True), *small_in,
+                    dptr(sh_rows, F32, allow_host=True), int(sh_by_filter), _np(vm), _np(K), _np(campos), W, H, deg,
+                    0.3, 0.01, 1e10, float(getattr(args, "radius_clip", 0.0)), dptr(radii), dptr(means2d),
+                    dptr(depths), None, None, None, dptr(packed),
+                    dptr(sh_index, I32, True))
+        if row_step is not None and V:
+            assert filt is not None and sh_by_filter and sh_index is None and small_packed is not None and sh_rows.is_cuda
+            st = row_step
+            check(L.clmgs_preprocess_fwd_step(
+                *pre_args, int(p.antialiased), dptr(st["m"], F32), dptr(st["v"], F32), dptr(st["g"], F32),
+                dptr(st["last_step"], I32), dptr(st["g_step"], I32), dptr(st["col_lr"], F32), float(st["beta1"]),
+                float(st["beta2"]), float(st["eps"]), int(st["to_step"]), int(bool(st["bias_correction"])),
+                int(st.get("max_replay", 256)), float(st["grad_scale"])))
+        else:
+            check((L.clmgs_preprocess_aa_fwd if p.antialiased else L.clmgs_preprocess_fwd)(*pre_args))
         if p.invdepth is not None:
             check(L.clmgs_invdepth_pack(_sptr(s_front), V, dptr(radii), dptr(depths), dptr(packed)))
             p.depths = depths
@@ -431,11 +440,11 @@
                      gt_u8, lambda_dssim=0.2, update_stats=True, keep=None, accumulate_after=None,
                      return_event=False, stats_only_visible=False, visibility_out=None,
                      raster_stream=None, small_packed=None, small_grad=None, stats_delta=None, sh_index=None,
-                     sh_stamp=None, cur_step=0):
+                     sh_stamp=None, cur_step=0, row_step=None):
     cur = torch.cuda.current_stream()
     p = camera_forward(gaussians, camera, this_filter, sh_rows, sh_by_filter, background, gt_u8,
                        lambda_dssim, small_packed, (cur, cur, raster_stream if raster_stream is not None else cur),
-                       sh_index, exact=False)
+                       sh_index, exact=False, row_step=row_step)
     camera_backward(gaussians, p, g_sh_rows, small_grad, update_stats, stats_delta,
                     stats_only_visible, visibility_out, accumulate_after, sh_stamp, cur_step)
     loss = camera_loss(p)
diff --git a/clm_gs_amd/strategies/clm_offload/engine.py b/clm_gs_amd/strategies/clm_offload/engine.py
--- a/clm_gs_amd/strategies/clm_offload/engine.py
+++ b/clm_gs_amd/strategies/clm_offload/engine.py
@@ -340,6 +340,14 @@
     b.touched_rows = b.touched_rows.to(torch.int32)
     _lib.STATS.setdefault("touched_rows", []).append(int(b.touched_rows.shape[0]))
     b.ft_stamp = gaussians._row_g_step if (b.lazy and b.fused and gaussians.first_touch_grads) else None
+    b.row_step = None
+    if (getattr(args, "front_row_step", True) and b.ft_stamp is not None and b.use_packed and not dp.active()
+            and not gaussians.moments_sharded and getattr(args, "sh_residency", "hbm") == "hbm" and b.step - 1 > 0):
+        g_, st_ = b.row_adam.param_groups[0], b.row_adam.state[b.params]
+        b.row_step = dict(
+            m=st_["exp_avg"], v=st_["exp_avg_sq"], g=b.grad_buf, last_step=gaussians._row_last_step,
+            g_step=gaussians._row_g_step, col_lr=b.col_lr, beta1=g_["betas"][0], beta2=g_["betas"][1], eps=g_["eps"],
+            to_step=b.step - 1, bias_correction=g_["bias_correction"], grad_scale=1.0 / (args.bsz * dp.world_size()))
 
 
 def _mark_batch(gaussians):
@@ -403,6 +411,8 @@
         if b.owner.hi > b.owner.lo:
             gaussians.catch_up_rows(own_rows, to_step=step - 1)
         dp.owner_gather_rows(params.data, b.owner)
+    elif b.lazy and b.row_step is not None:
+        pass
     elif b.lazy:
         if (b.pipelined and bsz >= 2 and getattr(args, "split_catch_up", True) and b.filters is not None):
             b.foreign_rows = None
@@ -471,7 +481,7 @@
         with _lib.host_region("camera_front"):
             cur_pass = camera_front(gaussians, b.cameras[k], b.filters[k], b.params.data, 1, b.background,
                                     b.cameras[k].original_image, small_packed=b.small_pk,
-                                    streams=(s_front, s_mem, s_raster))
+                                    streams=(s_front, s_mem, s_raster), row_step=b.row_step)
         with _lib.host_region("camera_forward"):
             passes.append(camera_forward_finish(gaussians, cur_pass))
         if k >= 1:
@@ -506,7 +516,7 @@
             losses.append(train_one_camera(
                 gaussians, b.cameras[k], b.filters[k], b.params.data, 1, b.grad_buf, b.background,
                 b.cameras[k].original_image, small_packed=b.small_pk, small_grad=b.small_gk,
-                stats_delta=b.stats_d, sh_stamp=b.ft_stamp, cur_step=b.step))
+                stats_delta=b.stats_d, sh_stamp=b.ft_stamp, cur_step=b.step, row_step=b.row_step))
         return losses
     for k in range(bsz):
         this_filter = b.filters[k]
diff --git a/clm_gs_amd/utils.py b/clm_gs_amd/utils.py
--- a/clm_gs_amd/utils.py
+++ b/clm_gs_amd/utils.py
@@ -66,6 +66,7 @@
         defer_loss_log=True,
         spatial_row_order=True,
         first_touch_grads=True,
+        front_row_step=True,
         host_staging="window",
         placement_candidates=1,
         sh_hbm_budget_gb=0.0,
diff --git a/include/clmgs.h b/include/clmgs.h
--- a/include/clmgs.h
+++ b/include/clmgs.h
@@ -278,6 +278,18 @@
                                 const void* partials, const int64_t* row_cum, const int32_t* sh_index,
                                 int32_t* sh_stamp, int cur_step, float* v_means2d_abs_out);
 
+int clmgs_preprocess_fwd_step(void* stream, int V, const int64_t* filter, const float* xyz,
+                              const float* opacity_raw, const float* scaling_raw,
+                              const float* rotation_raw, const float* sh_rows, int sh_by_filter,
+                              const float* viewmat_host, const float* K_host, const float* campos_host,
+                              int width, int height, int degree, float eps2d, float near_plane,
+                              float far_plane, float radius_clip, int32_t* radii, float* means2d,
+                              float* depths, float* conics, float* colors, float* opacities, void* packed,
+                              const int32_t* sh_index, int antialiased, float* m, float* v, const float* g,
+                              int32_t* last_step, const int32_t* g_step, const float* col_lr, double beta1,
+                              double beta2, double eps, int to_step, int bias_correction, int max_replay,
+                              float grad_scale);
+
 int clmgs_ssim_fwd(void* stream, int B, int CH, int H, int W, const float* img1,
                    const float* img2, float* ssim_sum, float* dm_dmu1, float* dm_dsigma1_sq,
                    float* dm_dsigma12);
```

Measured after the change: 196.5 (median of 3 runs). No clear change (+0.9%).
